# ai-forever/Kandinsky-2

Hardware: AMD Instinct MI355X
Metric: UNet denoise steps/sec @ 768x768 bs=1, 50 steps (higher is better)
Workload: dtype bf16; 1 GPU; Kandinsky-2.x text2img 768x768, decoder_steps=50, bs=1/GPU (CFG batch 2x4x96x96), 2.1-architecture UNet (1.23B) p_sampler step; parity pinned against the reference's modules; head=2.1, tile_configs_measured_in_this_process=0, images_per_gpu=1, parallelism=prompt-sharded x1, weights by one RCCL broadcast, world_size_observed=1, graph=True, chains=1, loop_graph=a 5-step loop replayed as ONE hipGraph (83 replay(s) = 415 timed steps)

## Files before the change

### include/k22.h

```cpp
#ifndef K22_H
#define K22_H
#include <stddef.h>
#include <stdint.h>
#ifdef __cplusplus
extern "C" {
#endif

#define K22_OK 0
#define K22_EINVAL (-1)
#define K22_EHIP (-2)
#define K22_ENOMEM (-3)

#define K22_BF16 0
#define K22_F32 1
#define K22_F16 2
#define K22_F16X3 3
#define K22_F16X2 4

int k22_version(void);
#define K22_BUILD_PACKED_FP32 1
#define K22_BUILD_DEBUG_VARIANTS 2
int k22_build_flags(void);
const char* k22_last_error(void);
int k22_set_option(const char* name, int value);
long k22_debug_counter(const char* name);
size_t k22_stream_frag_bytes(int Npad, int taps, int Kc, int dtype);
int k22_stream_repack(const void* W, void* out, int Npad, int taps, int Kc, int dtype, void* stream);
int k22_debug_set_stream_frag(const void* wfrag, const void* wsfrag);
int k22_debug_set_stream_scratch(void* scratch, size_t bytes);

typedef struct K22UNetConfig {
  int dtype;
  int in_channels;
  int model_channels;
  int out_channels;
  int num_res_blocks;
  int n_levels;
  int channel_mult[8];
  int n_attention_ds;
  int attention_ds[8];
  int num_head_channels;
  int ctx_dim;
  int ctx_len;
  int n_image_embs;
  int text_dim1;
  int text_dim2;
  int image_dim;
  int head_type;
  int hint_channels;
} K22UNetConfig;

typedef struct K22Weight {
  const char* name;
  const void* ptr;
} K22Weight;

typedef struct K22UNet K22UNet;

int k22_unet_create(const K22UNetConfig* cfg, const K22Weight* weights, int n_weights, K22UNet** out);
void k22_unet_destroy(K22UNet* u);


int k22_unet_plan(K22UNet* u, int B, int H, int W, size_t* workspace_bytes);
int k22_unet_bind(K22UNet* u, void* workspace, size_t workspace_bytes);

int k22_unet_set_condition(K22UNet* u, const float* full_emb, const float* pooled_emb, const float* image_emb,
                           void* stream);

int k22_unet_set_hint(K22UNet* u, const float* hint, void* stream);

int k22_unet_forward(K22UNet* u, const float* x, const float* timesteps, const float* inpaint_image,
                     const float* inpaint_mask, float* out, int use_graph, void* stream);

int k22_unet_sample_loop(K22UNet* u, float* x, float* x_tmp, const float* timesteps, const float* noise_seq, const float* init_img,
                         const float* mask, const float* inpaint_image, const float* inpaint_mask, const float* table,
                         const int* table_rows, int n_steps, float guidance, float clamp_lo, float clamp_hi, int pct_index,
                         double pct_gamma, void* scratch, int use_graph, void* stream);
int k22_unet_num_ops(const K22UNet* u);
int k22_unet_set_autotune(K22UNet* u, int on);
int k22_unet_tuning_report(const K22UNet* u, char* buf, size_t cap);

int k22_comm_broadcast_weights(void* arena, size_t bytes, int root, void* nccl_comm, void* stream);

int k22_tile_table_load(const char* path);
int k22_tile_table_save(const char* path);
int k22_tile_table_size(void);
int k22_tile_table_measured(void);
void k22_tile_table_clear(void);

int k22_unet_profile(K22UNet* u, int reps, double* ms, double* flops, double* bytes, int* launches, void* stream);

size_t k22_sampler_scratch_bytes(int N, int HW);
int k22_ddim_step(const float* x, const float* model_out, const float* noise, const float* table_row, float guidance, int use_cfg,
                  float* x_out, float* x0_out, int N, int HW, void* stream);
int k22_prepare_mask(const float* mask, float* out, int C, int H, int W, void* stream);
int k22_plms_step(const float* x, const float* model_out, const float* eps_hist1, const float* eps_hist2, const float* eps_hist3, int order,
                  const float* table_row, float guidance, int use_cfg, float* x_out, float* eps_out, float* x0_out, int N, int HW, void* stream);
int k22_sampler_step(const float* x, const float* model_out, const float* noise, const float* init_img,
                     const float* mask, const float* table, int step_index, float guidance, int use_cfg,
                     float clamp_lo, float clamp_hi, int pct_index, double pct_gamma, void* scratch,
                     float* x_out, float* x0_out, int N, int HW, void* stream);

int k22_gemm(const void* A0, const void* A1, const void* Wp, const float* bias, const void* residual, void* out,
             void* partial, int M, int N, int Npad, int K0, int K1, long lda0, long lda1, int ldo, int ldr,
             int out_f32, int act, int splitk, int bm, int bn, int dtype, void* stream);
int k22_x3_pack(const float* src, void* dst, long n, float scale, void* stream);
int k22_conv3x3(const void* x_padded, const void* Wp, const float* bias, const void* residual, void* out,
                void* partial, int B, int H, int W, int Cin, int Cout, int Npad, int out_mode, int act, int splitk,
                int bm, int bn, int dtype, void* stream);
int k22_conv3x3_skip(const void* x_padded, const void* Wp, const float* bias, const void* skip0, const void* skip1,
                     int SK0, int SK1, const void* Ws, const float* bias_s, void* out, void* partial, int B, int H, int W,
                     int Cin, int Cout, int Npad, int splitk, int bm, int dtype, void* stream);
int k22_conv3x3_gnstats(const void* x_padded, const void* Wp, const float* bias, const void* residual, void* out,
                        void* partial, int B, int H, int W, int Cin, int Cout, int Npad, int splitk, int bm, int bn,
                        float* stats, int stats_capacity_rows, int* rows_per_image, int dtype, void* stream);
int k22_gemm_gnstats(const void* A, const void* Wp, const float* bias, const void* residual, void* out, void* partial,
                     int B, int H, int W, int N, int Npad, int K, int splitk, int bm, float* stats,
                     int stats_capacity_rows, int* rows_per_image, int dtype, void* stream);
typedef struct K22IgemmProblem {
  int dtype, taps, M, N, Kc, K0, H, W;
  int out_mode, res_f32, act, a_raw, want_stats;
  int SK0, SK1;
  int att_T, att_S, att_Tkp;
  int ldo, ldr;
  int has_frag;
  int algo, bm, bn, splitk, stages;
} K22IgemmProblem;
typedef struct K22IgemmOperands {
  const void *A0, *A1, *Wp, *bias, *residual;
  void *out, *partial;
  const void *S0, *S1, *Ws, *bias2;
  void *kall, *vtall;
  const void *Wfrag, *Wsfrag;
  float* stats;
  int stats_capacity_rows;
} K22IgemmOperands;
int k22_igemm_cfg_accepted(const K22IgemmProblem* pr);
int k22_igemm_cfg(const K22IgemmProblem* pr, const K22IgemmOperands* ops, int* rows_per_image, void* stream);
int k22_debug_conv_trace(const void* x_padded, const void* Wp, const float* bias, void* out, int B, int H, int W, int Cin, int Cout,
                         int Npad, unsigned long long* trace, void* stream);
int k22_conv3x3_gn(const void* x0, const void* x1, int C0, int C1, const float* gamma, const float* beta, const float* film, long film_ld,
                   float eps, int act, void* scratch, const void* Wp, const float* bias, const void* residual, void* out, void* partial,
                   int B, int H, int W, int Cout, int Npad, int splitk, int bm, int algo, int dtype, void* stream);
int k22_groupnorm(const void* x0, const void* x1, int C0, int C1, int B, int H, int W, const float* gamma,
                  const float* beta, const float* film, long film_ld, float eps, int act, int mode, int pad,
                  void* scratch, void* out, int dtype, void* stream);
size_t k22_groupnorm_scratch_bytes(int B, int C);
int k22_attention(const void* qkv, const void* ctxkv, void* kall, void* vtall, void* out, int B, int H, int T, int S,
                  int dtype, void* stream);
int k22_qkv_project(const void* x, const void* Wp, const float* bias, void* q_out, void* kall, void* vtall,
                    int B, int H, int T, int S, int K, int bm, int bn, int dtype, void* stream);
int k22_qkv_project_stream(const void* x, const void* Wp, const float* bias, void* q_out, void* kall, void* vtall, void* partial,
                           int B, int H, int T, int S, int K, int bm, int splitk, int dtype, void* stream);
int k22_linear_smallm(const float* x, const void* W, const float* bias, const float* add, float* out, int M, int N,
                      int K, int act_in, int act_out, int wdtype, void* stream);
int k22_conv3x3_direct(const float* x, const float* w, const float* bias, float* y, int B, int Cin, int Cout, int Hin, int Win,
                       int stride, int act, void* stream);

size_t k22_afrag_bytes(int M, int K);
int k22_afrag_pack(const void* A, long lda, void* out, int M, int K, int dtype, void* stream);
int k22_skinny_gemm(const void* Afrag, const void* Wfrag, const float* bias, void* out, float* partial, int M, int N, int Npad, int K,
                    int splitk, int epi, int act, int ldo, int mt, int nb, int dtype, void* stream);
int k22_finish_ln(const float* partial, int splitk, const float* bias, float* x, long ldx, const float* gain, const float* beta, void* yfrag,
                  int M, int N, float eps, int dtype, void* stream);
int k22_small_attention(const void* qkv, const float* qkv_partial, int nsplit, const float* qkv_bias, void* out, int out_frag, int B, int H, int T,
                        int causal, const float* key_valid, int kv_n, int dtype, void* stream);

typedef struct K22PriorConfig {
  int dtype;
  int text_ctx;
  int xf_width;
  int xf_layers;
  int xf_heads;
  int xf_final_ln;
  int clip_dim;
  int clip_xf_width;
} K22PriorConfig;
typedef struct K22Prior K22Prior;
int k22_prior_create(const K22PriorConfig* cfg, const K22Weight* weights, int n_weights, K22Prior** out);
void k22_prior_destroy(K22Prior* m);
int k22_prior_plan(K22Prior* m, int B, size_t* workspace_bytes);
int k22_prior_bind(K22Prior* m, void* workspace, size_t workspace_bytes);
int k22_prior_tuning_report(const K22Prior* m, char* buf, size_t cap);
int k22_prior_forward(K22Prior* m, const float* x, const float* timesteps, const float* text_emb, const float* text_enc,
                      const float* key_valid, float* out, void* stream);
int k22_prior_sampler_step(const float* x, const float* model_out, const float* noise, const float* scales, const float* table_row,
                           float clamp, float* x_out, int bs, int D, void* stream);

typedef struct K22MoVQConfig {
  int dtype;
  int ch;
  int n_levels;
  int ch_mult[8];
  int num_res_blocks;
  int attn_levels;
  int z_channels;
  int out_ch;
} K22MoVQConfig;
typedef struct K22MoVQ K22MoVQ;
int k22_movq_create(const K22MoVQConfig* cfg, const K22Weight* weights, int n_weights, K22MoVQ** out);
void k22_movq_destroy(K22MoVQ* m);
int k22_movq_plan(K22MoVQ* m, int B, int h, int w, size_t* workspace_bytes);
int k22_movq_bind(K22MoVQ* m, void* workspace, size_t workspace_bytes);
int k22_movq_decode(K22MoVQ* m, const float* z, float* out, unsigned char* out_u8, void* stream);
int k22_movq_plan_encoder(K22MoVQ* m, int B, int H, int W, size_t* workspace_bytes);
int k22_movq_encode(K22MoVQ* m, const float* image, float* latent, void* stream);
int k22_movq_num_ops(const K22MoVQ* m);

enum { K22_ENC_CLIP_TEXT = 0, K22_ENC_CLIP_VISION = 1, K22_ENC_XLMR = 2 };
typedef struct K22EncoderConfig {
  int dtype;
  int kind;
  int width;
  int layers;
  int heads;
  int n_ctx;
  int vocab;
  int out_dim;
  int image_size;
  int patch;
  int max_pos;
  int pad_id;
  float ln_eps;
  int mlp_dim;
  int hidden_act;
} K22EncoderConfig;
typedef struct K22Encoder K22Encoder;
int k22_encoder_create(const K22EncoderConfig* cfg, const K22Weight* weights, int n_weights, K22Encoder** out);
void k22_encoder_destroy(K22Encoder* m);
int k22_encoder_plan(K22Encoder* m, int B, size_t* workspace_bytes);
int k22_encoder_bind(K22Encoder* m, void* workspace, size_t workspace_bytes);
int k22_encoder_forward(K22Encoder* m, const int* tokens, const float* key_valid, const float* image, float* seq_out, float* pooled_out,
                        void* stream);

int k22_blend_noised(const float* x, const float* init, const float* noise, const float* mask, float sa, float sb, float* out,
                     int N, int C, int HW, int broadcast_first, void* stream);

#ifdef __cplusplus
}
#endif
#endif
```

### kandinsky-2_amd/_lib.py

```python
from __future__ import annotations

import ctypes as C
import os

_HERE = os.path.dirname(os.path.abspath(__file__))
LIB_PATH = os.environ.get("K22_LIB_PATH") or os.path.join(_HERE, "libk22hip.so")
TILE_TABLE_PATH = os.path.join(_HERE, "tiles_gfx950.txt")

K22_BF16, K22_F32, K22_F16, K22_F16X3, K22_F16X2 = 0, 1, 2, 3, 4
F16X3 = "f16x3"
F16X2 = "f16x2"
SPLIT_DTYPES = (F16X3, F16X2)
X3_WSCALE = 256.0


def dtype_code(backend_dtype) -> int:
    import torch
    try:
        return {torch.bfloat16: K22_BF16, torch.float32: K22_F32, torch.float16: K22_F16, F16X3: K22_F16X3, F16X2: K22_F16X2}[backend_dtype]
    except KeyError:
        raise ValueError('backend_dtype must be torch.bfloat16, torch.float16, torch.float32 "f16x3" or "f16x2"') from None
ACT_NONE, ACT_SILU, ACT_GELU = 0, 1, 2
OUT_ROWMAJOR, OUT_ROWMAJOR_F32, OUT_NCHW_F32, OUT_QKV = 0, 1, 2, 3


class K22UNetConfig(C.Structure):
    _fields_ = [
        ("dtype", C.c_int), ("in_channels", C.c_int), ("model_channels", C.c_int), ("out_channels", C.c_int),
        ("num_res_blocks", C.c_int), ("n_levels", C.c_int), ("channel_mult", C.c_int * 8),
        ("n_attention_ds", C.c_int), ("attention_ds", C.c_int * 8), ("num_head_channels", C.c_int),
        ("ctx_dim", C.c_int), ("ctx_len", C.c_int), ("n_image_embs", C.c_int), ("text_dim1", C.c_int),
        ("text_dim2", C.c_int), ("image_dim", C.c_int), ("head_type", C.c_int), ("hint_channels", C.c_int),
    ]


class K22IgemmProblem(C.Structure):
    _fields_ = [(n, C.c_int) for n in (
        "dtype", "taps", "M", "N", "Kc", "K0", "H", "W", "out_mode", "res_f32", "act", "a_raw", "want_stats", "SK0", "SK1",
        "att_T", "att_S", "att_Tkp", "ldo", "ldr", "has_frag", "algo", "bm", "bn", "splitk", "stages")]


class K22IgemmOperands(C.Structure):
    _fields_ = [(n, C.c_void_p) for n in (
        "A0", "A1", "Wp", "bias", "residual", "out", "partial", "S0", "S1", "Ws", "bias2", "kall", "vtall", "Wfrag", "Wsfrag",
        "stats")] + [("stats_capacity_rows", C.c_int)]


class K22MoVQConfig(C.Structure):
    _fields_ = [("dtype", C.c_int), ("ch", C.c_int), ("n_levels", C.c_int), ("ch_mult", C.c_int * 8),
                ("num_res_blocks", C.c_int), ("attn_levels", C.c_int), ("z_channels", C.c_int), ("out_ch", C.c_int)]


class K22PriorConfig(C.Structure):
    _fields_ = [("dtype", C.c_int), ("text_ctx", C.c_int), ("xf_width", C.c_int), ("xf_layers", C.c_int), ("xf_heads", C.c_int),
                ("xf_final_ln", C.c_int), ("clip_dim", C.c_int), ("clip_xf_width", C.c_int)]


class K22EncoderConfig(C.Structure):
    _fields_ = [("dtype", C.c_int), ("kind", C.c_int), ("width", C.c_int), ("layers", C.c_int), ("heads", C.c_int), ("n_ctx", C.c_int),
                ("vocab", C.c_int), ("out_dim", C.c_int), ("image_size", C.c_int), ("patch", C.c_int), ("max_pos", C.c_int),
                ("pad_id", C.c_int), ("ln_eps", C.c_float), ("mlp_dim", C.c_int), ("hidden_act", C.c_int)]


class K22Weight(C.Structure):
    _fields_ = [("name", C.c_char_p), ("ptr", C.c_void_p)]


_P, _I, _L, _F, _D, _Z = C.c_void_p, C.c_int, C.c_long, C.c_float, C.c_double, C.c_size_t

SIGNATURES = {
    "k22_version": (_I, []),
    "k22_build_flags": (_I, []),
    "k22_last_error": (C.c_char_p, []),
    "k22_set_option": (_I, [C.c_char_p, _I]),
    "k22_comm_broadcast_weights": (_I, [_P, _Z, _I, _P, _P]),
    "k22_tile_table_load": (_I, [C.c_char_p]),
    "k22_tile_table_save": (_I, [C.c_char_p]),
    "k22_tile_table_size": (_I, []),
    "k22_tile_table_measured": (_I, []),
    "k22_tile_table_clear": (None, []),
    "k22_unet_create": (_I, [C.POINTER(K22UNetConfig), C.POINTER(K22Weight), _I, C.POINTER(_P)]),
    "k22_unet_destroy": (None, [_P]),
    "k22_unet_plan": (_I, [_P, _I, _I, _I, C.POINTER(_Z)]),
    "k22_unet_bind": (_I, [_P, _P, _Z]),
    "k22_unet_set_condition": (_I, [_P, _P, _P, _P, _P]),
    "k22_unet_set_hint": (_I, [_P, _P, _P]),
    "k22_unet_forward": (_I, [_P, _P, _P, _P, _P, _P, _I, _P]),
    "k22_unet_sample_loop": (_I, [_P, _P, _P, _P, _P, _P, _P, _P, _P, _P, C.POINTER(_I), _I, _F, _F, _F, _I, _D, _P, _I, _P]),
    "k22_unet_num_ops": (_I, [_P]),
    "k22_unet_set_autotune": (_I, [_P, _I]),
    "k22_unet_tuning_report": (_I, [_P, C.c_char_p, _Z]),
    "k22_unet_profile": (_I, [_P, _I, C.POINTER(_D), C.POINTER(_D), C.POINTER(_D), C.POINTER(_I), _P]),
    "k22_afrag_bytes": (_Z, [_I, _I]),
    "k22_afrag_pack": (_I, [_P, _L, _P, _I, _I, _I, _P]),
    "k22_skinny_gemm": (_I, [_P, _P, _P, _P, _P, _I, _I, _I, _I, _I, _I, _I, _I, _I, _I, _I, _P]),
    "k22_finish_ln": (_I, [_P, _I, _P, _P, _L, _P, _P, _P, _I, _I, _F, _I, _P]),
    "k22_small_attention": (_I, [_P, _P, _I, _P, _P, _I, _I, _I, _I, _I, _P, _I, _I, _P]),
    "k22_prior_create": (_I, [C.POINTER(K22PriorConfig), C.POINTER(K22Weight), _I, C.POINTER(_P)]),
    "k22_prior_destroy": (None, [_P]),
    "k22_prior_plan": (_I, [_P, _I, C.POINTER(_Z)]),
    "k22_prior_bind": (_I, [_P, _P, _Z]),
    "k22_prior_tuning_report": (_I, [_P, C.c_char_p, _Z]),
    "k22_prior_forward": (_I, [_P, _P, _P, _P, _P, _P, _P, _P]),
    "k22_prior_sampler_step": (_I, [_P, _P, _P, _P, _P, _F, _P, _I, _I, _P]),
    "k22_encoder_create": (_I, [C.POINTER(K22EncoderConfig), C.POINTER(K22Weight), _I, C.POINTER(_P)]),
    "k22_encoder_destroy": (None, [_P]),
    "k22_encoder_plan": (_I, [_P, _I, C.POINTER(_Z)]),
    "k22_encoder_bind": (_I, [_P, _P, _Z]),
    "k22_encoder_forward": (_I, [_P, _P, _P, _P, _P, _P, _P]),
    "k22_movq_create": (_I, [C.POINTER(K22MoVQConfig), C.POINTER(K22Weight), _I, C.POINTER(_P)]),
    "k22_movq_destroy": (None, [_P]),
    "k22_movq_plan": (_I, [_P, _I, _I, _I, C.POINTER(_Z)]),
    "k22_movq_bind": (_I, [_P, _P, _Z]),
    "k22_movq_decode": (_I, [_P, _P, _P, _P, _P]),
    "k22_movq_plan_encoder": (_I, [_P, _I, _I, _I, C.POINTER(_Z)]),
    "k22_movq_encode": (_I, [_P, _P, _P, _P]),
    "k22_movq_num_ops": (_I, [_P]),
    "k22_ddim_step": (_I, [_P, _P, _P, _P, _F, _I, _P, _P, _I, _I, _P]),
    "k22_blend_noised": (_I, [_P, _P, _P, _P, _F, _F, _P, _I, _I, _I, _I, _P]),
    "k22_prepare_mask": (_I, [_P, _P, _I, _I, _I, _P]),
    "k22_plms_step": (_I, [_P, _P, _P, _P, _P, _I, _P, _F, _I, _P, _P, _P, _I, _I, _P]),
    "k22_sampler_scratch_bytes": (_Z, [_I, _I]),
    "k22_sampler_step": (_I, [_P, _P, _P, _P, _P, _P, _I, _F, _I, _F, _F, _I, _D, _P, _P, _P, _I, _I, _P]),
    "k22_gemm": (_I, [_P, _P, _P, _P, _P, _P, _P, _I, _I, _I, _I, _I, _L, _L, _I, _I, _I, _I, _I, _I, _I, _I, _P]),
    "k22_x3_pack": (_I, [_P, _P, _L, _F, _P]),
    "k22_conv3x3": (_I, [_P, _P, _P, _P, _P, _P, _I, _I, _I, _I, _I, _I, _I, _I, _I, _I, _I, _I, _P]),
    "k22_conv3x3_skip": (_I, [_P, _P, _P, _P, _P, _I, _I, _P, _P, _P, _P, _I, _I, _I, _I, _I, _I, _I, _I, _I, _P]),
    "k22_gemm_gnstats": (_I, [_P, _P, _P, _P, _P, _P, _I, _I, _I, _I, _I, _I, _I, _I, _P, _I, C.POINTER(_I), _I, _P]),
    "k22_conv3x3_gnstats": (_I, [_P, _P, _P, _P, _P, _P, _I, _I, _I, _I, _I, _I, _I, _I, _I, _P, _I, C.POINTER(_I), _I, _P]),
    "k22_igemm_cfg_accepted": (_I, [C.POINTER(K22IgemmProblem)]),
    "k22_igemm_cfg": (_I, [C.POINTER(K22IgemmProblem), C.POINTER(K22IgemmOperands), C.POINTER(_I), _P]),
    "k22_conv3x3_gn": (_I, [_P, _P, _I, _I, _P, _P, _P, _L, _F, _I, _P, _P, _P, _P, _P, _P, _I, _I, _I, _I, _I, _I, _I, _I, _I, _P]),
    "k22_debug_conv_trace": (_I, [_P, _P, _P, _P, _I, _I, _I, _I, _I, _I, _P, _P]),
    "k22_groupnorm": (_I, [_P, _P, _I, _I, _I, _I, _I, _P, _P, _P, _L, _F, _I, _I, _I, _P, _P, _I, _P]),
    "k22_groupnorm_scratch_bytes": (_Z, [_I, _I]),
    "k22_attention": (_I, [_P, _P, _P, _P, _P, _I, _I, _I, _I, _I, _P]),
    "k22_qkv_project": (_I, [_P, _P, _P, _P, _P, _P, _I, _I, _I, _I, _I, _I, _I, _I, _P]),
    "k22_qkv_project_stream": (_I, [_P, _P, _P, _P, _P, _P, _P, _I, _I, _I, _I, _I, _I, _I, _I, _P]),
    "k22_linear_smallm": (_I, [_P, _P, _P, _P, _P, _I, _I, _I, _I, _I, _I, _P]),
    "k22_conv3x3_direct": (_I, [_P, _P, _P, _P, _I, _I, _I, _I, _I, _I, _I, _P]),
    "k22_debug_counter": (_L, [C.c_char_p]),
    "k22_stream_frag_bytes": (C.c_size_t, [_I, _I, _I, _I]),
    "k22_stream_repack": (_I, [_P, _P, _I, _I, _I, _I, _P]),
    "k22_debug_set_stream_frag": (_I, [_P, _P]),
    "k22_debug_set_stream_scratch": (_I, [_P, C.c_size_t]),
}

_lib = None


def lib() -> C.CDLL:
    global _lib
    if _lib is None:
        if not os.path.exists(LIB_PATH):
            raise RuntimeError(
                f"{LIB_PATH} is missing: the HIP extension is the only compute path (no CPU fallback). "
                "Build it with `python -c 'import __graft_entry__ as g; g.build()'`.")
        l = C.CDLL(LIB_PATH)
        for name, (res, args) in SIGNATURES.items():
            fn = getattr(l, name)
            fn.restype = res
            fn.argtypes = args
        _lib = l
        tbl = os.environ.get("K22_TILE_TABLE", TILE_TABLE_PATH)
        if tbl != "0" and os.path.exists(tbl):
            if l.k22_tile_table_load(tbl.encode()) < 0:
                raise RuntimeError(f"k22: cannot read the tile table {tbl}")
    return _lib


def check(rc: int) -> None:
    if rc != 0:
        msg = lib().k22_last_error()
        raise RuntimeError(f"k22 error {rc}: {msg.decode() if msg else ''}")


def weight_array(arena, table):
    base = arena.data_ptr()
    arr = (K22Weight * len(table))()
    names = []
    for i, (name, (off, _n)) in enumerate(table.items()):
        nb = name.encode()
        names.append(nb)
        arr[i].name = nb
        arr[i].ptr = base + off
    return arr, names


def plan_and_bind(plan_fn, bind_fn, handle, device, *shape):
    import torch
    nbytes = C.c_size_t()
    check(plan_fn(handle, *shape, C.byref(nbytes)))
    ws = torch.empty(nbytes.value + 256, dtype=torch.uint8, device=device)
    check(bind_fn(handle, (ws.data_ptr() + 255) // 256 * 256, nbytes.value))
    return ws


def ptr(t) -> int:
    if t is None:
        return None
    assert t.is_contiguous(), "k22: tensors crossing the C ABI must be contiguous"
    return t.data_ptr()


def current_stream() -> int:
    import torch
    return torch.cuda.current_stream().cuda_stream
```

### kandinsky-2_amd/csrc/capi.hip

```cpp
#include "kernels.h"
#include "elementwise.h"
#include "../../include/k22.h"
#include "tuning.h"
#include "skinny.h"
#include <dlfcn.h>
#include <stdio.h>
#include <string.h>

static thread_local char g_err[512] = "";

int k22_set_error(int code, const char* msg) {
  snprintf(g_err, sizeof(g_err), "%s", msg ? msg : "");
  return code;
}
int k22_set_error_hip(hipError_t e, const char* file, int line) {
  snprintf(g_err, sizeof(g_err), "HIP error %d (%s) at %s:%d", (int)e, hipGetErrorString(e), file, line);
  return K22_EHIP;
}

extern "C" {

int k22_version(void) { return 100; }
int k22_build_flags(void) {
  int f = 0;
#ifndef K22_NOPK
  f |= K22_BUILD_PACKED_FP32;
#endif
#if defined(K22_DEBUG_VARIANTS) || defined(K22_STREAM_DEBUG) || defined(K22_SKINNY_DEBUG)
  f |= K22_BUILD_DEBUG_VARIANTS;
#endif
  return f;
}

int k22_set_option(const char* name, int value) {
  if (name && !strcmp(name, "igemm_stages")) { igemm_set_default_stages(value); return K22_OK; }
  if (name && !strcmp(name, "igemm_xcd_remap")) { igemm_set_xcd_remap(value); return K22_OK; }
  if (name && !strcmp(name, "conv_algo")) { igemm_set_conv_algo(value); return K22_OK; }
  if (name && !strcmp(name, "gemm_algo")) { igemm_set_gemm_algo(value); return K22_OK; }
  return k22_set_error(K22_EINVAL, "k22_set_option: unknown option");
}
const char* k22_last_error(void) { return g_err; }

#ifdef K22_STREAM_DEBUG
static unsigned long long* g_dbg_trace = nullptr;
extern "C" int k22_debug_set_stream_trace(unsigned long long* t) { g_dbg_trace = t; return K22_OK; }
#define K22_DBG_TRACE(p) (p).st_trace = g_dbg_trace
#else
#define K22_DBG_TRACE(p) (void)0
#endif
static const void* g_dbg_wfrag = nullptr;
static const void* g_dbg_wsfrag = nullptr;
static void* g_dbg_scratch = nullptr;
static size_t g_dbg_scratch_bytes = 0;
static int dbg_frag(IgemmParams& p, int dtype, hipStream_t st) {
  K22_DBG_TRACE(p);
  p.Wfrag = g_dbg_wfrag; p.Wsfrag = g_dbg_wsfrag;
  if (g_dbg_wfrag || !g_dbg_scratch || dtype == K22_F32 || (p.taps != 1 && p.taps != 9) || p.Kc % 64 || p.Npad % 64) return K22_OK;
  const size_t n1 = stream_frag_bytes(p.Npad, p.taps, p.Kc, dtype);
  const bool skip = p.S0 != nullptr && p.Ws != nullptr && (p.SK0 + p.SK1) % 64 == 0;
  const size_t n2 = skip ? stream_frag_bytes(p.Npad, 1, p.SK0 + p.SK1, dtype) : 0;
  if (n1 + n2 > g_dbg_scratch_bytes) return k22_set_error(K22_ENOMEM, "debug stream scratch too small");
  if (int rc = launch_stream_repack(p.Wp, g_dbg_scratch, p.Npad, p.taps, p.Kc, dtype, st)) return rc;
  p.Wfrag = g_dbg_scratch;
  if (skip) {
    void* w2 = static_cast<char*>(g_dbg_scratch) + n1;
    if (int rc = launch_stream_repack(p.Ws, w2, p.Npad, 1, p.SK0 + p.SK1, dtype, st)) return rc;
    p.Wsfrag = w2;
  }
  return K22_OK;
}
#define K22_DBG_FRAG(p) do { if (int rc_ = dbg_frag((p), dtype, reinterpret_cast<hipStream_t>(stream))) return rc_; } while (0)
int k22_debug_set_stream_frag(const void* wfrag, const void* wsfrag) { g_dbg_wfrag = wfrag; g_dbg_wsfrag = wsfrag; return K22_OK; }
int k22_debug_set_stream_scratch(void* scratch, size_t bytes) { g_dbg_scratch = scratch; g_dbg_scratch_bytes = scratch ? bytes : 0; return K22_OK; }
size_t k22_stream_frag_bytes(int Npad, int taps, int Kc, int dtype) { return stream_frag_bytes(Npad, taps, Kc, dtype); }
int k22_stream_repack(const void* W, void* out, int Npad, int taps, int Kc, int dtype, void* stream) {
  return launch_stream_repack(W, out, Npad, taps, Kc, dtype, reinterpret_cast<hipStream_t>(stream));
}

long k22_debug_counter(const char* name) {
  if (name && !strcmp(name, "stream_launches")) return stream_launch_count();
  return -1;
}

int k22_comm_broadcast_weights(void* arena, size_t bytes, int root, void* nccl_comm, void* stream) {
  if (!arena || !nccl_comm) return k22_set_error(K22_EINVAL, "k22_comm_broadcast_weights: null arena / communicator");
  typedef int (*bcast_fn)(const void*, void*, size_t, int , int, void*, hipStream_t);
  static bcast_fn fn = nullptr;
  if (!fn) {
    void* sym = dlsym(RTLD_DEFAULT, "ncclBroadcast");
    if (!sym) {
      void* h = dlopen("librccl.so.1", RTLD_NOW | RTLD_GLOBAL);
      if (!h) h = dlopen("librccl.so", RTLD_NOW | RTLD_GLOBAL);
      if (h) sym = dlsym(h, "ncclBroadcast");
    }
    if (!sym) return k22_set_error(K22_EINVAL, "k22_comm_broadcast_weights: RCCL (ncclBroadcast) is not loadable in this process");
    fn = reinterpret_cast<bcast_fn>(sym);
  }
  const size_t piece = (size_t)1 << 30;
  char* base = reinterpret_cast<char*>(arena);
  for (size_t off = 0; off < bytes; off += piece) {
    const size_t n = bytes - off < piece ? bytes - off : piece;
    const int rc = fn(base + off, base + off, n,  1, root, nccl_comm, reinterpret_cast<hipStream_t>(stream));
    if (rc != 0) { char msg[96]; snprintf(msg, sizeof msg, "k22_comm_broadcast_weights: ncclBroadcast returned %d", rc); return k22_set_error(K22_EHIP, msg); }
  }
  return K22_OK;
}

int k22_tile_table_load(const char* path) {
  if (!path) return k22_set_error(K22_EINVAL, "k22_tile_table_load: null path");
  const int n = tile_table_load_file(path);
  if (n < 0) return k22_set_error(K22_EINVAL, "k22_tile_table_load: cannot read the file");
  return n;
}
int k22_tile_table_save(const char* path) {
  if (!path) return k22_set_error(K22_EINVAL, "k22_tile_table_save: null path");
  const int n = tile_table_save_file(path);
  if (n < 0) return k22_set_error(K22_EINVAL, "k22_tile_table_save: cannot write the file");
  return n;
}
int k22_tile_table_size(void) {
  TileTable& tt = tile_table();
  std::lock_guard<std::mutex> lk(tt.mu);
  return (int)tt.m.size();
}
int k22_tile_table_measured(void) {
  TileTable& tt = tile_table();
  std::lock_guard<std::mutex> lk(tt.mu);
  return (int)tt.measured;
}
void k22_tile_table_clear(void) {
  TileTable& tt = tile_table();
  std::lock_guard<std::mutex> lk(tt.mu);
  tt.m.clear();
  tt.measured = 0;
}

int k22_gemm(const void* A0, const void* A1, const void* Wp, const float* bias, const void* residual, void* out,
             void* partial, int M, int N, int Npad, int K0, int K1, long lda0, long lda1, int ldo, int ldr,
             int out_f32, int act, int splitk, int bm, int bn, int dtype, void* stream) {
  IgemmParams p = {};
    p.stages = -1;
  p.A0 = A0; p.A1 = A1; p.Wp = Wp; p.bias = bias; p.residual = residual; p.out = out;
  p.partial = reinterpret_cast<float*>(partial);
  p.M = M; p.N = N; p.Npad = Npad; p.Kc = K0 + K1; p.K0 = K0; p.taps = 1; p.lda0 = lda0; p.lda1 = lda1;
  p.ldo = ldo; p.ldr = ldr; p.out_mode = out_f32 ? IG_OUT_ROWMAJOR_F32 : IG_OUT_ROWMAJOR; p.act = act;
  p.splitk = splitk; p.force_bm = bm; p.force_bn = bn;
  p.a_raw = k22_is_split(dtype) ? 1 : 0;
  if (p.splitk == 0) p.splitk = partial ? igemm_choose_splitk(p, dtype) : 1;
  K22_DBG_FRAG(p);
  return launch_igemm(p, dtype, reinterpret_cast<hipStream_t>(stream));
}

int k22_x3_pack(const float* src, void* dst, long n, float scale, void* stream) {
  if (!src || !dst || n < 0) return k22_set_error(K22_EINVAL, "x3_pack: null argument");
  return launch_x3_pack(src, dst, n, scale, reinterpret_cast<hipStream_t>(stream));
}

int k22_conv3x3(const void* x_padded, const void* Wp, const float* bias, const void* residual, void* out,
                void* partial, int B, int H, int W, int Cin, int Cout, int Npad, int out_mode, int act, int splitk,
                int bm, int bn, int dtype, void* stream) {
  IgemmParams p = {};
    p.stages = -1;
  p.A0 = x_padded; p.Wp = Wp; p.bias = bias; p.residual = residual; p.out = out;
  p.partial = reinterpret_cast<float*>(partial);
  p.M = B * H * W; p.N = Cout; p.Npad = Npad; p.Kc = Cin; p.K0 = Cin; p.taps = 9; p.H = H; p.W = W;
  p.ldo = Cout; p.ldr = Cout; p.out_mode = out_mode; p.act = act; p.splitk = splitk; p.force_bm = bm; p.force_bn = bn;
  if (p.splitk == 0) p.splitk = partial ? igemm_choose_splitk(p, dtype) : 1;
  K22_DBG_FRAG(p);
  return launch_igemm(p, dtype, reinterpret_cast<hipStream_t>(stream));
}

int k22_conv3x3_gnstats(const void* x_padded, const void* Wp, const float* bias, const void* residual, void* out,
                        void* partial, int B, int H, int W, int Cin, int Cout, int Npad, int splitk, int bm, int bn,
                        float* stats, int stats_capacity_rows, int* rows_per_image, int dtype, void* stream) {
  IgemmParams p = {};
  p.stages = -1;
  p.A0 = x_padded; p.Wp = Wp; p.bias = bias; p.residual = residual; p.out = out;
  p.partial = reinterpret_cast<float*>(partial);
  p.M = B * H * W; p.N = Cout; p.Npad = Npad; p.Kc = Cin; p.K0 = Cin; p.taps = 9; p.H = H; p.W = W;
  p.ldo = Cout; p.ldr = Cout; p.out_mode = IG_OUT_ROWMAJOR; p.act = K22_ACT_NONE; p.splitk = splitk; p.force_bm = bm; p.force_bn = bn;
  if (p.splitk == 0) p.splitk = partial ? igemm_choose_splitk(p, dtype) : 1;
  const int rpi = igemm_stats_rows_per_image(p, dtype);
  if (rows_per_image) *rows_per_image = rpi;
  if (rpi <= 0) return k22_set_error(K22_EINVAL, "conv3x3_gnstats: this configuration cannot produce GroupNorm partial sums");
  if (rpi * B > stats_capacity_rows) return k22_set_error(K22_ENOMEM, "conv3x3_gnstats: stats buffer too small");
  p.stats = stats;
  K22_DBG_FRAG(p);
  return launch_igemm(p, dtype, reinterpret_cast<hipStream_t>(stream));
}

int k22_gemm_gnstats(const void* A, const void* Wp, const float* bias, const void* residual, void* out, void* partial,
                     int B, int H, int W, int N, int Npad, int K, int splitk, int bm, float* stats,
                     int stats_capacity_rows, int* rows_per_image, int dtype, void* stream) {
  IgemmParams p = {};
  p.stages = -1;
  p.A0 = A; p.Wp = Wp; p.bias = bias; p.residual = residual; p.out = out; p.partial = reinterpret_cast<float*>(partial);
  p.M = B * H * W; p.N = N; p.Npad = Npad; p.Kc = K; p.K0 = K; p.taps = 1; p.H = H; p.W = W; p.lda0 = K;
  p.ldo = N; p.ldr = N; p.out_mode = IG_OUT_ROWMAJOR; p.act = K22_ACT_NONE; p.splitk = splitk > 0 ? splitk : 1;
  p.force_bm = bm; p.algo = (bm == 160 || bm == 288) ? 20 : 10;
  p.a_raw = k22_is_split(dtype) ? 1 : 0;
  const int rpi = igemm_stats_rows_per_image(p, dtype);
  if (rows_per_image) *rows_per_image = rpi;
  if (rpi <= 0) return k22_set_error(K22_EINVAL, "gemm_gnstats: this configuration cannot produce GroupNorm partial sums");
  if (rpi * B > stats_capacity_rows) return k22_set_error(K22_ENOMEM, "gemm_gnstats: stats buffer too small");
  p.stats = stats;
  K22_DBG_FRAG(p);
  return launch_igemm(p, dtype, reinterpret_cast<hipStream_t>(stream));
}

int k22_conv3x3_skip(const void* x_padded, const void* Wp, const float* bias, const void* skip0, const void* skip1,
                     int SK0, int SK1, const void* Ws, const float* bias_s, void* out, void* partial, int B, int H, int W,
                     int Cin, int Cout, int Npad, int splitk, int bm, int dtype, void* stream) {
  IgemmParams p = {};
  p.stages = -1;
  p.A0 = x_padded; p.Wp = Wp; p.bias = bias; p.out = out; p.partial = reinterpret_cast<float*>(partial);
  p.M = B * H * W; p.N = Cout; p.Npad = Npad; p.Kc = Cin; p.K0 = Cin; p.taps = 9; p.H = H; p.W = W;
  p.ldo = Cout; p.ldr = Cout; p.out_mode = IG_OUT_ROWMAJOR; p.act = K22_ACT_NONE; p.splitk = splitk; p.force_bm = bm; p.force_bn = 0;
  p.S0 = skip0; p.S1 = skip1; p.SK0 = SK0; p.SK1 = SK1; p.Ws = Ws; p.bias2 = bias_s; p.algo = 0;
  if (p.splitk == 0) p.splitk = partial ? igemm_choose_splitk(p, dtype) : 1;
  K22_DBG_FRAG(p);
  return launch_igemm(p, dtype, reinterpret_cast<hipStream_t>(stream));
}

static int igemm_problem_tuned(const K22IgemmProblem& d, Tuned& t) {
  if (d.dtype < K22_BF16 || d.dtype > K22_F16X2) return k22_set_error(K22_EINVAL, "igemm_cfg: bad dtype");
  if ((d.taps != 1 && d.taps != 9) || d.M <= 0 || d.N <= 0 || d.Kc <= 0 || d.K0 <= 0 || d.K0 > d.Kc)
    return k22_set_error(K22_EINVAL, "igemm_cfg: bad problem (taps 1 / 9, M, N > 0, 0 < K0 <= Kc)");
  if (d.out_mode < IG_OUT_ROWMAJOR || d.out_mode > IG_OUT_QKV || d.SK0 < 0 || d.SK1 < 0 || (d.SK1 > 0 && d.SK0 == 0))
    return k22_set_error(K22_EINVAL, "igemm_cfg: bad output mode / skip widths");
  if (d.taps == 9 && (d.H <= 0 || d.W <= 0 || d.M % (d.H * d.W))) return k22_set_error(K22_EINVAL, "igemm_cfg: a convolution needs M = B * H * W");
  const void* mark = reinterpret_cast<const void*>(1);
  IgemmParams& p = t.p;
  p = IgemmParams{};
  p.stages = -1;
  p.M = d.M; p.N = d.N; p.Npad = (d.N + 63) / 64 * 64; p.Kc = d.Kc; p.K0 = d.K0; p.taps = d.taps; p.H = d.H; p.W = d.W;
  p.lda0 = d.K0; p.lda1 = d.Kc - d.K0;
  p.ldo = d.ldo > 0 ? d.ldo : (d.out_mode == IG_OUT_QKV ? d.N / 3 : d.N);
  p.ldr = d.ldr > 0 ? d.ldr : (d.res_f32 ? p.ldo : d.N);
  p.out_mode = d.out_mode; p.act = d.act; p.res_f32 = d.res_f32 ? 1 : 0; p.a_raw = d.a_raw ? 1 : 0;
  p.Wp = mark; p.bias = reinterpret_cast<const float*>(mark);
  if (d.SK0 > 0) { p.S0 = mark; p.S1 = d.SK1 > 0 ? mark : nullptr; p.SK0 = d.SK0; p.SK1 = d.SK1; p.Ws = mark; p.bias2 = reinterpret_cast<const float*>(mark); }
  if (d.out_mode == IG_OUT_QKV) { p.att_T = d.att_T; p.att_S = d.att_S; p.att_Tkp = d.att_Tkp; }
  if (d.has_frag) { p.Wfrag = mark; if (d.SK0 > 0) p.Wsfrag = mark; }
  t.want_stats = d.want_stats != 0;
  t.dt = d.dtype;
  tuned_make_candidates(t, d.dtype);
  return K22_OK;
}
static Cfg igemm_problem_cfg(const K22IgemmProblem& d) {
  Cfg c; c.algo = d.algo; c.bm = d.bm; c.bn = d.bn; c.splitk = d.splitk; c.stages = d.stages;
  return c;
}

int k22_igemm_cfg_accepted(const K22IgemmProblem* pr) {
  if (!pr) return k22_set_error(K22_EINVAL, "igemm_cfg_accepted: null problem");
  Tuned t;
  if (int rc = igemm_problem_tuned(*pr, t)) return rc;
  return tuned_is_candidate(t, igemm_problem_cfg(*pr)) ? 1 : 0;
}

int k22_igemm_cfg(const K22IgemmProblem* pr, const K22IgemmOperands* ops, int* rows_per_image, void* stream) {
  if (rows_per_image) *rows_per_image = 0;
  if (!pr || !ops) return k22_set_error(K22_EINVAL, "igemm_cfg: null problem / operands");
  const K22IgemmProblem& d = *pr;
  const K22IgemmOperands& o = *ops;
  Tuned t;
  if (int rc = igemm_problem_tuned(d, t)) return rc;
  const Cfg c = igemm_problem_cfg(d);
  if (!tuned_is_candidate(t, c)) return k22_set_error(K22_EINVAL, "igemm_cfg: this build does not generate the configuration for the problem");
  if (!o.A0 || !o.Wp || !o.out) return k22_set_error(K22_EINVAL, "igemm_cfg: A0, Wp and out are required");
  if (d.K0 < d.Kc && !o.A1) return k22_set_error(K22_EINVAL, "igemm_cfg: A1 missing for the concat operand");
  if (d.SK0 > 0 && (!o.S0 || !o.Ws || (d.SK1 > 0 && !o.S1))) return k22_set_error(K22_EINVAL, "igemm_cfg: fused-skip operands missing");
  if (d.out_mode == IG_OUT_QKV && (!o.kall || !o.vtall)) return k22_set_error(K22_EINVAL, "igemm_cfg: kall / vtall missing");
  if ((c.splitk > 1 || c.algo == 20) && !o.partial) return k22_set_error(K22_EINVAL, "igemm_cfg: the configuration needs the fp32 partial buffer");
  if (c.algo == 20 && (!o.Wfrag || (d.SK0 > 0 && !o.Wsfrag))) return k22_set_error(K22_EINVAL, "igemm_cfg: algo 20 needs the fragment-major weights");
  IgemmParams q = t.p;
  tuned_apply_cfg(q, c);
  q.A0 = o.A0; q.A1 = o.A1; q.Wp = o.Wp; q.bias = reinterpret_cast<const float*>(o.bias); q.residual = o.residual; q.out = o.out;
  q.partial = reinterpret_cast<float*>(o.partial);
  q.S0 = d.SK0 > 0 ? o.S0 : nullptr; q.S1 = d.SK1 > 0 ? o.S1 : nullptr; q.Ws = d.SK0 > 0 ? o.Ws : nullptr;
  q.bias2 = d.SK0 > 0 ? reinterpret_cast<const float*>(o.bias2) : nullptr;
  q.kall = o.kall; q.vtall = o.vtall;
  q.Wfrag = c.algo == 20 ? o.Wfrag : nullptr; q.Wsfrag = (c.algo == 20 && d.SK0 > 0) ? o.Wsfrag : nullptr;
  if (t.want_stats) {
    const int rpi = igemm_stats_rows_per_image(q, d.dtype);
    const int B = d.H > 0 ? d.M / (d.H * d.W) : 1;
    if (rpi <= 0) return k22_set_error(K22_EINVAL, "igemm_cfg: this configuration cannot produce GroupNorm partial sums");
    if (!o.stats || (long)rpi * B > o.stats_capacity_rows) return k22_set_error(K22_ENOMEM, "igemm_cfg: stats buffer missing / too small");
    if (rows_per_image) *rows_per_image = rpi;
    q.stats = o.stats;
  }
  return launch_igemm(q, d.dtype, reinterpret_cast<hipStream_t>(stream));
}

int k22_debug_conv_trace(const void* x_padded, const void* Wp, const float* bias, void* out, int B, int H, int W, int Cin, int Cout,
                         int Npad, unsigned long long* trace, void* stream) {
  IgemmParams p = {};
  p.stages = -1;
  p.A0 = x_padded; p.Wp = Wp; p.bias = bias; p.out = out;
  p.M = B * H * W; p.N = Cout; p.Npad = Npad; p.Kc = Cin; p.K0 = Cin; p.taps = 9; p.H = H; p.W = W;
  p.ldo = Cout; p.ldr = Cout; p.out_mode = IG_OUT_ROWMAJOR; p.act = K22_ACT_NONE; p.splitk = 1; p.trace = trace;
  return launch_conv3_halo_trace(p, K22_BF16, reinterpret_cast<hipStream_t>(stream));
}

size_t k22_groupnorm_scratch_bytes(int B, int C) {
  return (size_t)B * 128 * C * 2 * sizeof(float) + (size_t)B * C * 2 * sizeof(float) + 512;
}

int k22_groupnorm(const void* x0, const void* x1, int C0, int C1, int B, int H, int W, const float* gamma,
                  const float* beta, const float* film, long film_ld, float eps, int act, int mode, int pad,
                  void* scratch, void* out, int dtype, void* stream) {
  hipStream_t st = reinterpret_cast<hipStream_t>(stream);
  const int C = C0 + C1, HW = H * W;
  const int out_x3 = k22_is_split(dtype) ? 1 : 0;
  dtype = k22_storage_dtype(dtype);
  float* partial = reinterpret_cast<float*>(scratch);
  float* coeff = partial + (size_t)B * 128 * C * 2;
  const int rc = launch_gn_stats_coeff(x0, x1, C0, C1, B, HW, eps, gamma, beta, film, film_ld, partial, coeff, dtype, st);
  if (rc) return rc;
  GnApplyParams ap = {};
  ap.x0 = x0; ap.x1 = x1; ap.C0 = C0; ap.C1 = C1; ap.B = B; ap.H = H; ap.W = W; ap.mode = mode; ap.pad = pad; ap.act = act;
  ap.coeff = coeff; ap.out = out; ap.out_x3 = out_x3;
  return launch_gn_apply(ap, dtype, st);
}

int k22_conv3x3_gn(const void* x0, const void* x1, int C0, int C1, const float* gamma, const float* beta, const float* film, long film_ld,
                   float eps, int act, void* scratch, const void* Wp, const float* bias, const void* residual, void* out, void* partial,
                   int B, int H, int W, int Cout, int Npad, int splitk, int bm, int algo, int dtype, void* stream) {
  hipStream_t st = reinterpret_cast<hipStream_t>(stream);
  const int C = C0 + C1, HW = H * W;
  const int sdt = k22_storage_dtype(dtype);
  float* part = reinterpret_cast<float*>(scratch);
  float* coeff = part + (size_t)B * 128 * C * 2;
  const int rc = launch_gn_stats_coeff(x0, x1, C0, C1, B, HW, eps, gamma, beta, film, film_ld, part, coeff, sdt, st);
  if (rc) return rc;
  IgemmParams p = {};
  p.stages = -1;
  p.Wp = Wp; p.bias = bias; p.residual = residual; p.out = out; p.partial = reinterpret_cast<float*>(partial);
  p.M = B * H * W; p.N = Cout; p.Npad = Npad; p.Kc = C; p.K0 = C; p.taps = 9; p.H = H; p.W = W;
  p.ldo = Cout; p.ldr = Cout; p.out_mode = IG_OUT_ROWMAJOR; p.act = K22_ACT_NONE; p.splitk = splitk > 0 ? splitk : 1; p.force_bm = bm; p.algo = algo;
  p.gn_coeff = coeff; p.gn_x0 = x0; p.gn_x1 = x1; p.gn_C0 = C0; p.gn_act = act;
  return launch_igemm(p, dtype, st);
}


int k22_attention(const void* qkv, const void* ctxkv, void* kall, void* vtall, void* out, int B, int H, int T, int S,
                  int dtype, void* stream) {
  hipStream_t st = reinterpret_cast<hipStream_t>(stream);
  const int C = H * 64, Tk = S + T, Tkp = (Tk + 63) / 64 * 64;
  KvPackParams kp;
  kp.qkv = qkv; kp.ctxkv = ctxkv; kp.kall = kall; kp.vtall = vtall; kp.B = B; kp.H = H; kp.T = T; kp.S = S; kp.Tkp = Tkp;
  int rc = launch_kv_pack(kp, k22_storage_dtype(dtype), st);
  if (rc) return rc;
  AttentionParams ap = {};
  ap.q = qkv; ap.ldq = 3 * C; ap.kall = kall; ap.vtall = vtall; ap.out = out; ap.ldo = C;
  ap.B = B; ap.H = H; ap.T = T; ap.Tk = Tk; ap.Tkp = Tkp; ap.scale = 0.125f;
  return launch_attention(ap, dtype, st);
}

int k22_qkv_project(const void* x, const void* Wp, const float* bias, void* q_out, void* kall, void* vtall,
                    int B, int H, int T, int S, int K, int bm, int bn, int dtype, void* stream) {
  const int C = H * 64, Tkp = (S + T + 63) / 64 * 64;
  IgemmParams p = {};
  p.stages = -1;
  p.A0 = x; p.Wp = Wp; p.bias = bias; p.out = q_out; p.kall = kall; p.vtall = vtall;
  p.M = B * T; p.N = 3 * C; p.Npad = 3 * C; p.Kc = K; p.K0 = K; p.taps = 1; p.lda0 = K; p.lda1 = 0;
  p.ldo = C; p.ldr = 3 * C; p.out_mode = IG_OUT_QKV; p.act = K22_ACT_NONE; p.splitk = 1; p.force_bm = bm; p.force_bn = bn;
  p.att_T = T; p.att_S = S; p.att_Tkp = Tkp; p.H = 1; p.W = T;
  p.a_raw = k22_is_split(dtype) ? 1 : 0;
  K22_DBG_FRAG(p);
  return launch_igemm(p, dtype, reinterpret_cast<hipStream_t>(stream));
}

int k22_qkv_project_stream(const void* x, const void* Wp, const float* bias, void* q_out, void* kall, void* vtall, void* partial,
                           int B, int H, int T, int S, int K, int bm, int splitk, int dtype, void* stream) {
  const int C = H * 64, Tkp = (S + T + 63) / 64 * 64;
  IgemmParams p = {};
  p.stages = -1;
  p.A0 = x; p.Wp = Wp; p.bias = bias; p.out = q_out; p.kall = kall; p.vtall = vtall; p.partial = reinterpret_cast<float*>(partial);
  p.M = B * T; p.N = 3 * C; p.Npad = 3 * C; p.Kc = K; p.K0 = K; p.taps = 1; p.lda0 = K; p.lda1 = 0;
  p.ldo = C; p.ldr = 3 * C; p.out_mode = IG_OUT_QKV; p.act = K22_ACT_NONE; p.splitk = splitk > 0 ? splitk : 1; p.force_bm = bm; p.algo = 20;
  p.att_T = T; p.att_S = S; p.att_Tkp = Tkp; p.H = 1; p.W = T;
  if (!stream_supported(p, dtype, bm == 288 ? 9 : 5)) return k22_set_error(K22_EINVAL, "qkv_project_stream: unsupported problem");
  K22_DBG_FRAG(p);
  return launch_igemm(p, dtype, reinterpret_cast<hipStream_t>(stream));
}

size_t k22_afrag_bytes(int M, int K) { return afrag_bytes(M, K); }
int k22_afrag_pack(const void* A, long lda, void* out, int M, int K, int dtype, void* stream) {
  return launch_afrag_pack(A, lda, out, M, K, dtype, reinterpret_cast<hipStream_t>(stream));
}
int k22_skinny_gemm(const void* Afrag, const void* Wfrag, const float* bias, void* out, float* partial, int M, int N, int Npad, int K,
                    int splitk, int epi, int act, int ldo, int mt, int nb, int dtype, void* stream) {
  SkinnyParams q = {};
  q.Af = Afrag; q.Wf = Wfrag; q.bias = bias; q.out = out; q.partial = partial; q.M = M; q.N = N; q.Npad = Npad; q.K = K; q.MA = (M + 31) / 32;
  q.splitk = splitk > 0 ? splitk : 1; q.epi = epi; q.act = act; q.ldo = ldo;
  q.trace = reinterpret_cast<unsigned long long*>(g_dbg_scratch);
  return launch_skinny(q, dtype, mt, nb, reinterpret_cast<hipStream_t>(stream));
}
int k22_finish_ln(const float* partial, int splitk, const float* bias, float* x, long ldx, const float* gain, const float* beta, void* yfrag,
                  int M, int N, float eps, int dtype, void* stream) {
  FinishLnParams q = {};
  q.partial = partial; q.splitk = splitk; q.bias = bias; q.x = x; q.ldx = ldx; q.g = gain; q.b = beta; q.yfrag = yfrag; q.M = M; q.N = N;
  q.MA = (M + 31) / 32; q.eps = eps;
  return launch_finish_ln(q, dtype, reinterpret_cast<hipStream_t>(stream));
}
int k22_small_attention(const void* qkv, const float* qkv_partial, int nsplit, const float* qkv_bias, void* out, int out_frag, int B, int H, int T,
                        int causal, const float* key_valid, int kv_n, int dtype, void* stream) {
  SmallAttnParams ap = {};
  ap.qkv = qkv; ap.part = qkv_partial; ap.nsplit = nsplit; ap.bias = qkv_bias; ap.ldq = 3 * H * 64; ap.out = out; ap.ldo = H * 64; ap.out_frag = out_frag; ap.MA = (B * T + 31) / 32;
  ap.B = B; ap.H = H; ap.T = T; ap.scale = 0.125f; ap.causal = causal; ap.key_valid = key_valid; ap.kv_ld = kv_n; ap.kv_n = kv_n;
  return launch_small_attention(ap, dtype, reinterpret_cast<hipStream_t>(stream));
}

int k22_linear_smallm(const float* x, const void* W, const float* bias, const float* add, float* out, int M, int N,
                      int K, int act_in, int act_out, int wdtype, void* stream) {
  LinearSmallParams lp = {};
  lp.x = x; lp.ldx = K; lp.W = W; lp.bias = bias; lp.add = add; lp.ld_add = N; lp.out = out; lp.ldo = N;
  lp.M = M; lp.N = N; lp.K = K; lp.act_in = act_in; lp.act_out = act_out;
  return launch_linear_smallm(lp, wdtype, reinterpret_cast<hipStream_t>(stream));
}

int k22_conv3x3_direct(const float* x, const float* w, const float* bias, float* y, int B, int Cin, int Cout, int Hin, int Win,
                       int stride, int act, void* stream) {
  if (!x || !w || !bias || !y) return k22_set_error(K22_EINVAL, "conv3x3_direct: null argument");
  if (B < 1 || Cin < 1 || Cout < 1 || Hin < 1 || Win < 1) return k22_set_error(K22_EINVAL, "conv3x3_direct: empty shape");
  if (act != K22_ACT_NONE && act != K22_ACT_SILU) return k22_set_error(K22_EINVAL, "conv3x3_direct: act must be 0 (none) or 1 (SiLU)");
  ConvDirectParams p = {};
  p.x = x; p.w = w; p.bias = bias; p.y = y;
  p.B = B; p.Cin = Cin; p.Cout = Cout; p.Hin = Hin; p.Win = Win; p.stride = stride; p.act = act;
  return launch_conv3x3_direct(p, reinterpret_cast<hipStream_t>(stream));
}

int k22_ddim_step(const float* x, const float* model_out, const float* noise, const float* table_row, float guidance, int use_cfg,
                  float* x_out, float* x0_out, int N, int HW, void* stream) {
  if (!x || !model_out || !table_row || !x_out) return k22_set_error(K22_EINVAL, "ddim_step: null argument");
  return launch_ddim_step(x, model_out, noise, table_row, guidance, use_cfg, x_out, x0_out, N, HW, reinterpret_cast<hipStream_t>(stream));
}

int k22_prepare_mask(const float* mask, float* out, int C, int H, int W, void* stream) {
  if (!mask || !out) return k22_set_error(K22_EINVAL, "prepare_mask: null argument");
  return launch_prepare_mask(mask, out, C, H, W, reinterpret_cast<hipStream_t>(stream));
}

int k22_plms_step(const float* x, const float* model_out, const float* eps_hist1, const float* eps_hist2, const float* eps_hist3, int order,
                  const float* table_row, float guidance, int use_cfg, float* x_out, float* eps_out, float* x0_out, int N, int HW, void* stream) {
  if (!x || !model_out || !table_row || !x_out) return k22_set_error(K22_EINVAL, "plms_step: null argument");
  return launch_plms_step(x, model_out, eps_hist1, eps_hist2, eps_hist3, order, table_row, guidance, use_cfg, x_out, eps_out, x0_out, N, HW,
                          reinterpret_cast<hipStream_t>(stream));
}

size_t k22_sampler_scratch_bytes(int N, int HW) { return (size_t)N * 4 * HW * sizeof(float) + 256; }

int k22_sampler_step(const float* x, const float* model_out, const float* noise, const float* init_img,
                     const float* mask, const float* table, int step_index, float guidance, int use_cfg,
                     float clamp_lo, float clamp_hi, int pct_index, double pct_gamma, void* scratch,
                     float* x_out, float* x0_out, int N, int HW, void* stream) {
  SamplerParams p = {};
  p.x = x; p.model_out = model_out; p.noise = noise; p.init_img = init_img; p.mask = mask; p.table = table;
  p.step = nullptr; p.step_host = step_index; p.guidance = guidance; p.clamp_lo = clamp_lo; p.clamp_hi = clamp_hi;
  p.use_cfg = use_cfg; p.n_lo = pct_index; p.gamma = pct_gamma;
  p.s_buf = reinterpret_cast<float*>(scratch);
  p.x0_buf = reinterpret_cast<float*>(scratch) + 64;
  p.x_out = x_out; p.x0_out = x0_out; p.N = N; p.HW = HW;
  if (pct_index >= 4 * HW) return k22_set_error(K22_EINVAL, "sampler: percentile index out of range");
  return launch_sampler_step(p, reinterpret_cast<hipStream_t>(stream));
}

}

__global__ __launch_bounds__(256) void lds_sentinel_kernel(int words, int spins, unsigned* rec) {
  extern __shared__ unsigned sent_lds[];
  for (int i = threadIdx.x; i < words; i += 256) sent_lds[i] = 0xA5000000u | (unsigned)i;
  __syncthreads();
  for (int s = 0; s < spins; ++s) {
    for (int i = threadIdx.x; i < words; i += 256) {
      const unsigned v = reinterpret_cast<volatile unsigned*>(sent_lds)[i];
      if (v != (0xA5000000u | (unsigned)i)) {
        const unsigned k = atomicAdd(rec, 1u);
        if (k < 255u) { rec[1 + 4 * k] = blockIdx.x; rec[2 + 4 * k] = 4u * i; rec[3 + 4 * k] = v; rec[4 + 4 * k] = (unsigned)s; }
        sent_lds[i] = 0xA5000000u | (unsigned)i;
      }
    }
    __builtin_amdgcn_s_sleep(8);
  }
}
extern "C" int k22_debug_lds_sentinel(int bytes, int workgroups, int spins, unsigned* rec, void* stream) {
  if (bytes <= 0 || bytes > 64 * 1024 || (bytes & 3) || !rec) return k22_set_error(K22_EINVAL, "lds_sentinel: bytes in 4..65536, multiple of 4");
  hipLaunchKernelGGL(lds_sentinel_kernel, dim3(workgroups), dim3(256), (size_t)bytes, reinterpret_cast<hipStream_t>(stream), bytes / 4, spins, rec);
  K22_CHECK_LAUNCH();
  return K22_OK;
}
```

### kandinsky-2_amd/csrc/elementwise.h

```cpp
#pragma once
#include "common.h"

struct GnStatsParams {
  const void* x0; const void* x1;
  int C0, C1, HW, B, groups, nsplit;
  float* partial;
};
struct GnSrc { const float* st; int rpi, C; };
struct GnCoeffParams {
  GnSrc src[2];
  int HW, C, groups; float eps;
  const float* gamma; const float* beta;
  const float* film; int64_t film_ld;
  float* coeff;
};
struct GnApplyParams {
  const void* x0; const void* x1; int C0, C1;
  int B, H, W;
  int mode;
  int pad;
  int act;
  const float* coeff;
  void* out;
  int out_x3;
};
struct ConvInParams {
  const float* x; const float* img; const float* mask;
  const float* w; const float* bias;
  void* out;
  int B, H, W, Cin, Cout;
  int img_premul;
};
struct ConvDirectParams {
  const float* x; const float* w; const float* bias; float* y;
  int B, Cin, Cout, Hin, Win, stride, act;
};
int launch_conv3x3_direct(const ConvDirectParams& p, hipStream_t s);
struct LinearSmallParams {
  const float* x; int64_t ldx;
  const void* W;
  const float* bias;
  const float* add; int64_t ld_add;
  int add_mod;
  float* out; int64_t ldo;
  int M, N, K, act_in, act_out;
  int rows_per_wave;
};
struct KvPackParams {
  const void* qkv; const void* ctxkv; void* kall; void* vtall;
  int B, H, T, S, Tkp;
};
struct AttentionParams {
  const void* q; int64_t ldq;
  const void* kall; const void* vtall;
  void* out; int64_t ldo;
  int B, H, T, Tk, Tkp;
  float scale;
  int causal;
  const float* key_valid;
  int kv_ld, kv_n;
  int out_x3;
};
struct SmallAttnParams {
  const void* qkv; int64_t ldq;
  const float* part; int nsplit; const float* bias;
  void* out; int64_t ldo;
  int out_frag, MA;
  int B, H, T;
  float scale;
  int causal;
  const float* key_valid; int kv_ld, kv_n;
};
struct SamplerParams {
  const float* x;
  const float* model_out;
  const float* noise;
  const float* init_img;
  const float* mask;
  const float* table;
  const int* step;
  int step_host;
  float guidance, clamp_lo, clamp_hi;
  int use_cfg;
  int n_lo; double gamma;
  float* x0_buf;
  float* s_buf;
  float* x_out;
  float* x0_out;
  int N, HW;
};

int launch_x3_pack(const float* in, void* out, int64_t n, float scale, hipStream_t s);
int gn_nsplit(int B, int HW);
int launch_gn_stats(const GnStatsParams& p, int dtype, hipStream_t s);
int launch_gn_coeff(const GnCoeffParams& p, int B, hipStream_t s);
inline int launch_gn_stats_coeff(const void* x0, const void* x1, int C0, int C1, int B, int HW, float eps, const float* gamma, const float* beta,
                                 const float* film, int64_t film_ld, float* partial, float* coeff, int dtype, hipStream_t s) {
  const int nsplit = gn_nsplit(B, HW), C = C0 + C1;
  GnStatsParams sp = {};
  sp.x0 = x0; sp.x1 = x1; sp.C0 = C0; sp.C1 = C1; sp.HW = HW; sp.B = B; sp.groups = 32; sp.nsplit = nsplit; sp.partial = partial;
  const int rc = launch_gn_stats(sp, dtype, s);
  if (rc) return rc;
  GnCoeffParams cp = {};
  cp.src[0].st = partial; cp.src[0].rpi = nsplit; cp.src[0].C = C;
  cp.HW = HW; cp.C = C; cp.groups = 32; cp.eps = eps; cp.gamma = gamma; cp.beta = beta; cp.film = film; cp.film_ld = film_ld; cp.coeff = coeff;
  return launch_gn_coeff(cp, B, s);
}
int launch_gn_apply(const GnApplyParams& p, int dtype, hipStream_t s);
int launch_resample(const void* x, void* y, int B, int H, int W, int C, int mode, int dtype, hipStream_t s);
int launch_conv_in(const ConvInParams& p, int dtype, hipStream_t s);
int launch_timestep_embedding(const float* t, const float* freqs, float* out, int B, int half, hipStream_t s);
int launch_linear_smallm(const LinearSmallParams& p, int wdtype, hipStream_t s);
int launch_layernorm_f32(const float* x, const float* g, const float* b, float* y, int rows, int D, float eps, hipStream_t s);
int launch_cast_rows(const float* x, void* y, int rows, int cols, int64_t ldx, int64_t ldy, int dtype, hipStream_t s);
int launch_kv_pack(const KvPackParams& p, int dtype, hipStream_t s);
int launch_attention(const AttentionParams& p, int dtype, hipStream_t s);
int launch_small_attention(const SmallAttnParams& p, int dtype, hipStream_t s);
int launch_sampler_step(const SamplerParams& p, hipStream_t s);
int launch_plms_step(const float* x, const float* model_out, const float* h1, const float* h2, const float* h3, int order, const float* tab,
                     float guidance, int use_cfg, float* x_out, float* e_store, float* x0_out, int N, int HW, hipStream_t s);
int launch_prepare_mask(const float* old_mask, float* out, int C, int H, int W, hipStream_t s);
int launch_ddim_step(const float* x, const float* model_out, const float* noise, const float* tab, float guidance, int use_cfg,
                     float* x_out, float* x0_out, int N, int HW, hipStream_t s);

struct SpatialNormParams {
  const void* x;
  const float* coeff;
  const float* zq;
  const float* wy; const float* by;
  const float* wb; const float* bb;
  void* out;
  int B, H, W, C, h0, w0, shift, act, pad;
};
int launch_spatialnorm_apply(const SpatialNormParams& p, int dtype, hipStream_t s);
int launch_upsample2_pad(const void* x, void* y, int B, int H, int W, int C, int dtype, hipStream_t s);
int launch_softmax_rows(void* x, int64_t rows, int L, float scale, int dtype, hipStream_t s);
int launch_movq_prepare(const float* z, const float* wpq, const float* bpq, float* zq, void* xin, int B, int h, int w,
                        int Cpad, int dtype, hipStream_t s);
int launch_movq_enc_prepare(const float* img, void* xin, int B, int H, int W, int Cpad, int dtype, hipStream_t s);
int launch_pad_copy(const void* x, void* y, int B, int H, int W, int C, int dtype, hipStream_t s);
int launch_subsample_odd(const void* x, void* y, int B, int H, int W, int C, int dtype, hipStream_t s);
int launch_movq_quant_conv(const float* h, const float* wq, const float* bq, float* out, int B, int HW, hipStream_t s);
int launch_to_uint8_nhwc(const float* x, unsigned char* y, int B, int C, int H, int W, hipStream_t s);
```

### kandinsky-2_amd/csrc/elementwise.hip

```cpp
#include "kernels.h"
#include "elementwise.h"

__device__ __forceinline__ void load4(const bf16_t* p, float* f) {
  const uint2 r = *reinterpret_cast<const uint2*>(p);
  f[0] = __uint_as_float(r.x << 16); f[1] = __uint_as_float(r.x & 0xffff0000u);
  f[2] = __uint_as_float(r.y << 16); f[3] = __uint_as_float(r.y & 0xffff0000u);
}
__device__ __forceinline__ void load4(const f16_t* p, float* f) {
  const uint2 r = *reinterpret_cast<const uint2*>(p);
  unpack2_f16(r.x, f[0], f[1]); unpack2_f16(r.y, f[2], f[3]);
}
__device__ __forceinline__ void load4(const float* p, float* f) {
  const float4 r = *reinterpret_cast<const float4*>(p);
  f[0] = r.x; f[1] = r.y; f[2] = r.z; f[3] = r.w;
}

template <typename T>
__global__ __launch_bounds__(256) void gn_stats_kernel(GnStatsParams p) {
  __shared__ float red[1024 * 2 * 2];
  const int tid = threadIdx.x, b = blockIdx.y, s = blockIdx.x;
  const int C = p.C0 + p.C1, VP = C / 4;
  const int per = (p.HW + p.nsplit - 1) / p.nsplit;
  const int pix0 = s * per, pix1 = min(p.HW, pix0 + per);
  const T* x0 = reinterpret_cast<const T*>(p.x0) + (int64_t)b * p.HW * p.C0;
  const T* x1 = p.x1 ? reinterpret_cast<const T*>(p.x1) + (int64_t)b * p.HW * p.C1 : nullptr;
  int PL, pl;
  if (VP >= 256) { PL = 1; pl = 0; } else { PL = 256 / VP; pl = tid / VP; }
  float sum[3][4], sq[3][4];
  int vj[3];
#pragma unroll
  for (int j = 0; j < 3; ++j) {
    int v = (VP >= 256) ? tid + 256 * j : ((j == 0 && pl < PL) ? tid - pl * VP : VP);
    vj[j] = v < VP ? v : -1;
#pragma unroll
    for (int k = 0; k < 4; ++k) { sum[j][k] = 0.f; sq[j][k] = 0.f; }
  }
#pragma unroll
  for (int j = 0; j < 3; ++j) {
    if (vj[j] >= 0) {
      const int c = vj[j] * 4;
      const T* src = c < p.C0 ? x0 + c : x1 + (c - p.C0);
      const int64_t ld = c < p.C0 ? p.C0 : p.C1;
      int pix = pix0 + pl;
      for (; pix + 7 * PL < pix1; pix += 8 * PL) {
        float f[8][4];
#pragma unroll
        for (int u = 0; u < 8; ++u) load4(src + (int64_t)(pix + u * PL) * ld, f[u]);
#pragma unroll
        for (int k = 0; k < 4; ++k) {
          sum[j][k] += ((f[0][k] + f[1][k]) + (f[2][k] + f[3][k])) + ((f[4][k] + f[5][k]) + (f[6][k] + f[7][k]));
          sq[j][k] += ((f[0][k] * f[0][k] + f[1][k] * f[1][k]) + (f[2][k] * f[2][k] + f[3][k] * f[3][k])) +
                      ((f[4][k] * f[4][k] + f[5][k] * f[5][k]) + (f[6][k] * f[6][k] + f[7][k] * f[7][k]));
        }
      }
      for (; pix < pix1; pix += PL) {
        float f[4];
        load4(src + (int64_t)pix * ld, f);
#pragma unroll
        for (int k = 0; k < 4; ++k) { sum[j][k] += f[k]; sq[j][k] += f[k] * f[k]; }
      }
    }
  }
  float* out = p.partial + ((int64_t)b * p.nsplit + s) * C * 2;
  if (PL == 1) {
#pragma unroll
    for (int j = 0; j < 3; ++j)
      if (vj[j] >= 0) {
        float* o = out + (int64_t)vj[j] * 8;
        *reinterpret_cast<float4*>(o) = make_float4(sum[j][0], sq[j][0], sum[j][1], sq[j][1]);
        *reinterpret_cast<float4*>(o + 4) = make_float4(sum[j][2], sq[j][2], sum[j][3], sq[j][3]);
      }
    return;
  }
  if (vj[0] >= 0) {
    float* o = red + ((int64_t)pl * C + vj[0] * 4) * 2;
    *reinterpret_cast<float4*>(o) = make_float4(sum[0][0], sq[0][0], sum[0][1], sq[0][1]);
    *reinterpret_cast<float4*>(o + 4) = make_float4(sum[0][2], sq[0][2], sum[0][3], sq[0][3]);
  }
  __syncthreads();
  for (int i = tid; i < C * 2; i += 256) {
    float a = 0.f;
    for (int q = 0; q < PL; ++q) a += red[(int64_t)q * C * 2 + i];
    out[i] = a;
  }
}

__global__ __launch_bounds__(256) void gn_coeff_kernel(GnCoeffParams p) {
  __shared__ double red[4][2];
  __shared__ float ms[2];
  const int tid = threadIdx.x, lane = tid & 63, wave = tid >> 6, g = blockIdx.x, b = blockIdx.y;
  const int cg = p.C / p.groups;
  float pg = 0.f, pb = 0.f, psc = 1.f, psh = 0.f;
  if (tid < cg) {
    const int c = g * cg + tid;
    pg = p.gamma[c]; pb = p.beta[c];
    if (p.film != nullptr) {
      psc = 1.f + p.film[(int64_t)b * p.film_ld + c];
      psh = p.film[(int64_t)b * p.film_ld + p.C + c];
    }
  }
  double s = 0.0, q = 0.0;
  int off = 0;
#pragma unroll
  for (int k = 0; k < 2; ++k) {
    const GnSrc sr = p.src[k];
    if (sr.C > 0) {
      const int c_lo = max(g * cg, off), c_hi = min((g + 1) * cg, off + sr.C);
      const int nc = c_hi - c_lo;
      if (nc > 0) {
        const float* base = sr.st + ((int64_t)b * sr.rpi * sr.C + (c_lo - off)) * 2;
        const int items = sr.rpi * nc;
        int i = tid;
        for (; i + 768 < items; i += 1024) {
          float2 v[4];
#pragma unroll
          for (int u = 0; u < 4; ++u) {
            const int ii = i + 256 * u, r = ii / nc, cc = ii - r * nc;
            v[u] = *reinterpret_cast<const float2*>(base + ((int64_t)r * sr.C + cc) * 2);
          }
          s += ((double)v[0].x + (double)v[1].x) + ((double)v[2].x + (double)v[3].x);
          q += ((double)v[0].y + (double)v[1].y) + ((double)v[2].y + (double)v[3].y);
        }
        for (; i < items; i += 256) {
          const int r = i / nc, cc = i - r * nc;
          const float2 v = *reinterpret_cast<const float2*>(base + ((int64_t)r * sr.C + cc) * 2);
          s += (double)v.x;
          q += (double)v.y;
        }
      }
    }
    off += sr.C;
  }
#pragma unroll
  for (int o = 32; o > 0; o >>= 1) {
    s += __shfl_xor(s, o, 64);
    q += __shfl_xor(q, o, 64);
  }
  if (lane == 0) { red[wave][0] = s; red[wave][1] = q; }
  __syncthreads();
  if (tid == 0) {
    const double st = (red[0][0] + red[1][0]) + (red[2][0] + red[3][0]);
    const double qt = (red[0][1] + red[1][1]) + (red[2][1] + red[3][1]);
    const double n = (double)p.HW * (double)cg;
    const double mean = st / n;
    double var = qt / n - mean * mean;
    if (var < 0.0) var = 0.0;
    ms[0] = (float)mean;
    ms[1] = (float)(1.0 / sqrt(var + (double)p.eps));
  }
  __syncthreads();
  const float mean_f = ms[0], rstd_f = ms[1];
  if (tid < cg) {
    const int c = g * cg + tid;
    float A = rstd_f * pg;
    float Bc = pb - mean_f * A;
    if (p.film != nullptr) {
      A *= psc;
      Bc = Bc * psc + psh;
    }
    *reinterpret_cast<float2*>(p.coeff + ((int64_t)b * p.C + c) * 2) = make_float2(A, Bc);
  }
}

template <typename T>
__global__ __launch_bounds__(256) void gn_apply_kernel(GnApplyParams p) {
  constexpr int EPV = Vec16<T>::N;
  const bool fast = p.out_x3 != 0;
  const int C = p.C0 + p.C1, CV = C / EPV;
  const int Ho = p.mode == 1 ? p.H / 2 : (p.mode == 2 ? p.H * 2 : p.H);
  const int Wo = p.mode == 1 ? p.W / 2 : (p.mode == 2 ? p.W * 2 : p.W);
  const int pad = p.pad, Hp = Ho + 2 * pad, Wp = Wo + 2 * pad;
  const int idx = blockIdx.x * 256 + threadIdx.x;
  if (idx >= Wp * CV) return;
  const int xp = idx / CV, cv = idx - xp * CV;
  const int xo = xp - pad, yo = (int)blockIdx.y - pad, b = blockIdx.z;
  T* out = reinterpret_cast<T*>(p.out) + (((int64_t)b * Hp + blockIdx.y) * Wp + xp) * C + cv * EPV;
  Vec16<T> o;
  if (xo < 0 || yo < 0 || xo >= Wo || yo >= Ho) {
#pragma unroll
    for (int k = 0; k < EPV / 2; ++k) o.set2(k, 0.f, 0.f);
  } else {
    const int c = cv * EPV;
    const T* src; int cs, ld;
    if (c < p.C0) { src = reinterpret_cast<const T*>(p.x0); cs = c; ld = p.C0; }
    else { src = reinterpret_cast<const T*>(p.x1); cs = c - p.C0; ld = p.C1; }
    float A[EPV], Bc[EPV];
    const float* cf = p.coeff + ((int64_t)b * C + c) * 2;
#pragma unroll
    for (int k = 0; k < EPV; k += 2) {
      const float4 q = *reinterpret_cast<const float4*>(cf + 2 * k);
      A[k] = q.x; Bc[k] = q.y; A[k + 1] = q.z; Bc[k + 1] = q.w;
    }
    float r[EPV];
    if (p.mode == 1) {
      Vec16<T> v[4];
#pragma unroll
      for (int dy = 0; dy < 2; ++dy)
#pragma unroll
        for (int dx = 0; dx < 2; ++dx)
          v[dy * 2 + dx].raw = *reinterpret_cast<const decltype(v[0].raw)*>(src + ((int64_t)(b * p.H + 2 * yo + dy) * p.W + 2 * xo + dx) * ld + cs);
#pragma unroll
      for (int k = 0; k < EPV; ++k) {
        float acc = 0.f;
#pragma unroll
        for (int q = 0; q < 4; ++q) acc += fast ? apply_act_sel<true>(v[q].get(k) * A[k] + Bc[k], p.act) : apply_act_sel<false>(v[q].get(k) * A[k] + Bc[k], p.act);
        r[k] = acc * 0.25f;
      }
    } else {
      const int yi = p.mode == 2 ? yo >> 1 : yo, xi = p.mode == 2 ? xo >> 1 : xo;
      Vec16<T> v;
      v.raw = *reinterpret_cast<const decltype(v.raw)*>(src + ((int64_t)(b * p.H + yi) * p.W + xi) * ld + cs);
#pragma unroll
      for (int k = 0; k < EPV; ++k) r[k] = fast ? apply_act_sel<true>(v.get(k) * A[k] + Bc[k], p.act) : apply_act_sel<false>(v.get(k) * A[k] + Bc[k], p.act);
    }
#pragma unroll
    for (int k = 0; k < EPV / 2; ++k) o.set2(k, r[2 * k], r[2 * k + 1]);
  }
  if constexpr (sizeof(T) == 4) {
    if (p.out_x3) { x3_store4(out, x3_split4(o.raw)); return; }
  }
  *reinterpret_cast<decltype(o.raw)*>(out) = o.raw;
}

template <typename T>
__global__ __launch_bounds__(256) void resample_kernel(const void* xin, void* yout, int B, int H, int W, int C, int mode) {
  constexpr int EPV = Vec16<T>::N;
  const int CV = C / EPV;
  const int Ho = mode == 1 ? H / 2 : H * 2, Wo = mode == 1 ? W / 2 : W * 2;
  const int64_t total = (int64_t)B * Ho * Wo * CV;
  const T* x = reinterpret_cast<const T*>(xin);
  T* y = reinterpret_cast<T*>(yout);
  for (int64_t i = (int64_t)blockIdx.x * 256 + threadIdx.x; i < total; i += (int64_t)gridDim.x * 256) {
    const int cv = (int)(i % CV);
    int64_t t = i / CV;
    const int xo = (int)(t % Wo); t /= Wo;
    const int yo = (int)(t % Ho);
    const int b = (int)(t / Ho);
    Vec16<T> o;
    if (mode == 1) {
      float r[EPV];
#pragma unroll
      for (int k = 0; k < EPV; ++k) r[k] = 0.f;
#pragma unroll
      for (int dy = 0; dy < 2; ++dy)
#pragma unroll
        for (int dx = 0; dx < 2; ++dx) {
          Vec16<T> v;
          v.raw = *reinterpret_cast<const decltype(v.raw)*>(x + ((int64_t)(b * H + 2 * yo + dy) * W + 2 * xo + dx) * C + cv * EPV);
#pragma unroll
          for (int k = 0; k < EPV; ++k) r[k] += v.get(k);
        }
#pragma unroll
      for (int k = 0; k < EPV / 2; ++k) o.set2(k, r[2 * k] * 0.25f, r[2 * k + 1] * 0.25f);
    } else {
      o.raw = *reinterpret_cast<const decltype(o.raw)*>(x + ((int64_t)(b * H + (yo >> 1)) * W + (xo >> 1)) * C + cv * EPV);
    }
    *reinterpret_cast<decltype(o.raw)*>(y + i * EPV) = o.raw;
  }
}

constexpr int CONV_IN_PT = 8;
template <typename T, int CIN>
__global__ __launch_bounds__(128) void conv_in_kernel(ConvInParams p) {
  constexpr int PT = CONV_IN_PT, PW = PT + 2;
  __shared__ float patch[CIN][3][PW];
  const int tid = threadIdx.x;
  const int xt = blockIdx.x, y = blockIdx.y, b = blockIdx.z;
  const int x0 = xt * PT;
  const int hw = p.H * p.W;
  for (int i = tid; i < CIN * 3 * PW; i += 128) {
    const int c = i / (3 * PW), r = (i / PW) % 3, xx = i % PW;
    const int yy = y + r - 1, xs = x0 + xx - 1;
    float v = 0.f;
    if (yy >= 0 && yy < p.H && xs >= 0 && xs < p.W) {
      const int64_t o = (int64_t)yy * p.W + xs;
      if (c < 4) v = p.x[((int64_t)b * 4 + c) * hw + o];
      else if (c < 8) v = p.img[((int64_t)b * 4 + (c - 4)) * hw + o] * (p.img_premul ? 1.f : p.mask[(int64_t)b * hw + o]);
      else v = p.mask[(int64_t)b * hw + o];
    }
    patch[c][r][xx] = v;
  }
  __syncthreads();
  T* out = reinterpret_cast<T*>(p.out);
  for (int n = tid; n < p.Cout; n += 128) {
    float w[CIN * 9];
#pragma unroll
    for (int k = 0; k < CIN * 9; ++k) w[k] = p.w[(int64_t)k * p.Cout + n];
    const float bias = p.bias[n];
    for (int px = 0; px < PT && x0 + px < p.W; ++px) {
      float acc = bias;
#pragma unroll
      for (int c = 0; c < CIN; ++c)
#pragma unroll
        for (int r = 0; r < 3; ++r)
#pragma unroll
          for (int q = 0; q < 3; ++q) acc += w[c * 9 + r * 3 + q] * patch[c][r][px + q];
      out[((int64_t)(b * p.H + y) * p.W + x0 + px) * p.Cout + n] = from_f32<T>(acc);
    }
  }
}

template <int OCB>
__global__ __launch_bounds__(256) void conv3x3_direct_kernel(ConvDirectParams p) {
  const int Ho = (p.Hin - 1) / p.stride + 1, Wo = (p.Win - 1) / p.stride + 1;
  const int pix = blockIdx.x * 256 + threadIdx.x;
  const int oc0 = blockIdx.y * OCB, b = blockIdx.z;
  if (pix >= Ho * Wo) return;
  const int yo = pix / Wo, xo = pix - yo * Wo;
  const int yi = yo * p.stride - 1, xi = xo * p.stride - 1;
  float acc[OCB];
#pragma unroll
  for (int o = 0; o < OCB; ++o) acc[o] = (oc0 + o < p.Cout) ? p.bias[oc0 + o] : 0.f;
  const int64_t plane = (int64_t)p.Hin * p.Win;
  for (int c = 0; c < p.Cin; ++c) {
    const float* xp = p.x + ((int64_t)b * p.Cin + c) * plane;
    float v[9];
#pragma unroll
    for (int r = 0; r < 3; ++r)
#pragma unroll
      for (int q = 0; q < 3; ++q) {
        const int yy = yi + r, xx = xi + q;
        v[r * 3 + q] = (yy >= 0 && yy < p.Hin && xx >= 0 && xx < p.Win) ? xp[(int64_t)yy * p.Win + xx] : 0.f;
      }
#pragma unroll
    for (int o = 0; o < OCB; ++o) {
      if (oc0 + o < p.Cout) {
        const float* wp = p.w + ((int64_t)(oc0 + o) * p.Cin + c) * 9;
#pragma unroll
        for (int k = 0; k < 9; ++k) acc[o] += wp[k] * v[k];
      }
    }
  }
#pragma unroll
  for (int o = 0; o < OCB; ++o)
    if (oc0 + o < p.Cout) p.y[(((int64_t)b * p.Cout + oc0 + o) * Ho + yo) * Wo + xo] = apply_act(acc[o], p.act);
}

__global__ void timestep_embedding_kernel(const float* t, const float* freqs, float* out, int B, int half) {
  const int i = blockIdx.x * blockDim.x + threadIdx.x;
  if (i >= B * half) return;
  const int b = i / half, k = i - b * half;
  const float a = t[b] * freqs[k];
  out[(int64_t)b * 2 * half + k] = cosf(a);
  out[(int64_t)b * 2 * half + half + k] = sinf(a);
}

template <typename TW, int MT>
__global__ __launch_bounds__(256) void linear_smallm_kernel(LinearSmallParams p) {
  constexpr int EPC = 16 / sizeof(TW);
  extern __shared__ __attribute__((aligned(16))) char smem_lin[];
  float* xs = reinterpret_cast<float*>(smem_lin);
  const int tid = threadIdx.x, lane = tid & 63, wave = tid >> 6;
  for (int i = tid; i < MT * p.K; i += 256) {
    const int m = i / p.K, k = i - m * p.K;
    float xv = m < p.M ? p.x[(int64_t)m * p.ldx + k] : 0.f;
    if (p.act_in == K22_ACT_SILU) xv = silu_f(xv);
    xs[i] = xv;
  }
  __syncthreads();
  const int per_wave = p.rows_per_wave;
  const int n_begin = (blockIdx.x * 4 + wave) * per_wave;
  for (int r = 0; r < per_wave; ++r) {
    const int n = n_begin + r;
    if (n >= p.N) return;
    const TW* w = reinterpret_cast<const TW*>(p.W) + (int64_t)n * p.K;
    float acc[MT];
#pragma unroll
    for (int m = 0; m < MT; ++m) acc[m] = 0.f;
    for (int k = lane * EPC; k < p.K; k += 64 * EPC) {
      Vec16<TW> wv;
      wv.raw = *reinterpret_cast<const decltype(wv.raw)*>(w + k);
#pragma unroll
      for (int m = 0; m < MT; ++m) {
        const float* xr = xs + m * p.K + k;
#pragma unroll
        for (int e = 0; e < EPC; e += 4) {
          const float4 xv = *reinterpret_cast<const float4*>(xr + e);
          acc[m] += xv.x * wv.get(e) + xv.y * wv.get(e + 1) + xv.z * wv.get(e + 2) + xv.w * wv.get(e + 3);
        }
      }
    }
#pragma unroll
    for (int m = 0; m < MT; ++m) {
      float v = wave_sum(acc[m]);
      if (lane == 0 && m < p.M) {
        if (p.bias) v += p.bias[n];
        v = apply_act(v, p.act_out);
        if (p.add) v += p.add[(int64_t)(p.add_mod > 0 ? m % p.add_mod : m) * p.ld_add + n];
        p.out[(int64_t)m * p.ldo + n] = v;
      }
    }
  }
}

__global__ __launch_bounds__(256) void layernorm_f32_kernel(const float* x, const float* g, const float* bta, float* y, int D, float eps) {
  __shared__ float red[8];
  const int row = blockIdx.x, tid = threadIdx.x;
  const float* xr = x + (int64_t)row * D;
  float s = 0.f;
  for (int i = tid; i < D; i += 256) s += xr[i];
  s = wave_sum(s);
  if ((tid & 63) == 0) red[tid >> 6] = s;
  __syncthreads();
  const float mean = (red[0] + red[1] + red[2] + red[3]) / D;
  float q = 0.f;
  for (int i = tid; i < D; i += 256) { const float d = xr[i] - mean; q += d * d; }
  q = wave_sum(q);
  if ((tid & 63) == 0) red[4 + (tid >> 6)] = q;
  __syncthreads();
  const float rstd = rsqrtf((red[4] + red[5] + red[6] + red[7]) / D + eps);
  for (int i = tid; i < D; i += 256) y[(int64_t)row * D + i] = (xr[i] - mean) * rstd * g[i] + bta[i];
}

template <typename T>
__global__ void cast_rows_kernel(const float* x, void* yout, int rows, int cols, int64_t ldx, int64_t ldy) {
  T* y = reinterpret_cast<T*>(yout);
  const int64_t total = (int64_t)rows * cols;
  for (int64_t i = (int64_t)blockIdx.x * blockDim.x + threadIdx.x; i < total; i += (int64_t)gridDim.x * blockDim.x) {
    const int r = (int)(i / cols), c = (int)(i - (int64_t)r * cols);
    y[r * ldy + c] = from_f32<T>(x[r * ldx + c]);
  }
}

template <typename T>
__global__ __launch_bounds__(256) void kv_pack_kernel(KvPackParams p) {
  __shared__ T vt[64][66];
  const int tid = threadIdx.x, jt = blockIdx.x, h = blockIdx.y, b = blockIdx.z;
  const int C = p.H * 64, Tk = p.S + p.T;
  const T* qkv = reinterpret_cast<const T*>(p.qkv);
  const T* ckv = reinterpret_cast<const T*>(p.ctxkv);
  T* Kall = reinterpret_cast<T*>(p.kall) + ((int64_t)(b * p.H + h) * p.Tkp) * 64;
  T* VTall = reinterpret_cast<T*>(p.vtall) + ((int64_t)(b * p.H + h) * 64) * p.Tkp;
  for (int i = tid; i < 64 * 64; i += 256) {
    const int jj = i >> 6, d = i & 63;
    const int j = jt * 64 + jj;
    T kv = from_f32<T>(0.f), vv = from_f32<T>(0.f);
    if (j < p.S) {
      const T* r = ckv + (int64_t)(b * p.S + j) * 2 * C + h * 64 + d;
      kv = r[0]; vv = r[C];
    } else if (j < Tk) {
      const T* r = qkv + (int64_t)(b * p.T + (j - p.S)) * 3 * C + C + h * 64 + d;
      kv = r[0]; vv = r[C];
    }
    Kall[(int64_t)j * 64 + d] = kv;
    vt[d][jj] = vv;
  }
  __syncthreads();
  for (int i = tid; i < 64 * 64; i += 256) {
    const int d = i >> 6, jj = i & 63;
    VTall[(int64_t)d * p.Tkp + jt * 64 + jj] = vt[d][jj];
  }
}

__global__ __launch_bounds__(256) void x3_pack_kernel(const float4* __restrict__ in, u32x4_t* __restrict__ out, int64_t n4, float scale) {
  for (int64_t i = (int64_t)blockIdx.x * 256 + threadIdx.x; i < n4; i += (int64_t)gridDim.x * 256) {
    const float4 v = in[i];
    x3_store4(out + i, x3_split4(v.x * scale, v.y * scale, v.z * scale, v.w * scale));
  }
}
int launch_x3_pack(const float* in, void* out, int64_t n, float scale, hipStream_t s) {
  if (n % 8 || (uintptr_t)in % 16 || (uintptr_t)out % 32) return k22_set_error(K22_EINVAL, "x3_pack: n % 8 == 0, 16-byte aligned input, 32-byte aligned output (groups of eight)");
  const int64_t n4 = n / 4;
  int nb = (int)((n4 + 255) / 256);
  if (nb > 4096) nb = 4096;
  if (nb < 1) return K22_OK;
  hipLaunchKernelGGL(x3_pack_kernel, dim3(nb), dim3(256), 0, s, reinterpret_cast<const float4*>(in), reinterpret_cast<u32x4_t*>(out), n4, scale);
  K22_CHECK_LAUNCH();
  return K22_OK;
}

static inline int grid_for(int64_t total, int threads, int cap) {
  int64_t nb = (total + threads - 1) / threads;
  if (nb > cap) nb = cap;
  if (nb < 1) nb = 1;
  return (int)nb;
}

int gn_nsplit(int B, int HW) {
  int ns = 512 / (B > 0 ? B : 1);
  if (ns > 128) ns = 128;
  while (ns > 1 && HW / ns < 32) ns >>= 1;
  return ns < 1 ? 1 : ns;
}

int launch_gn_stats(const GnStatsParams& p, int dtype, hipStream_t s) {
  const int C = p.C0 + p.C1;
  if (p.groups != 32 || C % 128 != 0 || p.C0 % 4 != 0) return k22_set_error(K22_EINVAL, "gn_stats: need 32 groups, C % 128 == 0");
  if (C / 4 > 768) return k22_set_error(K22_EINVAL, "gn_stats: C too large (max 3072)");
  if (C / 4 < 256 && (256 / (C / 4)) * C > 2048) return k22_set_error(K22_EINVAL, "gn_stats: internal LDS bound");
  dim3 grid(p.nsplit, p.B);
  if (dtype == K22_BF16) hipLaunchKernelGGL(gn_stats_kernel<bf16_t>, grid, dim3(256), 0, s, p);
  else if (dtype == K22_F16) hipLaunchKernelGGL(gn_stats_kernel<f16_t>, grid, dim3(256), 0, s, p);
  else hipLaunchKernelGGL(gn_stats_kernel<float>, grid, dim3(256), 0, s, p);
  K22_CHECK_LAUNCH();
  return K22_OK;
}
int launch_gn_coeff(const GnCoeffParams& p, int B, hipStream_t s) {
  if (p.C / p.groups > 256) return k22_set_error(K22_EINVAL, "gn_coeff: more than 256 channels per group");
  hipLaunchKernelGGL(gn_coeff_kernel, dim3(p.groups, B), dim3(256), 0, s, p);
  K22_CHECK_LAUNCH();
  return K22_OK;
}
int launch_gn_apply(const GnApplyParams& p, int dtype, hipStream_t s) {
  const int C = p.C0 + p.C1;
  const int epv = dtype == K22_F32 ? 4 : 8;
  if (C % epv || p.C0 % epv) return k22_set_error(K22_EINVAL, "gn_apply: channel alignment");
  if (p.out_x3 && dtype != K22_F32) return k22_set_error(K22_EINVAL, "gn_apply: x3-chunk output is an option of the fp32 launch");
  const int Ho = p.mode == 1 ? p.H / 2 : (p.mode == 2 ? p.H * 2 : p.H);
  const int Wo = p.mode == 1 ? p.W / 2 : (p.mode == 2 ? p.W * 2 : p.W);
  const int Hp = Ho + 2 * p.pad, Wp = Wo + 2 * p.pad;
  if (Hp > 65535 || p.B > 65535) return k22_set_error(K22_EINVAL, "gn_apply: tensor too large");
  dim3 grid((Wp * (C / epv) + 255) / 256, Hp, p.B);
  if (dtype == K22_BF16) hipLaunchKernelGGL(gn_apply_kernel<bf16_t>, grid, dim3(256), 0, s, p);
  else if (dtype == K22_F16) hipLaunchKernelGGL(gn_apply_kernel<f16_t>, grid, dim3(256), 0, s, p);
  else hipLaunchKernelGGL(gn_apply_kernel<float>, grid, dim3(256), 0, s, p);
  K22_CHECK_LAUNCH();
  return K22_OK;
}
int launch_resample(const void* x, void* y, int B, int H, int W, int C, int mode, int dtype, hipStream_t s) {
  const int epv = dtype == K22_F32 ? 4 : 8;
  const int Ho = mode == 1 ? H / 2 : H * 2, Wo = mode == 1 ? W / 2 : W * 2;
  const int nb = grid_for((int64_t)B * Ho * Wo * (C / epv), 256, 8192);
  if (dtype == K22_BF16) hipLaunchKernelGGL(resample_kernel<bf16_t>, dim3(nb), dim3(256), 0, s, x, y, B, H, W, C, mode);
  else if (dtype == K22_F16) hipLaunchKernelGGL(resample_kernel<f16_t>, dim3(nb), dim3(256), 0, s, x, y, B, H, W, C, mode);
  else hipLaunchKernelGGL(resample_kernel<float>, dim3(nb), dim3(256), 0, s, x, y, B, H, W, C, mode);
  K22_CHECK_LAUNCH();
  return K22_OK;
}
int launch_conv_in(const ConvInParams& p, int dtype, hipStream_t s) {
  dim3 grid((p.W + CONV_IN_PT - 1) / CONV_IN_PT, p.H, p.B);
  if (p.Cin == 4) {
    if (dtype == K22_BF16) hipLaunchKernelGGL((conv_in_kernel<bf16_t, 4>), grid, dim3(128), 0, s, p);
    else if (dtype == K22_F16) hipLaunchKernelGGL((conv_in_kernel<f16_t, 4>), grid, dim3(128), 0, s, p);
    else hipLaunchKernelGGL((conv_in_kernel<float, 4>), grid, dim3(128), 0, s, p);
  } else if (p.Cin == 9) {
    if (dtype == K22_BF16) hipLaunchKernelGGL((conv_in_kernel<bf16_t, 9>), grid, dim3(128), 0, s, p);
    else if (dtype == K22_F16) hipLaunchKernelGGL((conv_in_kernel<f16_t, 9>), grid, dim3(128), 0, s, p);
    else hipLaunchKernelGGL((conv_in_kernel<float, 9>), grid, dim3(128), 0, s, p);
  } else if (p.Cin == 8) {
    if (dtype == K22_BF16) hipLaunchKernelGGL((conv_in_kernel<bf16_t, 8>), grid, dim3(128), 0, s, p);
    else if (dtype == K22_F16) hipLaunchKernelGGL((conv_in_kernel<f16_t, 8>), grid, dim3(128), 0, s, p);
    else hipLaunchKernelGGL((conv_in_kernel<float, 8>), grid, dim3(128), 0, s, p);
  } else {
    return k22_set_error(K22_EINVAL, "conv_in: in_channels must be 4, 8 or 9");
  }
  K22_CHECK_LAUNCH();
  return K22_OK;
}
int launch_conv3x3_direct(const ConvDirectParams& p, hipStream_t s) {
  if (p.stride != 1 && p.stride != 2) return k22_set_error(K22_EINVAL, "conv3x3_direct: stride must be 1 or 2");
  const int Ho = (p.Hin - 1) / p.stride + 1, Wo = (p.Win - 1) / p.stride + 1;
  constexpr int OCB = 8;
  dim3 grid((Ho * Wo + 255) / 256, (p.Cout + OCB - 1) / OCB, p.B);
  hipLaunchKernelGGL((conv3x3_direct_kernel<OCB>), grid, dim3(256), 0, s, p);
  K22_CHECK_LAUNCH();
  return K22_OK;
}
int launch_timestep_embedding(const float* t, const float* freqs, float* out, int B, int half, hipStream_t s) {
  hipLaunchKernelGGL(timestep_embedding_kernel, dim3((B * half + 255) / 256), dim3(256), 0, s, t, freqs, out, B, half);
  K22_CHECK_LAUNCH();
  return K22_OK;
}
template <typename TW>
static void launch_linear_m(const LinearSmallParams& p, int Mt, dim3 grid, size_t smem, hipStream_t s) {
  switch (Mt) {
    case 1: hipLaunchKernelGGL((linear_smallm_kernel<TW, 1>), grid, dim3(256), smem, s, p); break;
    case 2: hipLaunchKernelGGL((linear_smallm_kernel<TW, 2>), grid, dim3(256), smem, s, p); break;
    case 4: hipLaunchKernelGGL((linear_smallm_kernel<TW, 4>), grid, dim3(256), smem, s, p); break;
    default: hipLaunchKernelGGL((linear_smallm_kernel<TW, 8>), grid, dim3(256), smem, s, p); break;
  }
}
int launch_linear_smallm(const LinearSmallParams& p0, int wdtype, hipStream_t s) {
  if (p0.M > 8 || p0.M < 1) return k22_set_error(K22_EINVAL, "linear_smallm: M must be in 1..8");
  const int epc = wdtype == K22_F32 ? 4 : 8;
  if (p0.K % epc) return k22_set_error(K22_EINVAL, "linear_smallm: K alignment");
  const int Mt = p0.M <= 2 ? p0.M : (p0.M <= 4 ? 4 : 8);
  const size_t smem = (size_t)Mt * p0.K * 4;
  if (smem > 64 * 1024) return k22_set_error(K22_EINVAL, "linear_smallm: M*K too large for the LDS stage");
  LinearSmallParams p = p0;
  int rpw = 1;
  while (rpw < 8 && (p.N + 8 * rpw - 1) / (8 * rpw) >= 1024) rpw *= 2;
  p.rows_per_wave = rpw;
  dim3 grid((p.N + 4 * rpw - 1) / (4 * rpw));
  if (wdtype == K22_BF16) launch_linear_m<bf16_t>(p, Mt, grid, smem, s);
  else if (wdtype == K22_F16) launch_linear_m<f16_t>(p, Mt, grid, smem, s);
  else launch_linear_m<float>(p, Mt, grid, smem, s);
  K22_CHECK_LAUNCH();
  return K22_OK;
}
int launch_layernorm_f32(const float* x, const float* g, const float* b, float* y, int rows, int D, float eps, hipStream_t s) {
  hipLaunchKernelGGL(layernorm_f32_kernel, dim3(rows), dim3(256), 0, s, x, g, b, y, D, eps);
  K22_CHECK_LAUNCH();
  return K22_OK;
}
int launch_cast_rows(const float* x, void* y, int rows, int cols, int64_t ldx, int64_t ldy, int dtype, hipStream_t s) {
  const int nb = grid_for((int64_t)rows * cols, 256, 4096);
  if (dtype == K22_BF16) hipLaunchKernelGGL(cast_rows_kernel<bf16_t>, dim3(nb), dim3(256), 0, s, x, y, rows, cols, ldx, ldy);
  else if (dtype == K22_F16) hipLaunchKernelGGL(cast_rows_kernel<f16_t>, dim3(nb), dim3(256), 0, s, x, y, rows, cols, ldx, ldy);
  else hipLaunchKernelGGL(cast_rows_kernel<float>, dim3(nb), dim3(256), 0, s, x, y, rows, cols, ldx, ldy);
  K22_CHECK_LAUNCH();
  return K22_OK;
}
int launch_kv_pack(const KvPackParams& p, int dtype, hipStream_t s) {
  if (p.Tkp % 64) return k22_set_error(K22_EINVAL, "kv_pack: Tkp % 64");
  dim3 grid(p.Tkp / 64, p.H, p.B);
  if (dtype == K22_BF16) hipLaunchKernelGGL(kv_pack_kernel<bf16_t>, grid, dim3(256), 0, s, p);
  else if (dtype == K22_F16) hipLaunchKernelGGL(kv_pack_kernel<f16_t>, grid, dim3(256), 0, s, p);
  else hipLaunchKernelGGL(kv_pack_kernel<float>, grid, dim3(256), 0, s, p);
  K22_CHECK_LAUNCH();
  return K22_OK;
}
```

### kandinsky-2_amd/csrc/engine.hip

```cpp
#include "kernels.h"
#include "elementwise.h"
#include "../../include/k22.h"
#include "tuning.h"
#include "plan.h"

#include <deque>
#include <functional>
#include <map>
#include <memory>
#include <string>
#include <tuple>
#include <unordered_map>
#include <vector>
#include <stdio.h>
#include <stdlib.h>
#include <string.h>

int launch_step_advance(int* step, int delta, hipStream_t s);

namespace {

enum OpKind { OP_CONV3 = 0, OP_GEMM = 1, OP_GN = 2, OP_ATTN = 3, OP_MISC = 4, OP_NKINDS = 5 };

struct Op {
  std::function<int(hipStream_t)> fn;
  int kind = OP_MISC;
  double flops = 0.0;
  double flops2 = 0.0;
  double bytes = 0.0;
  int kernels = 1;
  Op() {}
  template <typename F> Op(F f, int k = OP_MISC, double fl = 0.0, double by = 0.0, int nk = 1) : fn(f), kind(k), flops(fl), bytes(by), kernels(nk) {}
  int operator()(hipStream_t st) const { return fn(st); }
};
typedef std::vector<Op> OpList;

struct Act {
  Slot* s0 = nullptr; int C0 = 0;
  Slot* s1 = nullptr; int C1 = 0;
  int H = 0, W = 0;
  const Tuned* p0 = nullptr; Slot* st0 = nullptr;
  const Tuned* p1 = nullptr; Slot* st1 = nullptr;
  int C() const { return C0 + C1; }
};

}

struct K22UNet : GraphPlan {
  K22UNetConfig cfg;
  int sdt;

  int B = 0, H = 0, W = 0;
  OpList ops;
  OpList cond_ops;
  OpList hint_ops;
  bool hint_set = false;
  int fuse_skip = 1;
  int fuse_gn = 0;
  struct GnLink { const Tuned* consumer = nullptr; };
  std::deque<GnLink> gn_links;
  int stream_frag = 1;
  struct FragJob { const void* W; Slot* slot; int Npad, taps, Kc; };
  std::vector<FragJob> frag_jobs;
  bool frag_done = false;
  int repack_frags(hipStream_t st) {
    for (auto& j : frag_jobs) {
      int rc = launch_stream_repack(j.W, ptr(j.slot), j.Npad, j.taps, j.Kc, dtype, st);
      if (rc) return rc;
    }
    frag_done = true;
    return K22_OK;
  }
  bool cond_set = false;
  GraphCache loop;
  std::vector<unsigned long long> loop_key;

  Slot *s_xin, *s_img, *s_mask, *s_t, *s_out;
  Slot *s_temb, *s_e1, *s_emb, *s_film, *s_xfproj, *s_ctx;
  Slot *s_full, *s_pool, *s_imgemb, *s_tmpf, *s_tmpf2, *s_fullT;
  Slot *s_part, *s_coeff, *s_P1, *s_U1, *s_P2, *s_S, *s_N, *s_QKV, *s_KALL, *s_VT, *s_ATT, *s_splitk, *s_flush;
  Slot *s_U1st;
  Slot *s_ctxf = nullptr, *s_hint = nullptr, *s_hintin = nullptr, *s_hbuf[2] = {nullptr, nullptr};
  Slot* s_h[3];
  Slot* s_hst[3];
  std::vector<Slot*> s_ctxkv;
  int n_attn = 0;
  int64_t film_total = 0;
  float* film_all = nullptr;
  size_t film_all_bytes = 0;
  int hoist_time = 1;
  const float* film_cur = nullptr;
  const float* film_base() const { return film_cur ? film_cur : ptr<float>(s_film); }
  struct TimeW { const float* freqs; const float* w0; const float* b0; const float* w2; const float* b2; const void* we; const float* be; int mc, ted, dt; } tw = {};
  int time_rows(const float* t, float* temb, float* e1, float* emb, float* film, int rows, hipStream_t st) {
    int rc = launch_timestep_embedding(t, tw.freqs, temb, rows, tw.mc / 2, st);
    if (rc) return rc;
    LinearSmallParams lp = {};
    lp.x = temb; lp.ldx = tw.mc; lp.W = tw.w0; lp.bias = tw.b0; lp.out = e1; lp.ldo = tw.ted;
    lp.M = rows; lp.N = tw.ted; lp.K = tw.mc; lp.act_in = K22_ACT_NONE; lp.act_out = K22_ACT_SILU;
    rc = launch_linear_smallm(lp, K22_F32, st);
    if (rc) return rc;
    lp.x = e1; lp.ldx = tw.ted; lp.W = tw.w2; lp.bias = tw.b2; lp.add = ptr<float>(s_xfproj); lp.ld_add = tw.ted; lp.add_mod = B;
    lp.out = emb; lp.K = tw.ted; lp.act_out = K22_ACT_NONE;
    rc = launch_linear_smallm(lp, K22_F32, st);
    if (rc) return rc;
    LinearSmallParams le = {};
    le.x = emb; le.ldx = tw.ted; le.W = tw.we; le.bias = tw.be; le.out = film; le.ldo = film_total;
    le.M = rows; le.N = (int)film_total; le.K = tw.ted; le.act_in = K22_ACT_SILU; le.act_out = K22_ACT_NONE;
    return launch_linear_smallm(le, tw.dt, st);
  }

  float* model_out() { return ptr<float>(s_out); }
  int exec(hipStream_t st) { return run_ops(st); }
  int exec_eager(hipStream_t st) { return run_eager(st, [this](hipStream_t s) { return exec(s); }); }
  int prepare_run(hipStream_t st) {
    if (!frag_done) { int rc = repack_frags(st); if (rc) return rc; }
    return tune_once(s_flush, st);
  }

  ~K22UNet() {
    if (film_all) (void)hipFree(film_all);
  }

  int run_ops_range(hipStream_t st, size_t lo, size_t hi) {
    for (size_t i = lo; i < hi && i < ops.size(); ++i) { int rc = ops[i](st); if (rc) return rc; }
    return K22_OK;
  }
  int run_ops(hipStream_t st) { return run_ops_range(st, 0, ops.size()); }

  void op_gn(OpList& L, const Act& in, const std::string& pfx, int64_t film_off,
             int act, int mode, int pad, Slot* dst, const GnLink* link = nullptr) {
    const int Bn = B, C = in.C(), HW = in.H * in.W;
    const int nsplit = gn_nsplit(Bn, HW);
    const bool fused = in.st0 != nullptr && (in.s1 == nullptr || in.st1 != nullptr);
    if (!fused) need(s_part, (size_t)Bn * nsplit * C * 2 * sizeof(float));
    need(s_coeff, (size_t)Bn * C * 2 * sizeof(float));
    const int Ho = mode == 1 ? in.H / 2 : (mode == 2 ? in.H * 2 : in.H);
    const int Wo = mode == 1 ? in.W / 2 : (mode == 2 ? in.W * 2 : in.W);
    need(dst, (size_t)Bn * (Ho + 2 * pad) * (Wo + 2 * pad) * C * esz);
    const float* gamma = Wf(pfx + ".weight");
    const float* beta = Wf(pfx + ".bias");
    const Act a = in;
    const int dt = sdt;
    const int x3 = k22_is_split(dtype) ? 1 : 0;
    const double gn_bytes = (double)Bn * HW * C * esz * (fused ? 1.0 : 2.0) + (double)Bn * (Ho + 2 * pad) * (Wo + 2 * pad) * C * esz;
    L.push_back(Op([=](hipStream_t st) {
      const void* x0 = ptr(a.s0);
      const void* x1 = a.s1 ? ptr(a.s1) : nullptr;
      GnCoeffParams cp = {};
      if (fused) {
        cp.src[0].st = ptr<float>(a.st0); cp.src[0].rpi = a.p0->rpi; cp.src[0].C = a.C0;
        if (a.s1) { cp.src[1].st = ptr<float>(a.st1); cp.src[1].rpi = a.p1->rpi; cp.src[1].C = a.C1; }
        if (cp.src[0].rpi <= 0 || (a.s1 && cp.src[1].rpi <= 0)) return k22_set_error(K22_EINVAL, "unet: producer delivered no GroupNorm partial sums");
      } else {
        GnStatsParams sp;
        sp.x0 = x0; sp.x1 = x1; sp.C0 = a.C0; sp.C1 = a.C1;
        sp.HW = HW; sp.B = Bn; sp.groups = 32; sp.nsplit = nsplit; sp.partial = ptr<float>(s_part);
        int rc = launch_gn_stats(sp, dt, st);
        if (rc) return rc;
        cp.src[0].st = ptr<float>(s_part); cp.src[0].rpi = nsplit; cp.src[0].C = C;
      }
      cp.HW = HW; cp.C = C; cp.groups = 32; cp.eps = 1e-5f;
      cp.gamma = gamma; cp.beta = beta;
      cp.film = film_off >= 0 ? film_base() + film_off : nullptr; cp.film_ld = film_total;
      cp.coeff = ptr<float>(s_coeff);
      GnApplyParams ap = {};
      ap.x0 = x0; ap.x1 = x1; ap.C0 = a.C0; ap.C1 = a.C1; ap.B = Bn; ap.H = a.H; ap.W = a.W;
      ap.mode = mode; ap.pad = pad; ap.act = act; ap.coeff = ptr<float>(s_coeff); ap.out = ptr(dst); ap.out_x3 = x3;
      int rc = launch_gn_coeff(cp, Bn, st);
      if (rc) return rc;
      if (link != nullptr && link->consumer != nullptr && conv3_algo_fuses_gn(link->consumer->cfg.algo)) return K22_OK;
      return launch_gn_apply(ap, dt, st);
    }, OP_GN, 0.0, gn_bytes, fused ? 2 : 3));
  }

  static void apply_cfg(IgemmParams& q, const Cfg& c) { tuned_apply_cfg(q, c); }
  int op_dt(const Tuned& t) const { return t.dt >= 0 ? t.dt : dtype; }
  void make_candidates(Tuned& t) { tuned_make_candidates(t, op_dt(t)); }
  void default_cfg(Tuned& t) { tuned_default_cfg(t, op_dt(t)); }
  void finish_cfg(Tuned& t) { tuned_finish_cfg(t, op_dt(t)); }
  size_t max_splitk_bytes(const Tuned& t) const { return tuned_max_splitk_bytes(t, autotune != 0); }
  int max_rpi(const Tuned& t) const { return tuned_max_rpi(t, op_dt(t), autotune != 0); }

  int x2_plan = 0;
  enum ConvRole { CONV_IN = 0, CONV_OUT = 1, CONV_HEAD = 2 };
  int conv_dt(int role, int Hc) const {
    if (dtype != K22_F16X2) return dtype;
    if (role == CONV_HEAD) return K22_F16X3;
    if (Hc >= H) return (x2_plan >> role) & 1 ? K22_F16X2 : K22_F16X3;
    return K22_F16X2;
  }
  int gemm_dt(bool qkv) const { return dtype == K22_F16X2 ? (qkv ? K22_F16X2 : K22_F16X3) : dtype; }

  Tuned* op_conv(OpList& L, int role, Slot* src, int Hc, int Wc, int Cin, int Cout,
                 const std::string& pfx, const Act* residual, Slot* dst, int out_mode, Slot* stats = nullptr,
                 const Act* skip_in = nullptr, const std::string& skip_pfx = std::string(), const Act* gn_in = nullptr, int gn_act = K22_ACT_NONE) {
    tuned.emplace_back();
    Tuned* t = &tuned.back();
    t->dt = conv_dt(role, Hc);
    IgemmParams& p = t->p;
    p.stages = -1;
    p.M = B * Hc * Wc; p.N = Cout; p.Npad = (Cout + 63) / 64 * 64; p.Kc = Cin; p.K0 = Cin; p.taps = 9;
    p.H = Hc; p.W = Wc; p.ldo = Cout; p.ldr = Cout; p.out_mode = out_mode; p.act = K22_ACT_NONE;
    p.Wp = W_(pfx + ".weight"); p.bias = Wf(pfx + ".bias");
    Act sk;
    if (skip_in) {
      sk = *skip_in;
      p.S0 = reinterpret_cast<const void*>(1); p.S1 = sk.s1 ? reinterpret_cast<const void*>(1) : nullptr;
      p.SK0 = sk.C0; p.SK1 = sk.C1;
      p.Ws = W_(skip_pfx + ".weight"); p.bias2 = Wf(skip_pfx + ".bias");
    }
    t->want_stats = stats != nullptr;
    Slot *wf = nullptr, *wsf = nullptr;
    if (stream_frag && k22_esz(dtype) == 2 && p.M <= 1152 && (stream_supported(p, dtype, 5) || stream_supported(p, dtype, 9))) {
      wf = new_slot();
      need(wf, stream_frag_bytes(p.Npad, 9, Cin, dtype));
      frag_jobs.push_back({p.Wp, wf, p.Npad, 9, Cin});
      p.Wfrag = reinterpret_cast<const void*>(1);
      if (skip_in) {
        wsf = new_slot();
        need(wsf, stream_frag_bytes(p.Npad, 1, p.SK0 + p.SK1, dtype));
        frag_jobs.push_back({p.Ws, wsf, p.Npad, 1, p.SK0 + p.SK1});
        p.Wsfrag = reinterpret_cast<const void*>(1);
      }
    }
    make_candidates(*t);
    default_cfg(*t);
    if (wf && t->cfg.algo != 20 && (t->from_table || !autotune)) {
      wf->bytes = 0; wf = nullptr;
      if (wsf) { wsf->bytes = 0; wsf = nullptr; frag_jobs.pop_back(); }
      frag_jobs.pop_back();
      p.Wfrag = nullptr; p.Wsfrag = nullptr;
      make_candidates(*t);
      default_cfg(*t);
    }
    need(s_splitk, max_splitk_bytes(*t));
    if (t->want_stats) need(stats, (size_t)B * max_rpi(*t) * Cout * 2 * sizeof(float));
    need(dst, out_mode == IG_OUT_ROWMAJOR ? (size_t)p.M * Cout * esz : (size_t)p.M * Cout * sizeof(float));
    Slot* rs = residual ? residual->s0 : nullptr;
    const int dt = t->dt;
    const bool gnf = gn_in != nullptr && fuse_gn;
    Act ga;
    if (gnf) ga = *gn_in;
    t->run = [=](hipStream_t st) {
      IgemmParams q = t->p;
      apply_cfg(q, t->cfg);
      q.A0 = ptr(src); q.residual = rs ? ptr(rs) : nullptr; q.out = ptr(dst); q.partial = ptr<float>(s_splitk);
      if (gnf && conv3_algo_fuses_gn(t->cfg.algo)) {
        q.gn_coeff = ptr<float>(s_coeff); q.gn_x0 = ptr(ga.s0); q.gn_x1 = ga.s1 ? ptr(ga.s1) : nullptr; q.gn_C0 = ga.C0; q.gn_act = gn_act;
      }
      q.stats = t->want_stats ? ptr<float>(stats) : nullptr;
      if (q.S0) { q.S0 = ptr(sk.s0); q.S1 = sk.s1 ? ptr(sk.s1) : nullptr; }
      q.Wfrag = wf ? ptr(wf) : nullptr; q.Wsfrag = wsf ? ptr(wsf) : nullptr;
      return launch_igemm(q, dt, st);
    };
    const double fl = 2.0 * p.M * (double)p.N * 9.0 * p.Kc;
    L.push_back(Op([=](hipStream_t st) { return t->run(st); }, OP_CONV3, fl, 0.0, 1));
    if (skip_in) L.back().flops2 = 2.0 * p.M * (double)p.N * (p.SK0 + p.SK1);
    return t;
  }

  Tuned* op_gemm(OpList& L, const Act& in, int M, int N, const std::string& pfx,
                 const Act* residual, Slot* dst, int ldo = 0, int out_mode = IG_OUT_ROWMAJOR, Slot* stats = nullptr, bool a_raw = false) {
    tuned.emplace_back();
    Tuned* t = &tuned.back();
    t->dt = gemm_dt(out_mode == IG_OUT_QKV);
    IgemmParams& p = t->p;
    p.stages = -1;
    p.M = M; p.N = N; p.Npad = (N + 63) / 64 * 64; p.Kc = in.C(); p.K0 = in.C0; p.taps = 1;
    p.lda0 = in.C0; p.lda1 = in.C1; p.ldo = ldo ? ldo : N; p.ldr = N; p.out_mode = out_mode;
    p.act = K22_ACT_NONE;
    if (in.H > 0 && in.W > 0 && M % (in.H * in.W) == 0 && M / (in.H * in.W) == B) { p.H = in.H; p.W = in.W; }
    if (out_mode == IG_OUT_QKV) p.att_T = in.H * in.W;
    p.Wp = W_(pfx + ".weight"); p.bias = Wf(pfx + ".bias");
    p.a_raw = (a_raw && k22_is_split(dtype)) ? 1 : 0;
    t->want_stats = stats != nullptr && p.H > 0;
    make_candidates(*t);
    if (t->want_stats && t->cands.empty()) { t->want_stats = false; make_candidates(*t); }
    default_cfg(*t);
    need(s_splitk, max_splitk_bytes(*t));
    if (t->want_stats) need(stats, (size_t)B * max_rpi(*t) * N * 2 * sizeof(float));
    need(dst, (size_t)M * p.ldo * esz);
    const Act a = in;
    Slot* rs = residual ? residual->s0 : nullptr;
    const int dt = t->dt;
    t->run = [=](hipStream_t st) {
      IgemmParams q = t->p;
      apply_cfg(q, t->cfg);
      q.A0 = ptr(a.s0); q.A1 = a.s1 ? ptr(a.s1) : nullptr;
      q.residual = rs ? ptr(rs) : nullptr; q.out = ptr(dst); q.partial = ptr<float>(s_splitk);
      if (t->aux0) { q.kall = ptr(reinterpret_cast<Slot*>(t->aux0)); q.vtall = ptr(reinterpret_cast<Slot*>(t->aux1)); }
      q.stats = t->want_stats ? ptr<float>(stats) : nullptr;
      return launch_igemm(q, dt, st);
    };
    L.push_back(Op([=](hipStream_t st) { return t->run(st); }, OP_GEMM, 2.0 * p.M * (double)p.N * p.Kc, 0.0, 1));
    return t;
  }

  Act resblock(const std::string& pfx, const Act& in, int Cout, int updown, int64_t& film_cursor, Slot* dst, Slot* dst_stats) {
    const int Cin = in.C();
    const int Ho = updown == 1 ? in.H / 2 : (updown == 2 ? in.H * 2 : in.H);
    const int Wo = updown == 1 ? in.W / 2 : (updown == 2 ? in.W * 2 : in.W);
    GnLink* l1 = nullptr;
    if (fuse_gn && updown == 0) { gn_links.emplace_back(); l1 = &gn_links.back(); }
    op_gn(ops, in, pfx + ".in_layers.0", -1, K22_ACT_SILU, updown, 1, s_P1, l1);
    Tuned* t1 = op_conv(ops, CONV_IN, s_P1, Ho, Wo, Cin, Cout, pfx + ".in_layers.2", nullptr, s_U1, IG_OUT_ROWMAJOR, s_U1st, nullptr, std::string(),
                        l1 ? &in : nullptr, K22_ACT_SILU);
    if (l1) l1->consumer = t1;
    Act u1; u1.s0 = s_U1; u1.C0 = Cout; u1.H = Ho; u1.W = Wo;
    if (t1->want_stats) { u1.p0 = t1; u1.st0 = s_U1st; }
    const int64_t film_off = film_cursor;
    film_cursor += 2 * Cout;
    GnLink* l2 = nullptr;
    if (fuse_gn) { gn_links.emplace_back(); l2 = &gn_links.back(); }
    op_gn(ops, u1, pfx + ".out_layers.0", film_off, K22_ACT_SILU, 0, 1, s_P2, l2);
    Act skip;
    skip.H = Ho; skip.W = Wo; skip.C0 = Cout;
    if (updown) {
      if (Cin != Cout || in.s1) { if (err.empty()) err = "updown ResBlock with channel change is not supported"; }
      need(s_S, (size_t)B * Ho * Wo * Cin * esz);
      const Act a = in; const int Bn = B, dt = sdt;
      ops.push_back([=](hipStream_t st) { return launch_resample(ptr(a.s0), ptr(s_S), Bn, a.H, a.W, Cin, updown, dt, st); });
      skip.s0 = s_S;
    } else if (Cin != Cout) {
      IgemmParams probe = {};
      probe.M = B * Ho * Wo; probe.N = Cout; probe.Npad = (Cout + 63) / 64 * 64; probe.Kc = Cout; probe.K0 = Cout; probe.taps = 9;
      probe.H = Ho; probe.W = Wo; probe.ldo = Cout; probe.ldr = Cout; probe.out_mode = IG_OUT_ROWMAJOR;
      probe.S0 = reinterpret_cast<const void*>(1); probe.S1 = in.s1 ? reinterpret_cast<const void*>(1) : nullptr;
      probe.SK0 = in.C0; probe.SK1 = in.C1; probe.Ws = reinterpret_cast<const void*>(1);
      if (fuse_skip && Cout >= 128 && (conv3_halo_supported(probe, dtype, 256) || conv3_halo_supported(probe, dtype, 128))) {
        Tuned* t2 = op_conv(ops, CONV_OUT, s_P2, Ho, Wo, Cout, Cout, pfx + ".out_layers.3", nullptr, dst, IG_OUT_ROWMAJOR, dst_stats,
                            &in, pfx + ".skip_connection", l2 ? &u1 : nullptr, K22_ACT_SILU);
        if (l2) l2->consumer = t2;
        Act out; out.s0 = dst; out.C0 = Cout; out.H = Ho; out.W = Wo;
        if (t2->want_stats) { out.p0 = t2; out.st0 = dst_stats; }
        return out;
      }
      op_gemm(ops, in, B * Ho * Wo, Cout, pfx + ".skip_connection", nullptr, s_S, 0, IG_OUT_ROWMAJOR, nullptr, true);
      skip.s0 = s_S;
    } else {
      if (in.s1) { if (err.empty()) err = "identity skip over a concat input"; }
      skip.s0 = in.s0;
    }
    Tuned* t2 = op_conv(ops, CONV_OUT, s_P2, Ho, Wo, Cout, Cout, pfx + ".out_layers.3", &skip, dst, IG_OUT_ROWMAJOR, dst_stats, nullptr, std::string(),
                        l2 ? &u1 : nullptr, K22_ACT_SILU);
    if (l2) l2->consumer = t2;
    Act out; out.s0 = dst; out.C0 = Cout; out.H = Ho; out.W = Wo;
    if (t2->want_stats) { out.p0 = t2; out.st0 = dst_stats; }
    return out;
  }

  Act attnblock(const std::string& pfx, const Act& in, Slot* dst, Slot* dst_stats = nullptr) {
    const int C = in.C0, T = in.H * in.W, Hh = C / 64, S = cfg.ctx_len;
    const int Tk = S + T, Tkp = (Tk + 63) / 64 * 64;
    n_attn++;
    op_gn(ops, in, pfx + ".norm", -1, K22_ACT_NONE, 0, 0, s_N);
    Act n; n.s0 = s_N; n.C0 = C; n.H = in.H; n.W = in.W;
    Slot* kall = new_slot((size_t)B * Hh * Tkp * 64 * esz);
    Slot* vtall = new_slot((size_t)B * Hh * Tkp * 64 * esz);
    Slot* ckv = new_slot((size_t)B * S * 2 * C * esz);
    s_ctxkv.push_back(ckv);
    const int Bn = B, dt = dtype, sd = sdt;
    {
      Act c; c.s0 = s_ctx; c.C0 = cfg.ctx_dim; c.H = 1; c.W = S;
      op_gemm(cond_ops, c, B * S, 2 * C, pfx + ".encoder_kv", nullptr, ckv, 0, IG_OUT_ROWMAJOR, nullptr, true);
      cond_ops.push_back(Op([=](hipStream_t st) {
        KvPackParams kp;
        kp.qkv = nullptr; kp.ctxkv = ptr(ckv); kp.kall = ptr(kall); kp.vtall = ptr(vtall);
        kp.B = Bn; kp.H = Hh; kp.T = 0; kp.S = S; kp.Tkp = Tkp;
        return launch_kv_pack(kp, sd, st);
      }));
    }
    need(s_QKV, (size_t)B * T * C * esz);
    {
      Tuned* t = op_gemm(ops, n, B * T, 3 * C, pfx + ".qkv", nullptr, s_QKV, C, IG_OUT_QKV);
      t->p.att_T = T; t->p.att_S = S; t->p.att_Tkp = Tkp;
      t->aux0 = kall; t->aux1 = vtall;
    }
    need(s_ATT, (size_t)B * T * C * esz);
    ops.push_back(Op([=](hipStream_t st) {
      AttentionParams ap = {};
      ap.q = ptr(s_QKV); ap.ldq = C; ap.kall = ptr(kall); ap.vtall = ptr(vtall); ap.out = ptr(s_ATT); ap.ldo = C;
      ap.B = Bn; ap.H = Hh; ap.T = T; ap.Tk = Tk; ap.Tkp = Tkp; ap.scale = 0.125f;
      ap.out_x3 = k22_is_split(dt) ? 1 : 0;
      return launch_attention(ap, dt, st);
    }, OP_ATTN, 4.0 * Bn * Hh * (double)T * Tk * 64.0, 0.0, 1));
    Act a; a.s0 = s_ATT; a.C0 = C; a.H = in.H; a.W = in.W;
    Tuned* tp = op_gemm(ops, a, B * T, C, pfx + ".proj_out", &in, dst, 0, IG_OUT_ROWMAJOR, dst_stats);
    Act out; out.s0 = dst; out.C0 = C; out.H = in.H; out.W = in.W;
    if (tp->want_stats) { out.p0 = tp; out.st0 = dst_stats; }
    return out;
  }

  bool has_attn(int ds) const {
    for (int i = 0; i < cfg.n_attention_ds; ++i) if (cfg.attention_ds[i] == ds) return true;
    return false;
  }

  int plan(int nB, int nH, int nW) {
    const int n_down = cfg.n_levels - 1;
    if (nB < 1 || nH < 1 || nW < 1) return k22_set_error(K22_EINVAL, "unet: B, H, W must be positive");
    if (nH % (1 << n_down) || nW % (1 << n_down)) return k22_set_error(K22_EINVAL, "unet: H, W must be divisible by 2^(levels-1)");
    if (nB > 8) return k22_set_error(K22_EINVAL, "unet: batch (2*bs) must be <= 8 per engine call");
    begin_plan();
    B = nB; H = nH; W = nW;
    gn_links.clear();
    ops.clear(); cond_ops.clear(); hint_ops.clear(); s_ctxkv.clear(); frag_jobs.clear(); frag_done = false; n_attn = 0;
    cond_set = false; hint_set = false;
    loop.drop();
    const int mc = cfg.model_channels, ted = 4 * mc;

    film_total = 0;
    {
      int ch = mc * cfg.channel_mult[0];
      for (int l = 0; l < cfg.n_levels; ++l) {
        for (int i = 0; i < cfg.num_res_blocks; ++i) { ch = mc * cfg.channel_mult[l]; film_total += 2 * ch; }
        if (l != cfg.n_levels - 1) film_total += 2 * ch;
      }
      film_total += 2 * 2 * ch;
      for (int l = cfg.n_levels - 1; l >= 0; --l)
        for (int i = 0; i <= cfg.num_res_blocks; ++i) {
          ch = mc * cfg.channel_mult[l];
          film_total += 2 * ch;
          if (l && i == cfg.num_res_blocks) film_total += 2 * ch;
        }
    }

    s_xin = new_slot((size_t)B * 4 * H * W * 4); s_img = new_slot((size_t)B * 4 * H * W * 4);
    s_mask = new_slot((size_t)B * H * W * 4); s_t = new_slot((size_t)B * 4 + 64);
    s_out = new_slot((size_t)B * cfg.out_channels * H * W * 4);
    s_temb = new_slot((size_t)B * mc * 4); s_e1 = new_slot((size_t)B * ted * 4); s_emb = new_slot((size_t)B * ted * 4);
    s_film = new_slot((size_t)B * film_total * 4); s_xfproj = new_slot((size_t)B * ted * 4);
    s_ctx = new_slot((size_t)B * cfg.ctx_len * cfg.ctx_dim * esz);
    const int ntext_p = cfg.ctx_len - cfg.n_image_embs;
    s_full = new_slot((size_t)B * (ntext_p > 0 ? ntext_p : 1) * cfg.text_dim1 * 4); s_pool = new_slot((size_t)B * cfg.text_dim2 * 4);
    s_imgemb = new_slot((size_t)B * cfg.image_dim * 4);
    s_tmpf = new_slot((size_t)B * cfg.n_image_embs * cfg.ctx_dim * 4 + (size_t)B * ted * 4);
    s_tmpf2 = new_slot((size_t)B * ted * 4);
    s_fullT = new_slot((size_t)B * (ntext_p > 0 ? ntext_p : 1) * cfg.text_dim1 * esz);
    s_ctxf = new_slot(cfg.head_type == 1 ? (size_t)B * cfg.ctx_len * cfg.ctx_dim * 4 : 0);
    if (cfg.hint_channels) {
      s_hint = new_slot((size_t)B * 4 * H * W * 4);
      s_hintin = new_slot((size_t)B * cfg.hint_channels * 64 * H * W * 4);
      for (int i = 0; i < 2; ++i) s_hbuf[i] = new_slot((size_t)B * 16 * 64 * H * W * 4);
    }
    s_part = new_slot(); s_coeff = new_slot(); s_P1 = new_slot(); s_U1 = new_slot(); s_P2 = new_slot(); s_S = new_slot();
    s_N = new_slot(); s_QKV = new_slot(); s_KALL = new_slot(); s_VT = new_slot(); s_ATT = new_slot();
    s_splitk = new_slot(256);
    s_U1st = new_slot();
    s_flush = new_slot(autotune ? ((size_t)320 << 20) : 0);
    for (int i = 0; i < 3; ++i) { s_h[i] = new_slot(); s_hst[i] = new_slot(); }
    int hrot = 0, hcur = 0;
    auto next_h = [&]() { hcur = hrot; hrot = (hrot + 1) % 3; return s_h[hcur]; };
    auto cur_hst = [&]() { return s_hst[hcur]; };

    if (cfg.head_type == 1) build_cond_ops_22(); else build_cond_ops();
    if (cfg.hint_channels) build_hint_ops();

    {
      tw.freqs = Wf("time_freqs");
      tw.w0 = Wf("time_embed.0.weight"); tw.b0 = Wf("time_embed.0.bias");
      tw.w2 = Wf("time_embed.2.weight"); tw.b2 = Wf("time_embed.2.bias");
      tw.we = W_("emb_layers.weight"); tw.be = Wf("emb_layers.bias");
      tw.mc = mc; tw.ted = ted; tw.dt = sdt;
      const int Bn = B;
      ops.push_back([=](hipStream_t st) {
        if (film_cur) return (int)K22_OK;
        return time_rows(ptr<float>(s_t), ptr<float>(s_temb), ptr<float>(s_e1), ptr<float>(s_emb), ptr<float>(s_film), Bn, st);
      });
    }

    int64_t film_cursor = 0;
    std::vector<Act> hs;
    int ch = mc * cfg.channel_mult[0];
    {
      Slot* d = new_slot((size_t)B * H * W * ch * esz);
      ConvInParams cp = {};
      cp.w = Wf("input_blocks.0.0.weight"); cp.bias = Wf("input_blocks.0.0.bias");
      cp.B = B; cp.H = H; cp.W = W; cp.Cin = cfg.in_channels; cp.Cout = ch;
      const int dt = sdt; const bool inpaint = cfg.in_channels == 9, hinted = cfg.in_channels == 8;
      const int premul = (hinted || cfg.head_type == 1) ? 1 : 0;
      ops.push_back([=](hipStream_t st) {
        ConvInParams q = cp;
        q.x = ptr<float>(s_xin); q.img = inpaint ? ptr<float>(s_img) : (hinted ? ptr<float>(s_hint) : nullptr);
        q.mask = inpaint ? ptr<float>(s_mask) : nullptr; q.img_premul = premul;
        q.out = ptr(d);
        return launch_conv_in(q, dt, st);
      });
      Act a; a.s0 = d; a.C0 = ch; a.H = H; a.W = W;
      hs.push_back(a);
    }
    Act h = hs.back();
    int ds = 1, blk = 1;
    for (int l = 0; l < cfg.n_levels; ++l) {
      for (int i = 0; i < cfg.num_res_blocks; ++i) {
        const int co = mc * cfg.channel_mult[l];
        const std::string pfx = "input_blocks." + std::to_string(blk);
        Slot* d = new_slot();
        if (has_attn(ds)) {
          Slot* rd = next_h();
          Act r = resblock(pfx + ".0", h, co, 0, film_cursor, rd, cur_hst());
          h = attnblock(pfx + ".1", r, d, new_slot());
        } else {
          h = resblock(pfx + ".0", h, co, 0, film_cursor, d, new_slot());
        }
        ch = co; hs.push_back(h); ++blk;
      }
      if (l != cfg.n_levels - 1) {
        const std::string pfx = "input_blocks." + std::to_string(blk);
        Slot* d = new_slot();
        h = resblock(pfx + ".0", h, ch, 1, film_cursor, d, new_slot());
        hs.push_back(h); ++blk; ds *= 2;
      }
    }
    {
      Slot* d0 = next_h(); Slot* st0 = cur_hst();
      Act r = resblock("middle_block.0", h, ch, 0, film_cursor, d0, st0);
      Slot* da = next_h(); Slot* sta = cur_hst();
      Act a = attnblock("middle_block.1", r, da, sta);
      Slot* d2 = next_h(); Slot* st2 = cur_hst();
      h = resblock("middle_block.2", a, ch, 0, film_cursor, d2, st2);
    }
    blk = 0;
    for (int l = cfg.n_levels - 1; l >= 0; --l) {
      for (int i = 0; i <= cfg.num_res_blocks; ++i) {
        const Act skip = hs.back(); hs.pop_back();
        Act cat; cat.s0 = h.s0; cat.C0 = h.C0; cat.s1 = skip.s0; cat.C1 = skip.C0; cat.H = h.H; cat.W = h.W;
        cat.p0 = h.p0; cat.st0 = h.st0; cat.p1 = skip.p0; cat.st1 = skip.st0;
        if (skip.H != h.H || skip.W != h.W) return k22_set_error(K22_EINVAL, "unet: skip shape mismatch");
        const int co = mc * cfg.channel_mult[l];
        const std::string pfx = "output_blocks." + std::to_string(blk);
        { Slot* d = next_h(); Slot* dst_st = cur_hst(); h = resblock(pfx + ".0", cat, co, 0, film_cursor, d, dst_st); }
        int sub = 1;
        if (has_attn(ds)) { Slot* da = next_h(); Slot* sta = cur_hst(); h = attnblock(pfx + "." + std::to_string(sub), h, da, sta); ++sub; }
        if (l && i == cfg.num_res_blocks) {
          { Slot* d = next_h(); Slot* dst_st = cur_hst(); h = resblock(pfx + "." + std::to_string(sub), h, co, 2, film_cursor, d, dst_st); }
          ds /= 2;
        }
        ch = co; ++blk;
      }
    }
    if (film_cursor != film_total) return k22_set_error(K22_EINVAL, "unet: internal FiLM width mismatch");
    op_gn(ops, h, "out.0", -1, K22_ACT_SILU, 0, 1, s_P1);
    op_conv(ops, CONV_HEAD, s_P1, H, W, ch, cfg.out_channels, "out.2", nullptr, s_out, IG_OUT_NCHW_F32);

    return finish_plan();
  }

  void build_cond_ops_22() {
    const int mc = cfg.model_channels, ted = 4 * mc, Bn = B, dt = sdt;
    const int cd = cfg.ctx_dim, S = cfg.ctx_len, di = cfg.image_dim;
    const float* w_cp = Wf("head22.ctx_proj.weight"); const float* b_cp = Wf("head22.ctx_proj.bias");
    const float* g_cn = Wf("head22.ctx_norm.weight"); const float* b_cn = Wf("head22.ctx_norm.bias");
    const float* w_ep = Wf("head22.emb_proj.weight"); const float* b_ep = Wf("head22.emb_proj.bias");
    const float* g_en = Wf("head22.emb_norm.weight"); const float* b_en = Wf("head22.emb_norm.bias");
    cond_ops.push_back([=](hipStream_t st) {
      float* proj = ptr<float>(s_tmpf);
      float* embp = ptr<float>(s_tmpf) + (size_t)Bn * S * cd;
      LinearSmallParams lp = {};
      lp.x = ptr<float>(s_imgemb); lp.ldx = di; lp.W = w_cp; lp.bias = b_cp; lp.out = proj; lp.ldo = S * cd;
      lp.M = Bn; lp.N = S * cd; lp.K = di;
      int rc = launch_linear_smallm(lp, K22_F32, st);
      if (rc) return rc;
      rc = launch_layernorm_f32(proj, g_cn, b_cn, ptr<float>(s_ctxf), Bn * S, cd, 1e-5f, st);
      if (rc) return rc;
      rc = launch_cast_rows(ptr<float>(s_ctxf), ptr(s_ctx), Bn * S, cd, cd, cd, dt, st);
      if (rc) return rc;
      lp.W = w_ep; lp.bias = b_ep; lp.out = embp; lp.ldo = ted; lp.N = ted;
      rc = launch_linear_smallm(lp, K22_F32, st);
      if (rc) return rc;
      return launch_layernorm_f32(embp, g_en, b_en, ptr<float>(s_xfproj), Bn, ted, 1e-5f, st);
    });
  }

  void build_hint_ops() {
    static const int chans[9] = {0, 16, 16, 32, 32, 96, 96, 256, 4};
    static const int strides[8] = {1, 1, 2, 1, 2, 1, 2, 1};
    int hin = 8 * H, win = 8 * W, cin = cfg.hint_channels;
    for (int k = 0; k < 8; ++k) {
      const float* w = Wf("hint." + std::to_string(k) + ".weight");
      const float* b = Wf("hint." + std::to_string(k) + ".bias");
      const int cout = chans[k + 1], stride = strides[k], Bn = B, ci = cin, hi = hin, wi = win;
      Slot* src = k == 0 ? s_hintin : s_hbuf[(k - 1) & 1];
      Slot* dst = k == 7 ? s_hint : s_hbuf[k & 1];
      hint_ops.push_back([=](hipStream_t st) {
        ConvDirectParams q = {};
        q.x = ptr<float>(src); q.w = w; q.bias = b; q.y = ptr<float>(dst);
        q.B = Bn; q.Cin = ci; q.Cout = cout; q.Hin = hi; q.Win = wi; q.stride = stride; q.act = k == 7 ? K22_ACT_NONE : K22_ACT_SILU;
        return launch_conv3x3_direct(q, st);
      });
      cin = cout;
      if (stride == 2) { hin = (hin - 1) / 2 + 1; win = (win - 1) / 2 + 1; }
    }
  }

  void build_cond_ops() {
    const int mc = cfg.model_channels, ted = 4 * mc, Bn = B, dt = sdt;
    const int nie = cfg.n_image_embs, cd = cfg.ctx_dim, S = cfg.ctx_len, ntext = S - nie;
    const float* w_cs = Wf("clip_to_seq.weight"); const float* b_cs = Wf("clip_to_seq.bias");
    const float* w_pn = Wf("proj_n.weight"); const float* b_pn = Wf("proj_n.bias");
    const float* g_ln = Wf("ln_model_n.weight"); const float* b_ln = Wf("ln_model_n.bias");
    const float* w_il = Wf("img_layer.weight"); const float* b_il = Wf("img_layer.bias");
    const int d1 = cfg.text_dim1, d2 = cfg.text_dim2, di = cfg.image_dim;
    cond_ops.push_back([=](hipStream_t st) {
      float* clipseq = ptr<float>(s_tmpf);
      float* proj = ptr<float>(s_tmpf) + (size_t)Bn * nie * cd;
      LinearSmallParams lp = {};
      lp.x = ptr<float>(s_imgemb); lp.ldx = di; lp.W = w_cs; lp.bias = b_cs; lp.out = clipseq; lp.ldo = nie * cd;
      lp.M = Bn; lp.N = nie * cd; lp.K = di;
      int rc = launch_linear_smallm(lp, K22_F32, st);
      if (rc) return rc;
      for (int b = 0; b < Bn; ++b) {
        rc = launch_cast_rows(clipseq + (size_t)b * nie * cd, ptr(s_ctx) + (size_t)b * S * cd * esz, nie, cd, cd, cd, dt, st);
        if (rc) return rc;
      }
      lp.x = ptr<float>(s_pool); lp.ldx = d2; lp.W = w_pn; lp.bias = b_pn; lp.out = proj; lp.ldo = ted; lp.N = ted; lp.K = d2;
      rc = launch_linear_smallm(lp, K22_F32, st);
      if (rc) return rc;
      rc = launch_layernorm_f32(proj, g_ln, b_ln, ptr<float>(s_tmpf2), Bn, ted, 1e-5f, st);
      if (rc) return rc;
      lp.x = ptr<float>(s_imgemb); lp.ldx = di; lp.W = w_il; lp.bias = b_il; lp.add = ptr<float>(s_tmpf2); lp.ld_add = ted;
      lp.out = ptr<float>(s_xfproj); lp.ldo = ted; lp.N = ted; lp.K = di;
      rc = launch_linear_smallm(lp, K22_F32, st);
      if (rc) return rc;
      return launch_cast_rows(ptr<float>(s_full), ptr(s_fullT), Bn * ntext, d1, d1, d1, dt, st);
    });
    {
      IgemmParams p = {};
    p.stages = -1;
      p.M = ntext; p.N = cd; p.Npad = (cd + 63) / 64 * 64; p.Kc = d1; p.K0 = d1; p.taps = 1; p.lda0 = d1; p.ldo = cd;
      p.out_mode = IG_OUT_ROWMAJOR; p.splitk = 1;
      p.a_raw = k22_is_split(dtype) ? 1 : 0;
      p.Wp = W_("to_model_dim_n.weight"); p.bias = Wf("to_model_dim_n.bias");
      const size_t es = esz;
      const int gdt = gemm_dt(false);
      cond_ops.push_back([=](hipStream_t st) {
        for (int b = 0; b < Bn; ++b) {
          IgemmParams q = p;
          q.A0 = ptr(s_fullT) + (size_t)b * ntext * d1 * es;
          q.out = ptr(s_ctx) + ((size_t)b * S + nie) * cd * es;
          int rc = launch_igemm(q, gdt, st);
          if (rc) return rc;
        }
        return K22_OK;
      });
    }
  }
};

extern "C" {

int k22_unet_create(const K22UNetConfig* cfg, const K22Weight* weights, int n_weights, K22UNet** out) {
  if (!cfg || !out) return k22_set_error(K22_EINVAL, "unet_create: null argument");
  if (!k22_dtype_ok(cfg->dtype) && !k22_is_split(cfg->dtype)) return k22_set_error(K22_EINVAL, "unet_create: dtype");
  if (cfg->num_head_channels != 64) return k22_set_error(K22_EINVAL, "unet_create: only num_head_channels == 64");
  if (cfg->model_channels % 128) return k22_set_error(K22_EINVAL, "unet_create: model_channels % 128");
  if (cfg->n_levels < 1 || cfg->n_levels > 8) return k22_set_error(K22_EINVAL, "unet_create: n_levels");
  if (cfg->in_channels != 4 && cfg->in_channels != 9 && cfg->in_channels != 8) return k22_set_error(K22_EINVAL, "unet_create: in_channels must be 4, 8 or 9");
  if (cfg->head_type != 0 && cfg->head_type != 1) return k22_set_error(K22_EINVAL, "unet_create: head_type must be 0 (2.1) or 1 (2.2)");
  if ((cfg->hint_channels != 0) != (cfg->in_channels == 8) || (cfg->hint_channels != 0 && cfg->hint_channels != 3))
    return k22_set_error(K22_EINVAL, "unet_create: hint_channels = 3 goes with in_channels = 8 (latent + hint latent), else 0");
  if (cfg->head_type == 1 && cfg->n_image_embs != cfg->ctx_len) return k22_set_error(K22_EINVAL, "unet_create: the 2.2 head has image tokens only (n_image_embs == ctx_len)");
  K22UNet* u = new K22UNet();
  u->cfg = *cfg; u->set_dtype(cfg->dtype); u->sdt = k22_storage_dtype(cfg->dtype);
  u->stream_frag = env_flag("K22_STREAM", 1);
  u->fuse_gn = env_flag("K22_FUSE_GN", 0);
  u->fuse_skip = env_flag("K22_FUSE_SKIP", 1);
  u->hoist_time = env_flag("K22_HOIST_TIME", 1);
  const char* xp = getenv("K22_X2_PLAN");
  u->x2_plan = xp ? (atoi(xp) & 3) : 0;
  u->set_weights(weights, n_weights);
  *out = u;
  return K22_OK;
}

void k22_unet_destroy(K22UNet* u) { delete u; }

int k22_unet_plan(K22UNet* u, int B, int H, int W, size_t* workspace_bytes) {
  if (!u || !workspace_bytes) return k22_set_error(K22_EINVAL, "unet_plan: null argument");
  int rc = u->plan(B, H, W);
  if (rc) return rc;
  *workspace_bytes = u->ws_bytes;
  return K22_OK;
}

int k22_unet_bind(K22UNet* u, void* workspace, size_t workspace_bytes) {
  if (!u) return k22_set_error(K22_EINVAL, "unet_bind: null argument");
  if (int rc = u->bind(workspace, workspace_bytes, "unet_bind")) return rc;
  u->cond_set = false; u->hint_set = false; u->frag_done = false;
  u->loop.drop();
  return K22_OK;
}

int k22_unet_set_condition(K22UNet* u, const float* full_emb, const float* pooled_emb, const float* image_emb, void* stream) {
  if (!u || !u->ws) return k22_set_error(K22_EINVAL, "unet_set_condition: bind a workspace first");
  hipStream_t st = reinterpret_cast<hipStream_t>(stream);
  const K22UNetConfig& c = u->cfg;
  const int ntext = c.ctx_len - c.n_image_embs;
  if (!image_emb) return k22_set_error(K22_EINVAL, "unet_set_condition: image_emb is required");
  if (c.head_type == 0 && (!full_emb || !pooled_emb)) return k22_set_error(K22_EINVAL, "unet_set_condition: the 2.1 head needs full_emb and pooled_emb");
  const size_t pb = (size_t)u->B;
  if (c.head_type == 0) {
    if (int rc = copy_d2d(u->ptr(u->s_full), full_emb, pb * ntext * c.text_dim1 * 4, st)) return rc;
    if (int rc = copy_d2d(u->ptr(u->s_pool), pooled_emb, pb * c.text_dim2 * 4, st)) return rc;
  }
  if (int rc = copy_d2d(u->ptr(u->s_imgemb), image_emb, pb * c.image_dim * 4, st)) return rc;
  for (auto& op : u->cond_ops) { int rc = op(st); if (rc) return rc; }
  u->cond_set = true;
  return K22_OK;
}

int k22_unet_set_hint(K22UNet* u, const float* hint, void* stream) {
  if (!u || !u->ws) return k22_set_error(K22_EINVAL, "unet_set_hint: bind a workspace first");
  if (!u->cfg.hint_channels) return k22_set_error(K22_EINVAL, "unet_set_hint: this UNet has no hint input (hint_channels == 0)");
  if (!hint) return k22_set_error(K22_EINVAL, "unet_set_hint: null hint");
  hipStream_t st = reinterpret_cast<hipStream_t>(stream);
  const size_t per = (size_t)u->B * u->cfg.hint_channels * 64 * u->H * u->W;
  if (int rc = copy_d2d(u->ptr(u->s_hintin), hint, per * 4, st)) return rc;
  for (auto& op : u->hint_ops) { int rc = op(st); if (rc) return rc; }
  u->hint_set = true;
  return K22_OK;
}

int k22_unet_forward(K22UNet* u, const float* x, const float* timesteps, const float* inpaint_image,
                     const float* inpaint_mask, float* out, int use_graph, void* stream) {
  if (!u || !u->ws) return k22_set_error(K22_EINVAL, "unet_forward: bind a workspace first");
  if (!u->cond_set) return k22_set_error(K22_EINVAL, "unet_forward: call k22_unet_set_condition first");
  if (u->cfg.in_channels == 9 && (!inpaint_image || !inpaint_mask)) return k22_set_error(K22_EINVAL, "unet_forward: inpainting UNet needs inpaint_image and inpaint_mask");
  if (u->cfg.hint_channels && !u->hint_set) return k22_set_error(K22_EINVAL, "unet_forward: call k22_unet_set_hint first");
  hipStream_t st = reinterpret_cast<hipStream_t>(stream);
  const size_t hw = (size_t)u->H * u->W;
  const size_t pb = (size_t)u->B;
  if (int rc = copy_d2d(u->ptr(u->s_xin), x, pb * 4 * hw * 4, st)) return rc;
  if (int rc = copy_d2d(u->ptr(u->s_t), timesteps, pb * 4, st)) return rc;
  if (u->cfg.in_channels == 9) {
    if (int rc = copy_d2d(u->ptr(u->s_img), inpaint_image, pb * 4 * hw * 4, st)) return rc;
    if (int rc = copy_d2d(u->ptr(u->s_mask), inpaint_mask, pb * hw * 4, st)) return rc;
  }
  { int rc = u->prepare_run(st); if (rc) return rc; }
  const int rc = use_graph ? u->replay(u->graph, st, [u](hipStream_t s) { return u->exec(s); }) : u->exec_eager(st);
  if (rc) return rc;
  return copy_d2d(out, u->ptr(u->s_out), pb * u->cfg.out_channels * hw * 4, st);
}

int k22_unet_sample_loop(K22UNet* u, float* x, float* x_tmp, const float* timesteps, const float* noise_seq, const float* init_img,
                         const float* mask, const float* inpaint_image, const float* inpaint_mask, const float* table,
                         const int* table_rows, int n_steps, float guidance, float clamp_lo, float clamp_hi, int pct_index,
                         double pct_gamma, void* scratch, int use_graph, void* stream) {
  if (!u || !u->ws) return k22_set_error(K22_EINVAL, "unet_sample_loop: bind a workspace first");
  if (!u->cond_set) return k22_set_error(K22_EINVAL, "unet_sample_loop: call k22_unet_set_condition first");
  if (!x || !x_tmp || !timesteps || !noise_seq || !table || !table_rows || !scratch || n_steps < 1)
    return k22_set_error(K22_EINVAL, "unet_sample_loop: null argument");
  if (u->B % 2) return k22_set_error(K22_EINVAL, "unet_sample_loop: the batch is the CFG batch [cond | uncond] (even)");
  if (u->cfg.out_channels != 8) return k22_set_error(K22_EINVAL, "unet_sample_loop: the UNet must predict eps and variance (8 channels)");
  if (u->cfg.in_channels == 9 && (!inpaint_image || !inpaint_mask)) return k22_set_error(K22_EINVAL, "unet_sample_loop: inpainting UNet needs inpaint_image and inpaint_mask");
  if (u->cfg.hint_channels && !u->hint_set) return k22_set_error(K22_EINVAL, "unet_sample_loop: call k22_unet_set_hint first");
  const int B = u->B, HW = u->H * u->W;
  if (pct_index >= 4 * HW) return k22_set_error(K22_EINVAL, "unet_sample_loop: percentile index out of range");
  hipStream_t st = reinterpret_cast<hipStream_t>(stream);
  hipError_t e;
  { int rc = u->prepare_run(st); if (rc) return rc; }
  const size_t half = (size_t)(B / 2) * 4 * HW * sizeof(float);
  const size_t pb = (size_t)B;
  const bool hoist = B <= 8 && u->hoist_time;
  const int64_t rows_all = (int64_t)n_steps * B;
  float *fa_film = nullptr, *fa_temb = nullptr, *fa_e1 = nullptr, *fa_emb = nullptr;
  if (hoist) {
    const size_t need = (size_t)rows_all * (size_t)(u->film_total + u->tw.mc + 2 * u->tw.ted) * sizeof(float);
    if (need > u->film_all_bytes) {
      u->loop.drop();
      if (u->film_all) { (void)hipStreamSynchronize(st); (void)hipFree(u->film_all); u->film_all = nullptr; u->film_all_bytes = 0; }
      e = hipMalloc(reinterpret_cast<void**>(&u->film_all), need);
      if (e != hipSuccess) { u->film_all = nullptr; return k22_set_error_hip(e, __FILE__, __LINE__); }
      u->film_all_bytes = need;
    }
    fa_film = u->film_all;
    fa_temb = fa_film + rows_all * u->film_total;
    fa_e1 = fa_temb + rows_all * u->tw.mc;
    fa_emb = fa_e1 + rows_all * u->tw.ted;
  }
  auto run_loop_body = [&](hipStream_t s) -> int {
    if (hoist) {
      const int spl = 8 / B;
      for (int k0 = 0; k0 < n_steps; k0 += spl) {
        const int rows = (n_steps - k0 < spl ? n_steps - k0 : spl) * B;
        const int64_t r0 = (int64_t)k0 * B;
        const int rc = u->time_rows(timesteps + r0, fa_temb + r0 * u->tw.mc, fa_e1 + r0 * u->tw.ted, fa_emb + r0 * u->tw.ted, fa_film + r0 * u->film_total, rows, s);
        if (rc) return rc;
      }
    }
    if (u->cfg.in_channels == 9) {
      if (int rc = copy_d2d(u->ptr(u->s_img), inpaint_image, pb * 4 * HW * 4, s)) return rc;
      if (int rc = copy_d2d(u->ptr(u->s_mask), inpaint_mask, pb * HW * 4, s)) return rc;
    }
    float* cur = x; float* nxt = x_tmp;
    for (int k = 0; k < n_steps; ++k) {
      if (int rc = copy_d2d(u->ptr(u->s_xin), cur, half, s)) return rc;
      if (int rc = copy_d2d(u->ptr(u->s_xin) + half, cur, half, s)) return rc;
      if (hoist) {
        u->film_cur = fa_film + (int64_t)k * B * u->film_total;
      } else {
        if (int rc = copy_d2d(u->ptr(u->s_t), timesteps + (size_t)k * B, (size_t)B * 4, s)) return rc;
      }
      int rc = u->exec(s);
      if (rc) return rc;
      SamplerParams p = {};
      p.x = cur; p.model_out = u->model_out(); p.noise = noise_seq + (size_t)k * B * 4 * HW; p.init_img = init_img; p.mask = mask;
      p.table = table; p.step = nullptr; p.step_host = table_rows[k]; p.guidance = guidance; p.clamp_lo = clamp_lo; p.clamp_hi = clamp_hi;
      p.use_cfg = 1; p.n_lo = pct_index; p.gamma = pct_gamma;
      p.s_buf = reinterpret_cast<float*>(scratch); p.x0_buf = reinterpret_cast<float*>(scratch) + 64;
      p.x_out = nxt; p.x0_out = nullptr; p.N = B; p.HW = HW;
      rc = launch_sampler_step(p, s);
      if (rc) return rc;
      float* t_ = cur; cur = nxt; nxt = t_;
    }
    if (cur != x) return copy_d2d(x, cur, (size_t)B * 4 * HW * sizeof(float), s);
    return K22_OK;
  };
  auto run_loop = [&](hipStream_t s) -> int { const int rc = run_loop_body(s); u->film_cur = nullptr; return rc; };
  if (!use_graph) return run_loop(st);
  std::vector<unsigned long long> key = {(unsigned long long)(uintptr_t)x, (unsigned long long)(uintptr_t)x_tmp, (unsigned long long)(uintptr_t)timesteps,
      (unsigned long long)(uintptr_t)noise_seq, (unsigned long long)(uintptr_t)init_img, (unsigned long long)(uintptr_t)mask,
      (unsigned long long)(uintptr_t)inpaint_image, (unsigned long long)(uintptr_t)inpaint_mask, (unsigned long long)(uintptr_t)table,
      (unsigned long long)(uintptr_t)scratch, (unsigned long long)n_steps, (unsigned long long)pct_index, (unsigned long long)(hoist ? 1 : 0)};
  auto bits = [](double v) { unsigned long long b; memcpy(&b, &v, 8); return b; };
  key.push_back(bits(guidance)); key.push_back(bits(clamp_lo)); key.push_back(bits(clamp_hi)); key.push_back(bits(pct_gamma));
  for (int k = 0; k < n_steps; ++k) key.push_back((unsigned long long)table_rows[k]);
  if (!u->loop || key != u->loop_key) {
    if (!u->warmed) {
      e = hipMemsetAsync(u->ptr(u->s_xin), 0, pb * 4 * HW * 4, st);
      if (e != hipSuccess) return k22_set_error_hip(e, __FILE__, __LINE__);
      if (int rc = copy_d2d(u->ptr(u->s_t), timesteps, pb * 4, st)) return rc;
      if (u->cfg.in_channels == 9) {
        if (int rc = copy_d2d(u->ptr(u->s_img), inpaint_image, pb * 4 * HW * 4, st)) return rc;
        if (int rc = copy_d2d(u->ptr(u->s_mask), inpaint_mask, pb * HW * 4, st)) return rc;
      }
      int rc = u->exec_eager(st);
      if (rc) return rc;
      e = hipStreamSynchronize(st);
      if (e != hipSuccess) return k22_set_error_hip(e, __FILE__, __LINE__);
    }
    if (int rc = u->loop.capture(u->cap, run_loop)) return rc;
    u->loop_key = key;
  }
  return u->loop.launch(st);
}

int k22_unet_num_ops(const K22UNet* u) {
  return u && u->planned ? (int)u->ops.size() : 0;
}

int k22_unet_set_autotune(K22UNet* u, int on) {
  if (!u) return k22_set_error(K22_EINVAL, "unet_set_autotune: null handle");
  if (u->planned && (on != 0) != (u->autotune != 0)) return k22_set_error(K22_EINVAL, "unet_set_autotune: call before k22_unet_plan");
  u->autotune = on ? 1 : 0;
  return K22_OK;
}

int k22_unet_tuning_report(const K22UNet* u, char* buf, size_t cap) {
  if (!u || !buf || cap == 0) return k22_set_error(K22_EINVAL, "unet_tuning_report: null argument");
  const std::string out = tuning_report_text(u->tuned);
  snprintf(buf, cap, "%s", out.c_str());
  return K22_OK;
}

int k22_unet_profile(K22UNet* u, int reps, double* ms, double* flops, double* bytes, int* launches, void* stream) {
  if (!u || !u->ws || !u->cond_set) return k22_set_error(K22_EINVAL, "unet_profile: run k22_unet_forward once first");
  if (reps < 1) reps = 1;
  hipStream_t st = reinterpret_cast<hipStream_t>(stream);
  for (int k = 0; k < OP_NKINDS; ++k) { ms[k] = 0.0; flops[k] = 0.0; bytes[k] = 0.0; launches[k] = 0; }
  int rc = K22_OK;
  {
    K22UNet* q = u;
    if (!q->frag_done) { int rc0 = q->repack_frags(st); if (rc0) return rc0; }
    const size_t n = q->ops.size();
    std::vector<hipEvent_t> ev(2 * n);
    for (auto& e : ev) { hipError_t r = hipEventCreate(&e); if (r != hipSuccess) return k22_set_error_hip(r, __FILE__, __LINE__); }
    for (size_t i = 0; i < n; ++i) {
      flops[q->ops[i].kind] += q->ops[i].flops + q->ops[i].flops2;
      bytes[q->ops[i].kind] += q->ops[i].bytes;
      launches[q->ops[i].kind] += q->ops[i].kernels;
    }
    for (int r = 0; r < reps && rc == K22_OK; ++r) {
      for (size_t i = 0; i < n; ++i) {
        (void)hipEventRecord(ev[2 * i], st);
        rc = q->ops[i](st);
        (void)hipEventRecord(ev[2 * i + 1], st);
        if (rc) break;
      }
      hipError_t e = hipStreamSynchronize(st);
      if (e != hipSuccess) { rc = k22_set_error_hip(e, __FILE__, __LINE__); break; }
      for (size_t i = 0; i < n; ++i) {
        float t = 0.f;
        (void)hipEventElapsedTime(&t, ev[2 * i], ev[2 * i + 1]);
        ms[q->ops[i].kind] += (double)t / reps;
      }
    }
    for (auto& e : ev) (void)hipEventDestroy(e);
  }
  return rc;
}

}
```

### kandinsky-2_amd/csrc/sampler.hip

```cpp
#include "kernels.h"
#include "elementwise.h"

__device__ __forceinline__ const float* step_row(const SamplerParams& p) {
  const int st = p.step ? *p.step : p.step_host;
  return p.table + (int64_t)st * 8;
}

__device__ __forceinline__ float guided_eps(const SamplerParams& p, int n, int c, int pix) {
  const int64_t hw = p.HW;
  if (!p.use_cfg) return p.model_out[((int64_t)n * 8 + c) * hw + pix];
  const int bs = p.N / 2, i = n % bs;
  const float ce = p.model_out[((int64_t)i * 8 + c) * hw + pix];
  const float ue = p.model_out[((int64_t)(i + bs) * 8 + c) * hw + pix];
  return ue + p.guidance * (ce - ue);
}

__global__ __launch_bounds__(256) void sampler_x0_kernel(SamplerParams p) {
  const float* tr = step_row(p);
  const float sr = tr[0], srm1 = tr[1];
  const int64_t total = (int64_t)p.N * 4 * p.HW;
  for (int64_t i = (int64_t)blockIdx.x * 256 + threadIdx.x; i < total; i += (int64_t)gridDim.x * 256) {
    const int pix = (int)(i % p.HW);
    const int c = (int)((i / p.HW) % 4), n = (int)(i / (4 * (int64_t)p.HW));
    const float eps = guided_eps(p, n, c, pix);
    float x0 = __fsub_rn(__fmul_rn(sr, p.x[i]), __fmul_rn(srm1, eps));
    x0 = fminf(fmaxf(x0, p.clamp_lo), p.clamp_hi);
    if (p.mask != nullptr) {
      const float mk = p.mask[(int64_t)n * p.HW + pix];
      x0 = __fadd_rn(__fmul_rn(x0, 1.f - mk), __fmul_rn(p.init_img[i], mk));
    }
    p.x0_buf[i] = x0;
  }
}

__device__ __forceinline__ void hist_add_aggregated(int* hist, bool valid, uint32_t bin) {
  uint64_t todo = __ballot(valid);
  const int lane = threadIdx.x & 63;
  for (int round = 0; round < 4 && todo; ++round) {
    const int leader = __ffsll((unsigned long long)todo) - 1;
    const uint32_t lb = (uint32_t)__builtin_amdgcn_readlane((int)bin, leader);
    const uint64_t same = __ballot(valid && bin == lb) & todo;
    if (lane == leader) atomicAdd(&hist[lb], __popcll(same));
    todo &= ~same;
  }
  if ((todo >> lane) & 1) atomicAdd(&hist[bin], 1);
}

constexpr int K22_RS_BINS = 2048;
template <int KPT>
__device__ __forceinline__ uint32_t radix_select(const float* v, const uint32_t* keys, int n, int k, int* hist, uint32_t* bc, uint32_t floor_key = 0u) {
  const int tid = threadIdx.x;
  uint32_t prefix = 0, mask = 0;
#pragma unroll 1
  for (int pass = 0; pass < 3; ++pass) {
    const int shift = pass == 0 ? 21 : (pass == 1 ? 10 : 0);
    const int nb = pass == 2 ? 1024 : 2048;
    const uint32_t dmask = (uint32_t)(nb - 1);
    for (int i = tid; i < K22_RS_BINS; i += blockDim.x) hist[i] = 0;
    __syncthreads();
    if constexpr (KPT > 0) {
#pragma unroll
      for (int j = 0; j < KPT; ++j) {
        const uint32_t key = keys[j];
        const bool valid = key != 0xffffffffu && (key & mask) == prefix && key >= floor_key;
        hist_add_aggregated(hist, valid, (key >> shift) & dmask);
      }
    } else {
      for (int i0 = 0; i0 < n; i0 += blockDim.x) {
        const int i = i0 + tid;
        uint32_t key = 0;
        bool valid = false;
        if (i < n) {
          key = __float_as_uint(fabsf(v[i]));
          valid = (key & mask) == prefix;
        }
        hist_add_aggregated(hist, valid, (key >> shift) & dmask);
      }
    }
    __syncthreads();
    if (tid < 64) {
      const int per = nb >> 6;
      int run = 0;
      for (int j = 0; j < per; ++j) run += hist[tid * per + j];
      int incl = run;
#pragma unroll
      for (int o = 1; o < 64; o <<= 1) {
        const int t = __shfl_up(incl, o, 64);
        if (tid >= o) incl += t;
      }
      const int excl = incl - run;
      if (k >= excl && k < incl) {
        int acc = excl;
        for (int j = 0; j < per; ++j) {
          const int c = hist[tid * per + j];
          if (k < acc + c) { bc[0] = (uint32_t)(tid * per + j); bc[1] = (uint32_t)(k - acc); break; }
          acc += c;
        }
      }
    }
    __syncthreads();
    prefix |= bc[0] << shift;
    mask |= dmask << shift;
    k = (int)bc[1];
    __syncthreads();
  }
  return prefix;
}

template <int KPT>
__global__ __launch_bounds__(1024) void sampler_threshold_kernel(SamplerParams p) {
  __shared__ int hist[K22_RS_BINS];
  __shared__ uint32_t bc[2];
  __shared__ unsigned int succ_cnt[2];
  const int n = 4 * p.HW;
  const int k_hi = p.n_lo + 1 < n ? p.n_lo + 1 : n - 1;
  uint32_t keys[KPT > 0 ? KPT : 1];
  if constexpr (KPT > 0) {
#pragma unroll
    for (int j = 0; j < KPT; ++j) {
      const int i = j * 1024 + (int)threadIdx.x;
      keys[j] = i < n ? __float_as_uint(fabsf(p.x0_buf[i])) : 0xffffffffu;
    }
  }
  uint32_t floor_key = 0u;
  int k_sel = p.n_lo;
  if constexpr (KPT >= 16) {
    __shared__ unsigned int n_ge;
    uint32_t skey = 0xffffffffu;
    const int js = (int)threadIdx.x % KPT;
#pragma unroll
    for (int j = 0; j < KPT; ++j) skey = (j == js) ? keys[j] : skey;
    unsigned int ns_local = skey != 0xffffffffu ? 1u : 0u;
    if (threadIdx.x == 0) n_ge = 0u;
    __syncthreads();
    if (ns_local) atomicAdd(&n_ge, 1u);
    __syncthreads();
    const int ns = (int)n_ge;
    __syncthreads();
    if (ns >= 512) {
      const uint32_t pivot = radix_select<1>(nullptr, &skey, ns, (int)(ns * 0.973f), hist, bc);
      if (threadIdx.x == 0) n_ge = 0u;
      __syncthreads();
      unsigned int c = 0;
#pragma unroll
      for (int j = 0; j < KPT; ++j) c += (keys[j] != 0xffffffffu && keys[j] >= pivot) ? 1u : 0u;
#pragma unroll
      for (int o = 32; o > 0; o >>= 1) c += __shfl_xor(c, o, 64);
      if ((threadIdx.x & 63) == 0) atomicAdd(&n_ge, c);
      __syncthreads();
      const int below = n - (int)n_ge;
      if (p.n_lo >= below) { floor_key = pivot; k_sel = p.n_lo - below; }
      __syncthreads();
    }
  }
  const uint32_t ka = radix_select<KPT>(p.x0_buf, keys, n, k_sel, hist, bc, floor_key);
  if (threadIdx.x == 0) { succ_cnt[0] = 0u; succ_cnt[1] = 0xffffffffu; }
  __syncthreads();
  unsigned int cnt = 0, mn = 0xffffffffu;
  if constexpr (KPT > 0) {
#pragma unroll
    for (int j = 0; j < KPT; ++j) {
      const uint32_t key = keys[j];
      if (key == 0xffffffffu) continue;
      if (key <= ka) ++cnt;
      else mn = key < mn ? key : mn;
    }
  } else {
    for (int i = threadIdx.x; i < n; i += blockDim.x) {
      const uint32_t key = __float_as_uint(fabsf(p.x0_buf[i]));
      if (key <= ka) ++cnt;
      else mn = key < mn ? key : mn;
    }
  }
#pragma unroll
  for (int o = 32; o > 0; o >>= 1) {
    cnt += __shfl_xor(cnt, o, 64);
    const unsigned int t = __shfl_xor(mn, o, 64);
    mn = t < mn ? t : mn;
  }
  if ((threadIdx.x & 63) == 0) { atomicAdd(&succ_cnt[0], cnt); atomicMin(&succ_cnt[1], mn); }
  __syncthreads();
  if (threadIdx.x == 0) {
    const uint32_t kb = ((int)succ_cnt[0] > k_hi || k_hi == p.n_lo) ? ka : succ_cnt[1];
    const float a = __uint_as_float(ka), b = __uint_as_float(kb);
    const float t = (float)p.gamma;
    const float d = __fsub_rn(b, a);
    float r = __fadd_rn(a, __fmul_rn(d, t));
    if (t >= 0.5f) r = __fsub_rn(b, __fmul_rn(d, __fsub_rn(1.f, t)));
    p.s_buf[0] = r > 1.f ? r : 1.f;
  }
}

__global__ __launch_bounds__(256) void sampler_final_kernel(SamplerParams p) {
  const float* tr = step_row(p);
  const float c1 = tr[2], c2 = tr[3], min_log = tr[4], max_log = tr[5], nonzero = tr[6];
  const float s = (p.n_lo >= 0) ? p.s_buf[0] : 0.f;
  const int64_t total = (int64_t)p.N * 4 * p.HW;
  for (int64_t i = (int64_t)blockIdx.x * 256 + threadIdx.x; i < total; i += (int64_t)gridDim.x * 256) {
    const int pix = (int)(i % p.HW);
    const int c = (int)((i / p.HW) % 4), n = (int)(i / (4 * (int64_t)p.HW));
    float x0 = p.x0_buf[i];
    if (p.n_lo >= 0) x0 = fminf(fmaxf(x0, -s), s) / s;
    const float mean = __fadd_rn(__fmul_rn(c1, x0), __fmul_rn(c2, p.x[i]));
    const float v = p.model_out[((int64_t)n * 8 + 4 + c) * p.HW + pix];
    const float frac = (v + 1.f) / 2.f;
    const float logvar = __fadd_rn(__fmul_rn(frac, max_log), __fmul_rn(1.f - frac, min_log));
    p.x_out[i] = mean + nonzero * expf(0.5f * logvar) * p.noise[i];
    if (p.x0_out != nullptr) p.x0_out[i] = x0;
  }
}

__global__ __launch_bounds__(256) void ddim_step_kernel(const float* x, const float* model_out, const float* noise, const float* tab,
                                                        float guidance, int use_cfg, float* x_out, float* x0_out, int N, int HW) {
  const float a_t = tab[0], a_prev = tab[1], sigma = tab[2], s1m = tab[3];
  const float sq_at = sqrtf(a_t), sq_ap = sqrtf(a_prev);
  const float dirc = sqrtf(__fsub_rn(__fsub_rn(1.0f, a_prev), __fmul_rn(sigma, sigma)));
  const int64_t total = (int64_t)N * 4 * HW;
  for (int64_t i = (int64_t)blockIdx.x * 256 + threadIdx.x; i < total; i += (int64_t)gridDim.x * 256) {
    const int pix = (int)(i % HW);
    const int c = (int)((i / HW) % 4), n = (int)(i / (4 * (int64_t)HW));
    float e;
    if (use_cfg) {
      const int bs = N / 2, j = n % bs;
      const float ce = model_out[((int64_t)j * 8 + c) * HW + pix], ue = model_out[((int64_t)(j + bs) * 8 + c) * HW + pix];
      e = ue + guidance * (ce - ue);
    } else {
      e = model_out[((int64_t)n * 8 + c) * HW + pix];
    }
    const float x0 = __fdiv_rn(__fsub_rn(x[i], __fmul_rn(s1m, e)), sq_at);
    float xp = __fadd_rn(__fmul_rn(sq_ap, x0), __fmul_rn(dirc, e));
    if (noise != nullptr) xp = __fadd_rn(xp, __fmul_rn(sigma, noise[i]));
    x_out[i] = xp;
    if (x0_out != nullptr) x0_out[i] = x0;
  }
}

__global__ __launch_bounds__(256) void plms_step_kernel(const float* x, const float* model_out, const float* h1, const float* h2, const float* h3,
                                                        int order, const float* tab, float guidance, int use_cfg, float* x_out, float* e_store,
                                                        float* x0_out, int N, int HW) {
  const float a_t = tab[0], a_prev = tab[1], s1m = tab[3];
  const float sq_at = sqrtf(a_t), sq_ap = sqrtf(a_prev);
  const float dirc = sqrtf(__fsub_rn(__fsub_rn(1.0f, a_prev), 0.0f));
  const int64_t total = (int64_t)N * 4 * HW;
  for (int64_t i = (int64_t)blockIdx.x * 256 + threadIdx.x; i < total; i += (int64_t)gridDim.x * 256) {
    const int pix = (int)(i % HW);
    const int c = (int)((i / HW) % 4), n = (int)(i / (4 * (int64_t)HW));
    float e;
    if (use_cfg) {
      const int bs = N / 2, j = n % bs;
      const float ce = model_out[((int64_t)j * 8 + c) * HW + pix], ue = model_out[((int64_t)(j + bs) * 8 + c) * HW + pix];
      e = __fadd_rn(ue, __fmul_rn(guidance, __fsub_rn(ce, ue)));
    } else {
      e = model_out[((int64_t)n * 8 + c) * HW + pix];
    }
    float ep = e;
    if (order == 4) ep = __fdiv_rn(__fadd_rn(h1[i], e), 2.0f);
    else if (order == 1) ep = __fdiv_rn(__fsub_rn(__fmul_rn(3.0f, e), h1[i]), 2.0f);
    else if (order == 2) ep = __fdiv_rn(__fadd_rn(__fsub_rn(__fmul_rn(23.0f, e), __fmul_rn(16.0f, h1[i])), __fmul_rn(5.0f, h2[i])), 12.0f);
    else if (order == 3)
      ep = __fdiv_rn(__fsub_rn(__fadd_rn(__fsub_rn(__fmul_rn(55.0f, e), __fmul_rn(59.0f, h1[i])), __fmul_rn(37.0f, h2[i])), __fmul_rn(9.0f, h3[i])), 24.0f);
    const float x0 = __fdiv_rn(__fsub_rn(x[i], __fmul_rn(s1m, ep)), sq_at);
    x_out[i] = __fadd_rn(__fmul_rn(sq_ap, x0), __fmul_rn(dirc, ep));
    if (e_store != nullptr) e_store[i] = e;
    if (x0_out != nullptr) x0_out[i] = x0;
  }
}

int launch_plms_step(const float* x, const float* model_out, const float* h1, const float* h2, const float* h3, int order, const float* tab,
                     float guidance, int use_cfg, float* x_out, float* e_store, float* x0_out, int N, int HW, hipStream_t s) {
  if (N <= 0 || HW <= 0 || (use_cfg && (N & 1))) return k22_set_error(K22_EINVAL, "plms_step: bad batch");
  if (order < 0 || order > 4 || ((order == 1 || order == 4) && !h1) || (order == 2 && (!h1 || !h2)) || (order == 3 && (!h1 || !h2 || !h3)))
    return k22_set_error(K22_EINVAL, "plms_step: order 0-4 with the eps history it needs");
  const int64_t total = (int64_t)N * 4 * HW;
  int nb = (int)((total + 255) / 256);
  if (nb > 2048) nb = 2048;
  hipLaunchKernelGGL(plms_step_kernel, dim3(nb), dim3(256), 0, s, x, model_out, h1, h2, h3, order, tab, guidance, use_cfg, x_out, e_store, x0_out, N, HW);
  K22_CHECK_LAUNCH();
  return K22_OK;
}

__global__ __launch_bounds__(256) void prepare_mask_kernel(const float* old_mask, float* out, int C, int H, int W) {
  const int i = blockIdx.x * 256 + threadIdx.x;
  if (i >= H * W) return;
  const int y = i / W, x = i - y * W;
  const int sy[6] = {y + 1, y, y + 1, y - 1, y, y - 1};
  const int sx[6] = {x, x + 1, x + 1, x, x - 1, x - 1};
  bool kill = false;
#pragma unroll
  for (int k = 0; k < 6; ++k)
    if (sy[k] >= 0 && sy[k] < H && sx[k] >= 0 && sx[k] < W && old_mask[sy[k] * W + sx[k]] != 1.0f) kill = true;
  for (int c = 0; c < C; ++c) out[(c * H + y) * W + x] = kill ? 0.0f : old_mask[(c * H + y) * W + x];
}

int launch_prepare_mask(const float* old_mask, float* out, int C, int H, int W, hipStream_t s) {
  if (C < 1 || H < 1 || W < 1 || old_mask == out) return k22_set_error(K22_EINVAL, "prepare_mask: bad arguments (out of place only)");
  hipLaunchKernelGGL(prepare_mask_kernel, dim3((H * W + 255) / 256), dim3(256), 0, s, old_mask, out, C, H, W);
  K22_CHECK_LAUNCH();
  return K22_OK;
}

int launch_ddim_step(const float* x, const float* model_out, const float* noise, const float* tab, float guidance, int use_cfg,
                     float* x_out, float* x0_out, int N, int HW, hipStream_t s) {
  if (N <= 0 || HW <= 0 || (use_cfg && (N & 1))) return k22_set_error(K22_EINVAL, "ddim_step: bad batch");
  const int64_t total = (int64_t)N * 4 * HW;
  int nb = (int)((total + 255) / 256);
  if (nb > 2048) nb = 2048;
  hipLaunchKernelGGL(ddim_step_kernel, dim3(nb), dim3(256), 0, s, x, model_out, noise, tab, guidance, use_cfg, x_out, x0_out, N, HW);
  K22_CHECK_LAUNCH();
  return K22_OK;
}

__global__ void step_advance_kernel(int* step, int delta) { *step += delta; }

int launch_sampler_step(const SamplerParams& p, hipStream_t s) {
  if (p.N <= 0 || p.HW <= 0) return k22_set_error(K22_EINVAL, "sampler: empty batch");
  if (p.use_cfg && (p.N & 1)) return k22_set_error(K22_EINVAL, "sampler: CFG needs an even batch [cond | uncond]");
  if ((p.mask == nullptr) != (p.init_img == nullptr)) return k22_set_error(K22_EINVAL, "sampler: init_img and mask go together");
  const int64_t total = (int64_t)p.N * 4 * p.HW;
  int nb = (int)((total + 255) / 256);
  if (nb > 2048) nb = 2048;
  hipLaunchKernelGGL(sampler_x0_kernel, dim3(nb), dim3(256), 0, s, p);
  K22_CHECK_LAUNCH();
  if (p.n_lo >= 0) {
    const int kpt = (4 * p.HW + 1023) / 1024;
    if (kpt <= 4) hipLaunchKernelGGL(sampler_threshold_kernel<4>, dim3(1), dim3(1024), 0, s, p);
    else if (kpt <= 16) hipLaunchKernelGGL(sampler_threshold_kernel<16>, dim3(1), dim3(1024), 0, s, p);
    else if (kpt <= 36) hipLaunchKernelGGL(sampler_threshold_kernel<36>, dim3(1), dim3(1024), 0, s, p);
    else if (kpt <= 64) hipLaunchKernelGGL(sampler_threshold_kernel<64>, dim3(1), dim3(1024), 0, s, p);
    else hipLaunchKernelGGL(sampler_threshold_kernel<0>, dim3(1), dim3(1024), 0, s, p);
    K22_CHECK_LAUNCH();
  }
  hipLaunchKernelGGL(sampler_final_kernel, dim3(nb), dim3(256), 0, s, p);
  K22_CHECK_LAUNCH();
  return K22_OK;
}

int launch_step_advance(int* step, int delta, hipStream_t s) {
  hipLaunchKernelGGL(step_advance_kernel, dim3(1), dim3(1), 0, s, step, delta);
  K22_CHECK_LAUNCH();
  return K22_OK;
}
```

Before: 148.3 steps/s.

## Add lean tail: fused GN-resample raw output, row conv_in with GN stats, histogram-seeded sampler threshold

This adds a default-on 'lean_tail' mode that bundles several independent changes. GroupNorm-apply now also writes the raw resampled tensor, replacing a separate resample pass. A new row-based conv_in kernel emits GroupNorm partial sums, so the stats pass can be skipped, and it supports a modulo batch index so the CFG halves share one latent. The sampler x0 kernel now builds per-block first-pass histograms, which lets the single-block threshold kernel skip its first radix pass. Together these target small serial tail kernels and redundant memory passes, at the cost of more code paths, more scratch memory and a risk to parity.

```diff
diff --git a/include/k22.h b/include/k22.h
--- a/include/k22.h
+++ b/include/k22.h
@@ -146,6 +146,11 @@
                   const float* beta, const float* film, long film_ld, float eps, int act, int mode, int pad,
                   void* scratch, void* out, int dtype, void* stream);
 size_t k22_groupnorm_scratch_bytes(int B, int C);
+int k22_groupnorm_resample(const void* x, int C, int B, int H, int W, const float* gamma, const float* beta, float eps, int act, int mode,
+                           int pad, void* scratch, void* out, void* raw_out, int dtype, void* stream);
+int k22_conv_in_stats_rows(int H);
+int k22_conv_in(const float* x, const float* img, const float* mask, const float* w, const float* bias, void* out, float* stats,
+                int B, int H, int W, int Cin, int Cout, int img_premul, int x_mod, int dtype, void* stream);
 int k22_attention(const void* qkv, const void* ctxkv, void* kall, void* vtall, void* out, int B, int H, int T, int S,
                   int dtype, void* stream);
 int k22_qkv_project(const void* x, const void* Wp, const float* bias, void* q_out, void* kall, void* vtall,
diff --git a/kandinsky-2_amd/_lib.py b/kandinsky-2_amd/_lib.py
--- a/kandinsky-2_amd/_lib.py
+++ b/kandinsky-2_amd/_lib.py
@@ -120,6 +120,9 @@
     "k22_blend_noised": (_I, [_P, _P, _P, _P, _F, _F, _P, _I, _I, _I, _I, _P]),
     "k22_prepare_mask": (_I, [_P, _P, _I, _I, _I, _P]),
     "k22_plms_step": (_I, [_P, _P, _P, _P, _P, _I, _P, _F, _I, _P, _P, _P, _I, _I, _P]),
+    "k22_groupnorm_resample": (_I, [_P, _I, _I, _I, _I, _P, _P, _F, _I, _I, _I, _P, _P, _P, _I, _P]),
+    "k22_conv_in_stats_rows": (_I, [_I]),
+    "k22_conv_in": (_I, [_P, _P, _P, _P, _P, _P, _P, _I, _I, _I, _I, _I, _I, _I, _I, _P]),
     "k22_sampler_scratch_bytes": (_Z, [_I, _I]),
     "k22_sampler_step": (_I, [_P, _P, _P, _P, _P, _P, _I, _F, _I, _F, _F, _I, _D, _P, _P, _P, _I, _I, _P]),
     "k22_gemm": (_I, [_P, _P, _P, _P, _P, _P, _P, _I, _I, _I, _I, _I, _L, _L, _I, _I, _I, _I, _I, _I, _I, _I, _P]),
diff --git a/kandinsky-2_amd/csrc/capi.hip b/kandinsky-2_amd/csrc/capi.hip
--- a/kandinsky-2_amd/csrc/capi.hip
+++ b/kandinsky-2_amd/csrc/capi.hip
@@ -17,6 +17,10 @@
   snprintf(g_err, sizeof(g_err), "HIP error %d (%s) at %s:%d", (int)e, hipGetErrorString(e), file, line);
   return K22_EHIP;
 }
+
+static int g_lean_tail = 1;
+int k22_lean_tail() { return g_lean_tail; }
+void k22_set_lean_tail(int on) { g_lean_tail = on ? 1 : 0; }
 
 extern "C" {
 
@@ -33,6 +37,7 @@
 }
 
 int k22_set_option(const char* name, int value) {
+  if (name && !strcmp(name, "lean_tail")) { k22_set_lean_tail(value); return K22_OK; }
   if (name && !strcmp(name, "igemm_stages")) { igemm_set_default_stages(value); return K22_OK; }
   if (name && !strcmp(name, "igemm_xcd_remap")) { igemm_set_xcd_remap(value); return K22_OK; }
   if (name && !strcmp(name, "conv_algo")) { igemm_set_conv_algo(value); return K22_OK; }
@@ -324,6 +329,36 @@
   return launch_gn_apply(ap, dtype, st);
 }
 
+int k22_groupnorm_resample(const void* x, int C, int B, int H, int W, const float* gamma, const float* beta, float eps, int act, int mode,
+                           int pad, void* scratch, void* out, void* raw_out, int dtype, void* stream) {
+  hipStream_t st = reinterpret_cast<hipStream_t>(stream);
+  if (!x || !out || !raw_out || !scratch) return k22_set_error(K22_EINVAL, "groupnorm_resample: null argument");
+  if (mode != 1 && mode != 2) return k22_set_error(K22_EINVAL, "groupnorm_resample: mode must be 1 (avgpool2) or 2 (nearest-up2)");
+  const int out_x3 = k22_is_split(dtype) ? 1 : 0;
+  dtype = k22_storage_dtype(dtype);
+  float* partial = reinterpret_cast<float*>(scratch);
+  float* coeff = partial + (size_t)B * 128 * C * 2;
+  const int rc = launch_gn_stats_coeff(x, nullptr, C, 0, B, H * W, eps, gamma, beta, nullptr, 0, partial, coeff, dtype, st);
+  if (rc) return rc;
+  const int lean = k22_lean_tail();
+  GnApplyParams ap = {};
+  ap.x0 = x; ap.C0 = C; ap.B = B; ap.H = H; ap.W = W; ap.mode = mode; ap.pad = pad; ap.act = act;
+  ap.coeff = coeff; ap.out = out; ap.out_x3 = out_x3; ap.raw_out = lean ? raw_out : nullptr;
+  if (int rc2 = launch_gn_apply(ap, dtype, st)) return rc2;
+  return lean ? (int)K22_OK : launch_resample(x, raw_out, B, H, W, C, mode, dtype, st);
+}
+
+int k22_conv_in_stats_rows(int H) { return conv_in_rpi(H); }
+int k22_conv_in(const float* x, const float* img, const float* mask, const float* w, const float* bias, void* out, float* stats,
+                int B, int H, int W, int Cin, int Cout, int img_premul, int x_mod, int dtype, void* stream) {
+  if (!x || !w || !bias || !out) return k22_set_error(K22_EINVAL, "conv_in: null argument");
+  if ((Cin == 9 && (!img || !mask)) || (Cin == 8 && !img)) return k22_set_error(K22_EINVAL, "conv_in: img / mask missing");
+  ConvInParams p = {};
+  p.x = x; p.img = img; p.mask = mask; p.w = w; p.bias = bias; p.out = out; p.B = B; p.H = H; p.W = W; p.Cin = Cin; p.Cout = Cout;
+  p.img_premul = img_premul; p.x_mod = x_mod; p.rows = k22_lean_tail(); p.stats = stats;
+  return launch_conv_in(p, k22_storage_dtype(dtype), reinterpret_cast<hipStream_t>(stream));
+}
+
 int k22_conv3x3_gn(const void* x0, const void* x1, int C0, int C1, const float* gamma, const float* beta, const float* film, long film_ld,
                    float eps, int act, void* scratch, const void* Wp, const float* bias, const void* residual, void* out, void* partial,
                    int B, int H, int W, int Cout, int Npad, int splitk, int bm, int algo, int dtype, void* stream) {
@@ -450,7 +485,7 @@
                           reinterpret_cast<hipStream_t>(stream));
 }
 
-size_t k22_sampler_scratch_bytes(int N, int HW) { return (size_t)N * 4 * HW * sizeof(float) + 256; }
+size_t k22_sampler_scratch_bytes(int N, int HW) { return (size_t)N * 4 * HW * sizeof(float) + 256 + sampler_hist_bytes(HW); }
 
 int k22_sampler_step(const float* x, const float* model_out, const float* noise, const float* init_img,
                      const float* mask, const float* table, int step_index, float guidance, int use_cfg,
@@ -462,7 +497,7 @@
   p.use_cfg = use_cfg; p.n_lo = pct_index; p.gamma = pct_gamma;
   p.s_buf = reinterpret_cast<float*>(scratch);
   p.x0_buf = reinterpret_cast<float*>(scratch) + 64;
-  p.x_out = x_out; p.x0_out = x0_out; p.N = N; p.HW = HW;
+  p.x_out = x_out; p.x0_out = x0_out; p.N = N; p.HW = HW; p.lean = k22_lean_tail();
   if (pct_index >= 4 * HW) return k22_set_error(K22_EINVAL, "sampler: percentile index out of range");
   return launch_sampler_step(p, reinterpret_cast<hipStream_t>(stream));
 }
diff --git a/kandinsky-2_amd/csrc/elementwise.h b/kandinsky-2_amd/csrc/elementwise.h
--- a/kandinsky-2_amd/csrc/elementwise.h
+++ b/kandinsky-2_amd/csrc/elementwise.h
@@ -23,6 +23,7 @@
   const float* coeff;
   void* out;
   int out_x3;
+  void* raw_out;
 };
 struct ConvInParams {
   const float* x; const float* img; const float* mask;
@@ -30,7 +31,13 @@
   void* out;
   int B, H, W, Cin, Cout;
   int img_premul;
+  int x_mod;
+  int rows;
+  float* stats;
 };
+inline int conv_in_rpi(int H) { const int rpw = (H + 127) / 128; return (H + rpw - 1) / rpw; }
+inline size_t conv_in_rows_lds_bytes(int Cin, int W, int Cout) { return ((size_t)Cin * 3 * (W + 2) + 2 * (size_t)Cout) * sizeof(float); }
+inline bool conv_in_rows_supported(int Cin, int W, int Cout) { return Cout % 64 == 0 && Cout <= 768 && conv_in_rows_lds_bytes(Cin, W, Cout) <= 60 * 1024; }
 struct ConvDirectParams {
   const float* x; const float* w; const float* bias; float* y;
   int B, Cin, Cout, Hin, Win, stride, act;
@@ -88,7 +95,16 @@
   float* x_out;
   float* x0_out;
   int N, HW;
+  int lean;
 };
+constexpr int K22_SAMPLER_EPB = 1024;
+inline size_t sampler_hist_bytes(int HW) {
+  const long n = 4L * HW;
+  if (n > 64 * 1024) return 0;
+  return (size_t)((n + K22_SAMPLER_EPB - 1) / K22_SAMPLER_EPB) * 1024 * sizeof(int);
+}
+int k22_lean_tail();
+void k22_set_lean_tail(int on);
 
 int launch_x3_pack(const float* in, void* out, int64_t n, float scale, hipStream_t s);
 int gn_nsplit(int B, int HW);
diff --git a/kandinsky-2_amd/csrc/elementwise.hip b/kandinsky-2_amd/csrc/elementwise.hip
--- a/kandinsky-2_amd/csrc/elementwise.hip
+++ b/kandinsky-2_amd/csrc/elementwise.hip
@@ -206,10 +206,24 @@
         for (int q = 0; q < 4; ++q) acc += fast ? apply_act_sel<true>(v[q].get(k) * A[k] + Bc[k], p.act) : apply_act_sel<false>(v[q].get(k) * A[k] + Bc[k], p.act);
         r[k] = acc * 0.25f;
       }
+      if (p.raw_out != nullptr) {
+        float s[EPV];
+#pragma unroll
+        for (int k = 0; k < EPV; ++k) {
+          s[k] = 0.f;
+#pragma unroll
+          for (int q = 0; q < 4; ++q) s[k] += v[q].get(k);
+        }
+        Vec16<T> ro;
+#pragma unroll
+        for (int k = 0; k < EPV / 2; ++k) ro.set2(k, s[2 * k] * 0.25f, s[2 * k + 1] * 0.25f);
+        *reinterpret_cast<decltype(ro.raw)*>(reinterpret_cast<T*>(p.raw_out) + (((int64_t)b * Ho + yo) * Wo + xo) * C + c) = ro.raw;
+      }
     } else {
       const int yi = p.mode == 2 ? yo >> 1 : yo, xi = p.mode == 2 ? xo >> 1 : xo;
       Vec16<T> v;
       v.raw = *reinterpret_cast<const decltype(v.raw)*>(src + ((int64_t)(b * p.H + yi) * p.W + xi) * ld + cs);
+      if (p.raw_out != nullptr) *reinterpret_cast<decltype(v.raw)*>(reinterpret_cast<T*>(p.raw_out) + (((int64_t)b * Ho + yo) * Wo + xo) * C + c) = v.raw;
 #pragma unroll
       for (int k = 0; k < EPV; ++k) r[k] = fast ? apply_act_sel<true>(v.get(k) * A[k] + Bc[k], p.act) : apply_act_sel<false>(v.get(k) * A[k] + Bc[k], p.act);
     }
@@ -268,13 +282,14 @@
   const int xt = blockIdx.x, y = blockIdx.y, b = blockIdx.z;
   const int x0 = xt * PT;
   const int hw = p.H * p.W;
+  const int bx = p.x_mod > 0 ? b % p.x_mod : b;
   for (int i = tid; i < CIN * 3 * PW; i += 128) {
     const int c = i / (3 * PW), r = (i / PW) % 3, xx = i % PW;
     const int yy = y + r - 1, xs = x0 + xx - 1;
     float v = 0.f;
     if (yy >= 0 && yy < p.H && xs >= 0 && xs < p.W) {
       const int64_t o = (int64_t)yy * p.W + xs;
-      if (c < 4) v = p.x[((int64_t)b * 4 + c) * hw + o];
+      if (c < 4) v = p.x[((int64_t)bx * 4 + c) * hw + o];
       else if (c < 8) v = p.img[((int64_t)b * 4 + (c - 4)) * hw + o] * (p.img_premul ? 1.f : p.mask[(int64_t)b * hw + o]);
       else v = p.mask[(int64_t)b * hw + o];
     }
@@ -297,6 +312,66 @@
           for (int q = 0; q < 3; ++q) acc += w[c * 9 + r * 3 + q] * patch[c][r][px + q];
       out[((int64_t)(b * p.H + y) * p.W + x0 + px) * p.Cout + n] = from_f32<T>(acc);
     }
+  }
+}
+
+template <typename T, int CIN>
+__global__ __launch_bounds__(768) void conv_in_rows_kernel(ConvInParams p, int rows_per_wg, int halves) {
+  extern __shared__ float cin_lds[];
+  const int PW = p.W + 2;
+  float* patch = cin_lds;
+  float* red = cin_lds + CIN * 3 * PW;
+  const int tid = threadIdx.x, nthr = blockDim.x;
+  const int b = blockIdx.y, bx = p.x_mod > 0 ? b % p.x_mod : b;
+  const int y0 = blockIdx.x * rows_per_wg, y1 = min(p.H, y0 + rows_per_wg);
+  const int hw = p.H * p.W;
+  const int n = tid % p.Cout, half = tid / p.Cout;
+  const int wh = (p.W + halves - 1) / halves;
+  const int px0 = half * wh, px1 = min(p.W, px0 + wh);
+  constexpr int UNR = CIN <= 4 ? 4 : 2;
+  float w[CIN * 9];
+#pragma unroll
+  for (int k = 0; k < CIN * 9; ++k) w[k] = p.w[(int64_t)k * p.Cout + n];
+  const float bias = p.bias[n];
+  T* out = reinterpret_cast<T*>(p.out);
+  float ssum = 0.f, ssq = 0.f;
+  for (int y = y0; y < y1; ++y) {
+    __syncthreads();
+    for (int i = tid; i < CIN * 3 * PW; i += nthr) {
+      const int c = i / (3 * PW), r = (i / PW) % 3, xx = i % PW;
+      const int yy = y + r - 1, xs = xx - 1;
+      float v = 0.f;
+      if (yy >= 0 && yy < p.H && xs >= 0 && xs < p.W) {
+        const int64_t o = (int64_t)yy * p.W + xs;
+        if (c < 4) v = p.x[((int64_t)bx * 4 + c) * hw + o];
+        else if (c < 8) v = p.img[((int64_t)b * 4 + (c - 4)) * hw + o] * (p.img_premul ? 1.f : p.mask[(int64_t)b * hw + o]);
+        else v = p.mask[(int64_t)b * hw + o];
+      }
+      patch[i] = v;
+    }
+    __syncthreads();
+    T* orow = out + ((int64_t)(b * p.H + y) * p.W) * p.Cout + n;
+#pragma unroll UNR
+    for (int px = px0; px < px1; ++px) {
+      float acc = bias;
+#pragma unroll
+      for (int c = 0; c < CIN; ++c)
+#pragma unroll
+        for (int r = 0; r < 3; ++r)
+#pragma unroll
+          for (int q = 0; q < 3; ++q) acc += w[c * 9 + r * 3 + q] * patch[(c * 3 + r) * PW + px + q];
+      const T o = from_f32<T>(acc);
+      orow[(int64_t)px * p.Cout] = o;
+      const float f = to_f32(o);
+      ssum += f; ssq += f * f;
+    }
+  }
+  if (p.stats == nullptr) return;
+  if (half == 1) { red[2 * n] = ssum; red[2 * n + 1] = ssq; }
+  __syncthreads();
+  if (half == 0) {
+    if (halves == 2) { ssum += red[2 * n]; ssq += red[2 * n + 1]; }
+    *reinterpret_cast<float2*>(p.stats + (((int64_t)b * gridDim.x + blockIdx.x) * p.Cout + n) * 2) = make_float2(ssum, ssq);
   }
 }
 
@@ -506,6 +581,7 @@
   const int epv = dtype == K22_F32 ? 4 : 8;
   if (C % epv || p.C0 % epv) return k22_set_error(K22_EINVAL, "gn_apply: channel alignment");
   if (p.out_x3 && dtype != K22_F32) return k22_set_error(K22_EINVAL, "gn_apply: x3-chunk output is an option of the fp32 launch");
+  if (p.raw_out != nullptr && (p.mode == 0 || p.C1 != 0)) return k22_set_error(K22_EINVAL, "gn_apply: the raw resampled output goes with mode 1 / 2 and a single input tensor");
   const int Ho = p.mode == 1 ? p.H / 2 : (p.mode == 2 ? p.H * 2 : p.H);
   const int Wo = p.mode == 1 ? p.W / 2 : (p.mode == 2 ? p.W * 2 : p.W);
   const int Hp = Ho + 2 * p.pad, Wp = Wo + 2 * p.pad;
@@ -527,7 +603,35 @@
   K22_CHECK_LAUNCH();
   return K22_OK;
 }
+template <typename T, int CIN>
+static void launch_conv_in_rows(const ConvInParams& p, hipStream_t s) {
+  const int rpw = (p.H + 127) / 128, halves = p.Cout <= 384 ? 2 : 1;
+  const size_t lds = conv_in_rows_lds_bytes(CIN, p.W, p.Cout);
+  hipLaunchKernelGGL((conv_in_rows_kernel<T, CIN>), dim3(conv_in_rpi(p.H), p.B), dim3(p.Cout * halves), lds, s, p, rpw, halves);
+}
+
 int launch_conv_in(const ConvInParams& p, int dtype, hipStream_t s) {
+  if (p.stats != nullptr && !p.rows) return k22_set_error(K22_EINVAL, "conv_in: the GroupNorm partial sums come from the row kernel");
+  if (p.rows) {
+    if (!conv_in_rows_supported(p.Cin, p.W, p.Cout) || p.B > 65535) return k22_set_error(K22_EINVAL, "conv_in: the row kernel needs Cout % 64 == 0, Cout <= 768 and a row patch that fits the LDS");
+    if (p.Cin == 4) {
+      if (dtype == K22_BF16) launch_conv_in_rows<bf16_t, 4>(p, s);
+      else if (dtype == K22_F16) launch_conv_in_rows<f16_t, 4>(p, s);
+      else launch_conv_in_rows<float, 4>(p, s);
+    } else if (p.Cin == 9) {
+      if (dtype == K22_BF16) launch_conv_in_rows<bf16_t, 9>(p, s);
+      else if (dtype == K22_F16) launch_conv_in_rows<f16_t, 9>(p, s);
+      else launch_conv_in_rows<float, 9>(p, s);
+    } else if (p.Cin == 8) {
+      if (dtype == K22_BF16) launch_conv_in_rows<bf16_t, 8>(p, s);
+      else if (dtype == K22_F16) launch_conv_in_rows<f16_t, 8>(p, s);
+      else launch_conv_in_rows<float, 8>(p, s);
+    } else {
+      return k22_set_error(K22_EINVAL, "conv_in: in_channels must be 4, 8 or 9");
+    }
+    K22_CHECK_LAUNCH();
+    return K22_OK;
+  }
   dim3 grid((p.W + CONV_IN_PT - 1) / CONV_IN_PT, p.H, p.B);
   if (p.Cin == 4) {
     if (dtype == K22_BF16) hipLaunchKernelGGL((conv_in_kernel<bf16_t, 4>), grid, dim3(128), 0, s, p);
diff --git a/kandinsky-2_amd/csrc/engine.hip b/kandinsky-2_amd/csrc/engine.hip
--- a/kandinsky-2_amd/csrc/engine.hip
+++ b/kandinsky-2_amd/csrc/engine.hip
@@ -41,6 +41,7 @@
   int H = 0, W = 0;
   const Tuned* p0 = nullptr; Slot* st0 = nullptr;
   const Tuned* p1 = nullptr; Slot* st1 = nullptr;
+  int rpi0 = 0, rpi1 = 0;
   int C() const { return C0 + C1; }
 };
 
@@ -71,6 +72,8 @@
     frag_done = true;
     return K22_OK;
   }
+  int lean = 1;
+  const float* xin_cur = nullptr;
   bool cond_set = false;
   GraphCache loop;
   std::vector<unsigned long long> loop_key;
@@ -129,7 +132,7 @@
   int run_ops(hipStream_t st) { return run_ops_range(st, 0, ops.size()); }
 
   void op_gn(OpList& L, const Act& in, const std::string& pfx, int64_t film_off,
-             int act, int mode, int pad, Slot* dst, const GnLink* link = nullptr) {
+             int act, int mode, int pad, Slot* dst, const GnLink* link = nullptr, Slot* raw_dst = nullptr) {
     const int Bn = B, C = in.C(), HW = in.H * in.W;
     const int nsplit = gn_nsplit(Bn, HW);
     const bool fused = in.st0 != nullptr && (in.s1 == nullptr || in.st1 != nullptr);
@@ -149,8 +152,8 @@
       const void* x1 = a.s1 ? ptr(a.s1) : nullptr;
       GnCoeffParams cp = {};
       if (fused) {
-        cp.src[0].st = ptr<float>(a.st0); cp.src[0].rpi = a.p0->rpi; cp.src[0].C = a.C0;
-        if (a.s1) { cp.src[1].st = ptr<float>(a.st1); cp.src[1].rpi = a.p1->rpi; cp.src[1].C = a.C1; }
+        cp.src[0].st = ptr<float>(a.st0); cp.src[0].rpi = a.p0 ? a.p0->rpi : a.rpi0; cp.src[0].C = a.C0;
+        if (a.s1) { cp.src[1].st = ptr<float>(a.st1); cp.src[1].rpi = a.p1 ? a.p1->rpi : a.rpi1; cp.src[1].C = a.C1; }
         if (cp.src[0].rpi <= 0 || (a.s1 && cp.src[1].rpi <= 0)) return k22_set_error(K22_EINVAL, "unet: producer delivered no GroupNorm partial sums");
       } else {
         GnStatsParams sp;
@@ -167,6 +170,7 @@
       GnApplyParams ap = {};
       ap.x0 = x0; ap.x1 = x1; ap.C0 = a.C0; ap.C1 = a.C1; ap.B = Bn; ap.H = a.H; ap.W = a.W;
       ap.mode = mode; ap.pad = pad; ap.act = act; ap.coeff = ptr<float>(s_coeff); ap.out = ptr(dst); ap.out_x3 = x3;
+      ap.raw_out = raw_dst ? ptr(raw_dst) : nullptr;
       int rc = launch_gn_coeff(cp, Bn, st);
       if (rc) return rc;
       if (link != nullptr && link->consumer != nullptr && conv3_algo_fuses_gn(link->consumer->cfg.algo)) return K22_OK;
@@ -303,7 +307,9 @@
     const int Wo = updown == 1 ? in.W / 2 : (updown == 2 ? in.W * 2 : in.W);
     GnLink* l1 = nullptr;
     if (fuse_gn && updown == 0) { gn_links.emplace_back(); l1 = &gn_links.back(); }
-    op_gn(ops, in, pfx + ".in_layers.0", -1, K22_ACT_SILU, updown, 1, s_P1, l1);
+    const bool fold_rs = updown != 0 && lean && in.s1 == nullptr;
+    if (fold_rs) need(s_S, (size_t)B * Ho * Wo * Cin * esz);
+    op_gn(ops, in, pfx + ".in_layers.0", -1, K22_ACT_SILU, updown, 1, s_P1, l1, fold_rs ? s_S : nullptr);
     Tuned* t1 = op_conv(ops, CONV_IN, s_P1, Ho, Wo, Cin, Cout, pfx + ".in_layers.2", nullptr, s_U1, IG_OUT_ROWMAJOR, s_U1st, nullptr, std::string(),
                         l1 ? &in : nullptr, K22_ACT_SILU);
     if (l1) l1->consumer = t1;
@@ -320,7 +326,7 @@
       if (Cin != Cout || in.s1) { if (err.empty()) err = "updown ResBlock with channel change is not supported"; }
       need(s_S, (size_t)B * Ho * Wo * Cin * esz);
       const Act a = in; const int Bn = B, dt = sdt;
-      ops.push_back([=](hipStream_t st) { return launch_resample(ptr(a.s0), ptr(s_S), Bn, a.H, a.W, Cin, updown, dt, st); });
+      if (!fold_rs) ops.push_back([=](hipStream_t st) { return launch_resample(ptr(a.s0), ptr(s_S), Bn, a.H, a.W, Cin, updown, dt, st); });
       skip.s0 = s_S;
     } else if (Cin != Cout) {
       IgemmParams probe = {};
@@ -404,6 +410,7 @@
     if (nB > 8) return k22_set_error(K22_EINVAL, "unet: batch (2*bs) must be <= 8 per engine call");
     begin_plan();
     B = nB; H = nH; W = nW;
+    lean = k22_lean_tail();
     gn_links.clear();
     ops.clear(); cond_ops.clear(); hint_ops.clear(); s_ctxkv.clear(); frag_jobs.clear(); frag_done = false; n_attn = 0;
     cond_set = false; hint_set = false;
@@ -480,14 +487,21 @@
       cp.B = B; cp.H = H; cp.W = W; cp.Cin = cfg.in_channels; cp.Cout = ch;
       const int dt = sdt; const bool inpaint = cfg.in_channels == 9, hinted = cfg.in_channels == 8;
       const int premul = (hinted || cfg.head_type == 1) ? 1 : 0;
+      const bool rows = lean && conv_in_rows_supported(cfg.in_channels, W, ch);
+      Slot* dstat = rows ? new_slot((size_t)B * conv_in_rpi(H) * ch * 2 * sizeof(float)) : nullptr;
+      cp.rows = rows ? 1 : 0;
+      const int half_b = B / 2;
       ops.push_back([=](hipStream_t st) {
         ConvInParams q = cp;
-        q.x = ptr<float>(s_xin); q.img = inpaint ? ptr<float>(s_img) : (hinted ? ptr<float>(s_hint) : nullptr);
+        q.x = ptr<float>(s_xin);
+        if (xin_cur) { q.x = xin_cur; q.x_mod = half_b; }
+        q.img = inpaint ? ptr<float>(s_img) : (hinted ? ptr<float>(s_hint) : nullptr);
         q.mask = inpaint ? ptr<float>(s_mask) : nullptr; q.img_premul = premul;
-        q.out = ptr(d);
+        q.out = ptr(d); q.stats = dstat ? ptr<float>(dstat) : nullptr;
         return launch_conv_in(q, dt, st);
       });
       Act a; a.s0 = d; a.C0 = ch; a.H = H; a.W = W;
+      if (dstat) { a.st0 = dstat; a.rpi0 = conv_in_rpi(H); }
       hs.push_back(a);
     }
     Act h = hs.back();
@@ -526,7 +540,7 @@
       for (int i = 0; i <= cfg.num_res_blocks; ++i) {
         const Act skip = hs.back(); hs.pop_back();
         Act cat; cat.s0 = h.s0; cat.C0 = h.C0; cat.s1 = skip.s0; cat.C1 = skip.C0; cat.H = h.H; cat.W = h.W;
-        cat.p0 = h.p0; cat.st0 = h.st0; cat.p1 = skip.p0; cat.st1 = skip.st0;
+        cat.p0 = h.p0; cat.st0 = h.st0; cat.rpi0 = h.rpi0; cat.p1 = skip.p0; cat.st1 = skip.st0; cat.rpi1 = skip.rpi0;
         if (skip.H != h.H || skip.W != h.W) return k22_set_error(K22_EINVAL, "unet: skip shape mismatch");
         const int co = mc * cfg.channel_mult[l];
         const std::string pfx = "output_blocks." + std::to_string(blk);
@@ -795,8 +809,12 @@
     }
     float* cur = x; float* nxt = x_tmp;
     for (int k = 0; k < n_steps; ++k) {
-      if (int rc = copy_d2d(u->ptr(u->s_xin), cur, half, s)) return rc;
-      if (int rc = copy_d2d(u->ptr(u->s_xin) + half, cur, half, s)) return rc;
+      if (u->lean) {
+        u->xin_cur = cur;
+      } else {
+        if (int rc = copy_d2d(u->ptr(u->s_xin), cur, half, s)) return rc;
+        if (int rc = copy_d2d(u->ptr(u->s_xin) + half, cur, half, s)) return rc;
+      }
       if (hoist) {
         u->film_cur = fa_film + (int64_t)k * B * u->film_total;
       } else {
@@ -809,7 +827,7 @@
       p.table = table; p.step = nullptr; p.step_host = table_rows[k]; p.guidance = guidance; p.clamp_lo = clamp_lo; p.clamp_hi = clamp_hi;
       p.use_cfg = 1; p.n_lo = pct_index; p.gamma = pct_gamma;
       p.s_buf = reinterpret_cast<float*>(scratch); p.x0_buf = reinterpret_cast<float*>(scratch) + 64;
-      p.x_out = nxt; p.x0_out = nullptr; p.N = B; p.HW = HW;
+      p.x_out = nxt; p.x0_out = nullptr; p.N = B; p.HW = HW; p.lean = u->lean;
       rc = launch_sampler_step(p, s);
       if (rc) return rc;
       float* t_ = cur; cur = nxt; nxt = t_;
@@ -817,7 +835,7 @@
     if (cur != x) return copy_d2d(x, cur, (size_t)B * 4 * HW * sizeof(float), s);
     return K22_OK;
   };
-  auto run_loop = [&](hipStream_t s) -> int { const int rc = run_loop_body(s); u->film_cur = nullptr; return rc; };
+  auto run_loop = [&](hipStream_t s) -> int { const int rc = run_loop_body(s); u->film_cur = nullptr; u->xin_cur = nullptr; return rc; };
   if (!use_graph) return run_loop(st);
   std::vector<unsigned long long> key = {(unsigned long long)(uintptr_t)x, (unsigned long long)(uintptr_t)x_tmp, (unsigned long long)(uintptr_t)timesteps,
       (unsigned long long)(uintptr_t)noise_seq, (unsigned long long)(uintptr_t)init_img, (unsigned long long)(uintptr_t)mask,
diff --git a/kandinsky-2_amd/csrc/sampler.hip b/kandinsky-2_amd/csrc/sampler.hip
--- a/kandinsky-2_amd/csrc/sampler.hip
+++ b/kandinsky-2_amd/csrc/sampler.hip
@@ -15,22 +15,24 @@
   return ue + p.guidance * (ce - ue);
 }
 
+__device__ __forceinline__ float sampler_x0_at(const SamplerParams& p, int64_t i, float sr, float srm1) {
+  const int pix = (int)(i % p.HW);
+  const int c = (int)((i / p.HW) % 4), n = (int)(i / (4 * (int64_t)p.HW));
+  const float eps = guided_eps(p, n, c, pix);
+  float x0 = __fsub_rn(__fmul_rn(sr, p.x[i]), __fmul_rn(srm1, eps));
+  x0 = fminf(fmaxf(x0, p.clamp_lo), p.clamp_hi);
+  if (p.mask != nullptr) {
+    const float mk = p.mask[(int64_t)n * p.HW + pix];
+    x0 = __fadd_rn(__fmul_rn(x0, 1.f - mk), __fmul_rn(p.init_img[i], mk));
+  }
+  return x0;
+}
+
 __global__ __launch_bounds__(256) void sampler_x0_kernel(SamplerParams p) {
   const float* tr = step_row(p);
   const float sr = tr[0], srm1 = tr[1];
   const int64_t total = (int64_t)p.N * 4 * p.HW;
-  for (int64_t i = (int64_t)blockIdx.x * 256 + threadIdx.x; i < total; i += (int64_t)gridDim.x * 256) {
-    const int pix = (int)(i % p.HW);
-    const int c = (int)((i / p.HW) % 4), n = (int)(i / (4 * (int64_t)p.HW));
-    const float eps = guided_eps(p, n, c, pix);
-    float x0 = __fsub_rn(__fmul_rn(sr, p.x[i]), __fmul_rn(srm1, eps));
-    x0 = fminf(fmaxf(x0, p.clamp_lo), p.clamp_hi);
-    if (p.mask != nullptr) {
-      const float mk = p.mask[(int64_t)n * p.HW + pix];
-      x0 = __fadd_rn(__fmul_rn(x0, 1.f - mk), __fmul_rn(p.init_img[i], mk));
-    }
-    p.x0_buf[i] = x0;
-  }
+  for (int64_t i = (int64_t)blockIdx.x * 256 + threadIdx.x; i < total; i += (int64_t)gridDim.x * 256) p.x0_buf[i] = sampler_x0_at(p, i, sr, srm1);
 }
 
 __device__ __forceinline__ void hist_add_aggregated(int* hist, bool valid, uint32_t bin) {
@@ -46,13 +48,67 @@
   if ((todo >> lane) & 1) atomicAdd(&hist[bin], 1);
 }
 
+constexpr int K22_RS_BINS0 = 1024;
+__global__ __launch_bounds__(256) void sampler_x0_hist_kernel(SamplerParams p, int* rows) {
+  __shared__ int hist[K22_RS_BINS0];
+  const float* tr = step_row(p);
+  const float sr = tr[0], srm1 = tr[1];
+  const int64_t total = (int64_t)p.N * 4 * p.HW;
+  const int64_t base = (int64_t)blockIdx.x * K22_SAMPLER_EPB;
+  const int64_t n0 = 4 * (int64_t)p.HW;
+  const bool counts = base < n0;
+  if (counts) {
+    for (int i = threadIdx.x; i < K22_RS_BINS0; i += 256) hist[i] = 0;
+    __syncthreads();
+  }
+  float v[K22_SAMPLER_EPB / 256];
+#pragma unroll
+  for (int j = 0; j < K22_SAMPLER_EPB / 256; ++j) {
+    const int64_t i = base + j * 256 + threadIdx.x;
+    v[j] = i < total ? sampler_x0_at(p, i, sr, srm1) : 0.f;
+  }
+#pragma unroll
+  for (int j = 0; j < K22_SAMPLER_EPB / 256; ++j) {
+    const int64_t i = base + j * 256 + threadIdx.x;
+    if (i < total) p.x0_buf[i] = v[j];
+    if (counts) hist_add_aggregated(hist, i < n0, __float_as_uint(fabsf(v[j])) >> 21);
+  }
+  if (counts) {
+    __syncthreads();
+    int* row = rows + (int64_t)blockIdx.x * K22_RS_BINS0;
+    for (int i = threadIdx.x; i < K22_RS_BINS0; i += 256) row[i] = hist[i];
+  }
+}
+
 constexpr int K22_RS_BINS = 2048;
+__device__ __forceinline__ void pick_bin(const int* hist, int nb, int k, uint32_t* bc) {
+  const int tid = threadIdx.x;
+  const int per = nb >> 6;
+  int run = 0;
+  for (int j = 0; j < per; ++j) run += hist[tid * per + j];
+  int incl = run;
+#pragma unroll
+  for (int o = 1; o < 64; o <<= 1) {
+    const int t = __shfl_up(incl, o, 64);
+    if (tid >= o) incl += t;
+  }
+  const int excl = incl - run;
+  if (k >= excl && k < incl) {
+    int acc = excl;
+    for (int j = 0; j < per; ++j) {
+      const int c = hist[tid * per + j];
+      if (k < acc + c) { bc[0] = (uint32_t)(tid * per + j); bc[1] = (uint32_t)(k - acc); break; }
+      acc += c;
+    }
+  }
+}
+
 template <int KPT>
-__device__ __forceinline__ uint32_t radix_select(const float* v, const uint32_t* keys, int n, int k, int* hist, uint32_t* bc, uint32_t floor_key = 0u) {
+__device__ __forceinline__ uint32_t radix_select(const float* v, const uint32_t* keys, int n, int k, int* hist, uint32_t* bc, uint32_t floor_key = 0u,
+                                                 int first_pass = 0, uint32_t prefix = 0u, uint32_t mask = 0u) {
   const int tid = threadIdx.x;
-  uint32_t prefix = 0, mask = 0;
 #pragma unroll 1
-  for (int pass = 0; pass < 3; ++pass) {
+  for (int pass = first_pass; pass < 3; ++pass) {
     const int shift = pass == 0 ? 21 : (pass == 1 ? 10 : 0);
     const int nb = pass == 2 ? 1024 : 2048;
     const uint32_t dmask = (uint32_t)(nb - 1);
@@ -78,26 +134,7 @@
       }
     }
     __syncthreads();
-    if (tid < 64) {
-      const int per = nb >> 6;
-      int run = 0;
-      for (int j = 0; j < per; ++j) run += hist[tid * per + j];
-      int incl = run;
-#pragma unroll
-      for (int o = 1; o < 64; o <<= 1) {
-        const int t = __shfl_up(incl, o, 64);
-        if (tid >= o) incl += t;
-      }
-      const int excl = incl - run;
-      if (k >= excl && k < incl) {
-        int acc = excl;
-        for (int j = 0; j < per; ++j) {
-          const int c = hist[tid * per + j];
-          if (k < acc + c) { bc[0] = (uint32_t)(tid * per + j); bc[1] = (uint32_t)(k - acc); break; }
-          acc += c;
-        }
-      }
-    }
+    if (tid < 64) pick_bin(hist, nb, k, bc);
     __syncthreads();
     prefix |= bc[0] << shift;
     mask |= dmask << shift;
@@ -107,8 +144,8 @@
   return prefix;
 }
 
-template <int KPT>
-__global__ __launch_bounds__(1024) void sampler_threshold_kernel(SamplerParams p) {
+template <int KPT, bool LEAN>
+__global__ __launch_bounds__(1024) void sampler_threshold_kernel(SamplerParams p, const int* rows, int nrows) {
   __shared__ int hist[K22_RS_BINS];
   __shared__ uint32_t bc[2];
   __shared__ unsigned int succ_cnt[2];
@@ -124,7 +161,20 @@
   }
   uint32_t floor_key = 0u;
   int k_sel = p.n_lo;
-  if constexpr (KPT >= 16) {
+  if constexpr (LEAN) {
+    int tot = 0;
+    int r = 0;
+    for (; r + 3 < nrows; r += 4) {
+      const int a0 = rows[(int64_t)r * K22_RS_BINS0 + threadIdx.x], a1 = rows[(int64_t)(r + 1) * K22_RS_BINS0 + threadIdx.x];
+      const int a2 = rows[(int64_t)(r + 2) * K22_RS_BINS0 + threadIdx.x], a3 = rows[(int64_t)(r + 3) * K22_RS_BINS0 + threadIdx.x];
+      tot += (a0 + a1) + (a2 + a3);
+    }
+    for (; r < nrows; ++r) tot += rows[(int64_t)r * K22_RS_BINS0 + threadIdx.x];
+    hist[threadIdx.x] = tot;
+    __syncthreads();
+    if (threadIdx.x < 64) pick_bin(hist, K22_RS_BINS0, p.n_lo, bc);
+    __syncthreads();
+  } else if constexpr (KPT >= 16) {
     __shared__ unsigned int n_ge;
     uint32_t skey = 0xffffffffu;
     const int js = (int)threadIdx.x % KPT;
@@ -153,7 +203,15 @@
       __syncthreads();
     }
   }
-  const uint32_t ka = radix_select<KPT>(p.x0_buf, keys, n, k_sel, hist, bc, floor_key);
+  uint32_t ka;
+  if constexpr (LEAN) {
+    const uint32_t d0 = bc[0];
+    k_sel = (int)bc[1];
+    __syncthreads();
+    ka = radix_select<KPT>(p.x0_buf, keys, n, k_sel, hist, bc, 0u, 1, d0 << 21, 0x7ffu << 21);
+  } else {
+    ka = radix_select<KPT>(p.x0_buf, keys, n, k_sel, hist, bc, floor_key);
+  }
   if (threadIdx.x == 0) { succ_cnt[0] = 0u; succ_cnt[1] = 0xffffffffu; }
   __syncthreads();
   unsigned int cnt = 0, mn = 0xffffffffu;
@@ -319,15 +377,25 @@
   const int64_t total = (int64_t)p.N * 4 * p.HW;
   int nb = (int)((total + 255) / 256);
   if (nb > 2048) nb = 2048;
-  hipLaunchKernelGGL(sampler_x0_kernel, dim3(nb), dim3(256), 0, s, p);
-  K22_CHECK_LAUNCH();
-  if (p.n_lo >= 0) {
-    const int kpt = (4 * p.HW + 1023) / 1024;
-    if (kpt <= 4) hipLaunchKernelGGL(sampler_threshold_kernel<4>, dim3(1), dim3(1024), 0, s, p);
-    else if (kpt <= 16) hipLaunchKernelGGL(sampler_threshold_kernel<16>, dim3(1), dim3(1024), 0, s, p);
-    else if (kpt <= 36) hipLaunchKernelGGL(sampler_threshold_kernel<36>, dim3(1), dim3(1024), 0, s, p);
-    else if (kpt <= 64) hipLaunchKernelGGL(sampler_threshold_kernel<64>, dim3(1), dim3(1024), 0, s, p);
-    else hipLaunchKernelGGL(sampler_threshold_kernel<0>, dim3(1), dim3(1024), 0, s, p);
+  const int kpt = (4 * p.HW + 1023) / 1024;
+  const bool lean = p.lean && p.n_lo >= 0 && sampler_hist_bytes(p.HW) > 0;
+  int* rows = reinterpret_cast<int*>(p.x0_buf + total);
+  const int nrows = (4 * p.HW + K22_SAMPLER_EPB - 1) / K22_SAMPLER_EPB;
+  if (lean) hipLaunchKernelGGL(sampler_x0_hist_kernel, dim3((unsigned)((total + K22_SAMPLER_EPB - 1) / K22_SAMPLER_EPB)), dim3(256), 0, s, p, rows);
+  else hipLaunchKernelGGL(sampler_x0_kernel, dim3(nb), dim3(256), 0, s, p);
+  K22_CHECK_LAUNCH();
+  if (lean) {
+    if (kpt <= 4) hipLaunchKernelGGL((sampler_threshold_kernel<4, true>), dim3(1), dim3(1024), 0, s, p, rows, nrows);
+    else if (kpt <= 16) hipLaunchKernelGGL((sampler_threshold_kernel<16, true>), dim3(1), dim3(1024), 0, s, p, rows, nrows);
+    else if (kpt <= 36) hipLaunchKernelGGL((sampler_threshold_kernel<36, true>), dim3(1), dim3(1024), 0, s, p, rows, nrows);
+    else hipLaunchKernelGGL((sampler_threshold_kernel<64, true>), dim3(1), dim3(1024), 0, s, p, rows, nrows);
+    K22_CHECK_LAUNCH();
+  } else if (p.n_lo >= 0) {
+    if (kpt <= 4) hipLaunchKernelGGL((sampler_threshold_kernel<4, false>), dim3(1), dim3(1024), 0, s, p, nullptr, 0);
+    else if (kpt <= 16) hipLaunchKernelGGL((sampler_threshold_kernel<16, false>), dim3(1), dim3(1024), 0, s, p, nullptr, 0);
+    else if (kpt <= 36) hipLaunchKernelGGL((sampler_threshold_kernel<36, false>), dim3(1), dim3(1024), 0, s, p, nullptr, 0);
+    else if (kpt <= 64) hipLaunchKernelGGL((sampler_threshold_kernel<64, false>), dim3(1), dim3(1024), 0, s, p, nullptr, 0);
+    else hipLaunchKernelGGL((sampler_threshold_kernel<0, false>), dim3(1), dim3(1024), 0, s, p, nullptr, 0);
     K22_CHECK_LAUNCH();
   }
   hipLaunchKernelGGL(sampler_final_kernel, dim3(nb), dim3(256), 0, s, p);
```

Measured after the change: 149.4 steps/s (median of 6 runs). Within noise of the previous version (+0.8%).
